# Ntropy86/review-recommender

Hardware: AMD Instinct MI355X
Metric: queries/sec at top-k=100 (hybrid alpha=0.5) (higher is better)
Workload: dtype f32; 1 GPU; hybrid BM25+dense alpha=0.5 top-k=100 pool=150, 10000000 products x 384 fp32, BM25 ~40 tokens/doc vocab 200000 (327073593 postings on rank 0, 11164874 postings per query), batches of 256 queries; query_sets=4, docs=10000000, docs_per_gpu=10000000, batch=256, k=100, pool=150, parallelism=single GPU: no collective

## Files before the change

include/rr_hip.h:

```cpp
#ifndef RR_HIP_H
#define RR_HIP_H

#include <stdint.h>

#ifdef __cplusplus
extern "C" {
#endif

#define RR_OK            0
#define RR_E_INVALID    -1
#define RR_E_HIP        -2
#define RR_E_NOMEM      -3
#define RR_E_STATE      -4

#define RR_DTYPE_F32     0
#define RR_DTYPE_BF16    1

#define RR_MAX_POOL   2048
#define RR_MAX_BATCH  1024
#define RR_MAX_QTERMS   64

typedef struct rr_index rr_index;
typedef struct rr_bm25  rr_bm25;

const char* rr_last_error(void);
int rr_version(void);
int rr_device_count(int* out);


int rr_index_create(const void* h_matrix, int64_t n_rows, int32_t dim, int32_t dtype,
                    int32_t device, int64_t row_offset, rr_index** out);
int rr_index_upload_rows(rr_index* ix, int64_t first_row, int64_t n_rows, const void* h_rows);
int rr_index_upload_rows_f32(rr_index* ix, int64_t first_row, int64_t n_rows, const float* h_rows,
                             float normalize_eps);
int rr_index_adopt_device(rr_index* ix, const void* d_matrix);
int rr_index_store_rows_dev(rr_index* ix, const float* d_rows, int64_t n, int64_t first_row, const int64_t* d_row_ids,
                            float normalize_eps, void* stream);
int rr_index_download_rows_f32(rr_index* ix, int64_t first_row, int64_t n, float* h_rows);
int rr_index_matrix_changed(rr_index* ix);
int rr_index_dim_padded(const rr_index* ix, int32_t* out);
int rr_index_l2_normalize(rr_index* ix, float eps);
int rr_index_set_meta(rr_index* ix, const double* h_n_reviews, const double* h_avg_stars,
                      const double* h_log1p_n);
int rr_index_destroy(rr_index* ix);


int rr_dense_topk(rr_index* ix, const float* h_queries, int32_t n_queries, int32_t pool,
                  int64_t* h_out_rows, float* h_out_scores, int32_t* pool_out);
int rr_dense_topk_dev(rr_index* ix, const float* d_queries, int32_t n_queries, int32_t pool,
                      int64_t* d_out_rows, float* d_out_scores, void* stream);
int rr_index_last_scan_ms(rr_index* ix, float* out_ms);
int rr_index_scan_stats(rr_index* ix, double* out_total_ms, int64_t* out_launches);
int rr_index_last_scan_info(rr_index* ix, int32_t* out8);
int rr_index_select_trace(rr_index* ix, int32_t* out16);
int rr_index_set_shadow(rr_index* ix, int32_t enable);
#define RR_SCAN_MODE_DEFAULT 0
#define RR_SCAN_MODE_STORED 1
int rr_index_set_scan_mode(rr_index* ix, int32_t mode);


int rr_bm25_create(int32_t device, int64_t n_docs, int64_t n_terms, int64_t nnz,
                   const int64_t* post_indptr, const int32_t* post_docs, const int32_t* post_tf,
                   const int64_t* doc_indptr, const int32_t* doc_terms, const int32_t* doc_tf,
                   const int32_t* doc_len, const double* idf, double avgdl, double k1, double b,
                   int64_t row_offset, rr_bm25** out);
int rr_bm25_create_dev(int32_t device, int64_t n_docs, int64_t n_terms, int64_t nnz,
                       const int64_t* d_post_indptr, const int32_t* d_post_docs, const int32_t* d_post_tf,
                       const int64_t* d_doc_indptr, const int32_t* d_doc_terms, const int32_t* d_doc_tf,
                       const int32_t* d_doc_len, const double* d_idf, double avgdl, double k1, double b,
                       int64_t row_offset, rr_bm25** out);
int rr_bm25_destroy(rr_bm25* bm);
int rr_bm25_get_scores(rr_bm25* bm, const int32_t* h_term_ids, int32_t n_terms_in_query,
                       double* h_out_scores);
int rr_bm25_scores_at(rr_bm25* bm, const int32_t* h_term_ids, const int32_t* h_term_off,
                      int32_t n_queries, const int64_t* h_rows, int32_t pool, int32_t mode,
                      float* h_out);
int rr_bm25_scores_at_dev(rr_bm25* bm, const int32_t* d_term_ids, const int32_t* d_term_off,
                          int32_t n_queries, const int64_t* d_rows, int32_t pool, int32_t mode,
                          float* d_out, void* stream);

int rr_bm25_build(int32_t device, int32_t inputs_on_device, const int32_t* tok, int64_t n_tok,
                  const int64_t* doc_off, int64_t n_src, int64_t n_terms, const int64_t* order,
                  int64_t n_order, int64_t row_lo, int64_t row_hi, double k1, double b,
                  int64_t row_offset, void* stream, rr_bm25** out);
int rr_bm25_build_stats(rr_bm25* bm, int64_t* h_df, int64_t* h_sizes);
int rr_bm25_set_idf(rr_bm25* bm, const double* h_idf, double avgdl);
int rr_bm25_copy_csr(rr_bm25* bm, int64_t* doc_indptr, int32_t* doc_terms, int32_t* doc_tf,
                     int32_t* doc_len, int64_t* post_indptr, int32_t* post_docs, int32_t* post_tf);


#define RR_MAX_CANDIDATES 4096

typedef struct rr_fuse_params {
    double w_dense, w_bm25, w_rerank, w_prior, w_best;
    double prior_C;
    int32_t min_reviews;
    int32_t trust_sat;
    int32_t apply_trust;
    int32_t rerank_active;
    int32_t rerank_k;
    int32_t k;
    int32_t n_candidates;
    int32_t pool;
    int32_t cand_per_rank;
    int32_t bm25_f64;
    int64_t cand_rank_stride_bytes;
} rr_fuse_params;

int rr_fuse_topk_dev(rr_index* ix, const rr_fuse_params* p, int32_t n_queries,
                     const int64_t* d_rows, const float* d_dense, const float* d_bm25,
                     const double* d_n_reviews, const double* d_avg_stars, const double* d_log1p_n,
                     const float* d_rerank, const float* d_best, const float* d_gate,
                     int64_t* d_out_rows, double* d_out_cols, int32_t* d_out_order, void* stream);
int rr_fuse_topk(rr_index* ix, const rr_fuse_params* p, int32_t n_queries,
                 const int64_t* h_rows, const float* h_dense, const float* h_bm25,
                 const double* h_n_reviews, const double* h_avg_stars, const double* h_log1p_n,
                 const float* h_rerank, const float* h_best, const float* h_gate,
                 int64_t* h_out_rows, double* h_out_cols, int32_t* h_out_order);
int rr_index_gather_meta_dev(rr_index* ix, const int64_t* d_rows, int64_t n,
                             double* d_n_reviews, double* d_avg_stars, double* d_log1p_n,
                             void* stream);

#define RR_COPY_MAX_SEGS 4
typedef struct rr_copy_seg {
    void* dst;
    const void* src;
    int64_t row_bytes, rows, dst_pitch, src_pitch;
} rr_copy_seg;
int rr_copy_segments_dev(const rr_copy_seg* segs, int32_t n_segs, int32_t device, void* stream);


typedef struct rr_reviews rr_reviews;
int rr_reviews_create(const float* h_emb, int64_t n_reviews, int32_t dim, int64_t n_products,
                      const int64_t* h_indptr, const int32_t* h_ids, int32_t device,
                      float normalize_eps, rr_reviews** out);
int rr_reviews_destroy(rr_reviews* rv);
int rr_reviews_best_dev(rr_reviews* rv, const float* d_queries, int32_t n_queries,
                        const int64_t* d_rows, int32_t pool, int64_t row_offset, int32_t max_review_id,
                        float* d_best_score, int32_t* d_best_id, void* stream);

int rr_reviews_best_cut_dev(rr_reviews* rv, const float* d_queries, int32_t n_queries,
                            const int64_t* d_rows, int32_t pool, int64_t row_offset, int64_t max_rows,
                            float* d_best_score, int32_t* d_best_id, void* stream);


typedef struct rr_ce rr_ce;
typedef struct rr_ce_config {
    int32_t hidden, n_layers, n_heads, ffn;
    int32_t vocab, max_pos, type_vocab;
    int32_t n_labels;
    float ln_eps;
    int32_t precision;
} rr_ce_config;
#define RR_CE_PRECISION_BF16 0
#define RR_CE_PRECISION_F32 1
int rr_ce_create(int32_t device, const rr_ce_config* cfg, const float* const* h_tensors, int32_t n_tensors, rr_ce** out);
int rr_ce_destroy(rr_ce* ce);
#define RR_CE_OUT_LOGITS 0
#define RR_CE_OUT_CLS    1
#define RR_CE_OUT_HIDDEN 2
int rr_ce_forward_dev(rr_ce* ce, const int32_t* d_token_ids, const int32_t* d_type_ids, const int32_t* d_pos_ids,
                      const int32_t* d_cu_seqlens, int32_t n_seqs, int64_t n_tokens, int32_t max_len, int32_t mode,
                      float* d_out, void* stream);
int rr_ce_last_forward_ms(rr_ce* ce, float* out_ms);
int rr_ce_range_status(rr_ce* ce, int32_t* out_of_range);
int rr_ce_set_wide_range(rr_ce* ce, int32_t on);


typedef struct rr_wp rr_wp;
int rr_wp_create(int32_t device, const uint8_t* h_piece_bytes, const int64_t* h_piece_off, int32_t n_pieces,
                 int32_t unk_id, int32_t cls_id, int32_t sep_id, int32_t max_chars_per_word, rr_wp** out);
int rr_wp_destroy(rr_wp* wp);
int rr_wp_create_utf8(int32_t device, const uint8_t* h_piece_bytes, const int64_t* h_piece_off, int32_t n_pieces,
                      int32_t unk_id, int32_t cls_id, int32_t sep_id, int32_t max_chars_per_word,
                      const uint16_t* h_stage1, int32_t n_stage1, const uint32_t* h_stage2, int32_t n_stage2,
                      const uint32_t* h_pool, int32_t n_pool, rr_wp** out);
int rr_wp_encode_dev(rr_wp* wp, const uint8_t* d_text, int64_t text_bytes, const int64_t* d_text_off, int32_t n_docs,
                     int32_t max_length, int64_t token_capacity, int32_t* d_token_ids, int32_t* d_type_ids, int32_t* d_pos_ids,
                     int32_t* d_cu_seqlens, int32_t* d_needs_host, int32_t* d_max_len, void* stream);
int rr_wp_status(rr_wp* wp, int32_t* out_bad_docs);
int rr_wp_table_slots(int32_t n_pieces, int32_t* out_slots);
int rr_wp_build_table(const uint8_t* h_piece_bytes, const int64_t* h_piece_off, int32_t n_pieces, int32_t max_chars_per_word,
                      int32_t n_slots, int32_t* h_slots, int32_t* out_kept);
int rr_wp_build_table_utf8(const uint8_t* h_piece_bytes, const int64_t* h_piece_off, int32_t n_pieces, int32_t max_chars_per_word,
                           int32_t n_slots, int32_t* h_slots, int32_t* out_kept);

int rr_dense_scan_dev(rr_index* ix, const float* d_queries, int32_t n_queries, int32_t top_k, int32_t kth,
                      float* d_bound, int32_t* applied, void* stream);
int rr_dense_select_dev(rr_index* ix, const float* d_queries, int32_t n_queries, int32_t top_k,
                        const float* d_floor, int64_t* d_out_rows, float* d_out_scores, void* stream);

int rr_dense_scan_slot_dev(rr_index* ix, int32_t slot, const float* d_queries, int32_t n_queries, int32_t top_k, int32_t kth,
                           float* d_bound, int32_t* applied, void* stream);
int rr_dense_select_slot_dev(rr_index* ix, int32_t slot, int32_t n_queries, int32_t top_k, const float* d_floor,
                             int64_t* d_out_rows, float* d_out_scores, void* stream);
int rr_dense_topk_slot_dev(rr_index* ix, int32_t slot, const float* d_queries, int32_t n_queries, int32_t top_k,
                           int64_t* d_out_rows, float* d_out_scores, void* stream);
#define RR_SELECT_LIST    1
#define RR_SELECT_RESCORE 2
#define RR_SELECT_ORDER   4
int rr_dense_select_part_dev(rr_index* ix, int32_t slot, int32_t parts, int32_t n_queries, int32_t top_k, const float* d_floor,
                             int64_t* d_out_rows, float* d_out_scores, void* stream);
int rr_stream_create_cu_range(int32_t device, int32_t first_cu, int32_t n_cus, void** out_stream);
int rr_stream_destroy(void* stream);
int rr_index_set_scan_cus(rr_index* ix, int32_t n_cus);

int rr_index_stream(rr_index* ix, void** out_stream);
int rr_index_synchronize(rr_index* ix);

#ifdef __cplusplus
}
#endif
#endif
```

review-recommender_amd/_lib.py:

```python
from __future__ import annotations

import ctypes as C
import os
import threading

from .build import DEBUG_BUILD_ID, BUILD_ID, DEBUG_LIB_PATH, LIB_PATH, library_digest

c_i32, c_i64, c_f32, c_f64, c_vp = C.c_int32, C.c_int64, C.c_float, C.c_double, C.c_void_p
P = C.POINTER


class CopySeg(C.Structure):
    _fields_ = [("dst", C.c_void_p), ("src", C.c_void_p), ("row_bytes", C.c_int64), ("rows", C.c_int64),
                ("dst_pitch", C.c_int64), ("src_pitch", C.c_int64)]


class FuseParams(C.Structure):
    _fields_ = [("w_dense", c_f64), ("w_bm25", c_f64), ("w_rerank", c_f64),
                ("w_prior", c_f64), ("w_best", c_f64), ("prior_C", c_f64),
                ("min_reviews", c_i32), ("trust_sat", c_i32), ("apply_trust", c_i32),
                ("rerank_active", c_i32), ("rerank_k", c_i32), ("k", c_i32),
                ("n_candidates", c_i32), ("pool", c_i32), ("cand_per_rank", c_i32),
                ("bm25_f64", c_i32), ("cand_rank_stride_bytes", c_i64)]


class CEConfig(C.Structure):
    _fields_ = [("hidden", c_i32), ("n_layers", c_i32), ("n_heads", c_i32), ("ffn", c_i32),
                ("vocab", c_i32), ("max_pos", c_i32), ("type_vocab", c_i32), ("n_labels", c_i32),
                ("ln_eps", c_f32), ("precision", c_i32)]


PROTOTYPES = {
    "rr_last_error": (C.c_char_p, []),
    "rr_version": (C.c_int, []),
    "rr_device_count": (C.c_int, [P(C.c_int)]),
    "rr_index_create": (C.c_int, [c_vp, c_i64, c_i32, c_i32, c_i32, c_i64, P(c_vp)]),
    "rr_index_upload_rows": (C.c_int, [c_vp, c_i64, c_i64, c_vp]),
    "rr_index_upload_rows_f32": (C.c_int, [c_vp, c_i64, c_i64, c_vp, c_f32]),
    "rr_index_adopt_device": (C.c_int, [c_vp, c_vp]),
    "rr_index_store_rows_dev": (C.c_int, [c_vp, c_vp, c_i64, c_i64, c_vp, c_f32, c_vp]),
    "rr_index_download_rows_f32": (C.c_int, [c_vp, c_i64, c_i64, c_vp]),
    "rr_index_dim_padded": (C.c_int, [c_vp, P(c_i32)]),
    "rr_index_l2_normalize": (C.c_int, [c_vp, c_f32]),
    "rr_index_set_meta": (C.c_int, [c_vp, c_vp, c_vp, c_vp]),
    "rr_index_destroy": (C.c_int, [c_vp]),
    "rr_dense_topk": (C.c_int, [c_vp, c_vp, c_i32, c_i32, c_vp, c_vp, P(c_i32)]),
    "rr_dense_topk_dev": (C.c_int, [c_vp, c_vp, c_i32, c_i32, c_vp, c_vp, c_vp]),
    "rr_index_last_scan_ms": (C.c_int, [c_vp, P(c_f32)]),
    "rr_index_scan_stats": (C.c_int, [c_vp, P(c_f64), P(c_i64)]),
    "rr_index_last_scan_info": (C.c_int, [c_vp, P(c_i32)]),
    "rr_index_select_trace": (C.c_int, [c_vp, P(c_i32)]),
    "rr_index_set_shadow": (C.c_int, [c_vp, c_i32]),
    "rr_index_set_scan_mode": (C.c_int, [c_vp, c_i32]),
    "rr_dense_scan_dev": (C.c_int, [c_vp, c_vp, c_i32, c_i32, c_i32, c_vp, P(c_i32), c_vp]),
    "rr_dense_select_dev": (C.c_int, [c_vp, c_vp, c_i32, c_i32, c_vp, c_vp, c_vp, c_vp]),
    "rr_dense_scan_slot_dev": (C.c_int, [c_vp, c_i32, c_vp, c_i32, c_i32, c_i32, c_vp, P(c_i32), c_vp]),
    "rr_dense_select_slot_dev": (C.c_int, [c_vp, c_i32, c_i32, c_i32, c_vp, c_vp, c_vp, c_vp]),
    "rr_dense_topk_slot_dev": (C.c_int, [c_vp, c_i32, c_vp, c_i32, c_i32, c_vp, c_vp, c_vp]),
    "rr_dense_select_part_dev": (C.c_int, [c_vp, c_i32, c_i32, c_i32, c_i32, c_vp, c_vp, c_vp, c_vp]),
    "rr_stream_create_cu_range": (C.c_int, [c_i32, c_i32, c_i32, P(c_vp)]),
    "rr_stream_destroy": (C.c_int, [c_vp]),
    "rr_index_set_scan_cus": (C.c_int, [c_vp, c_i32]),
    "rr_bm25_create": (C.c_int, [c_i32, c_i64, c_i64, c_i64, c_vp, c_vp, c_vp, c_vp, c_vp,
                                 c_vp, c_vp, c_vp, c_f64, c_f64, c_f64, c_i64, P(c_vp)]),
    "rr_bm25_create_dev": (C.c_int, [c_i32, c_i64, c_i64, c_i64, c_vp, c_vp, c_vp, c_vp, c_vp,
                                     c_vp, c_vp, c_vp, c_f64, c_f64, c_f64, c_i64, P(c_vp)]),
    "rr_bm25_destroy": (C.c_int, [c_vp]),
    "rr_bm25_get_scores": (C.c_int, [c_vp, c_vp, c_i32, c_vp]),
    "rr_bm25_scores_at": (C.c_int, [c_vp, c_vp, c_vp, c_i32, c_vp, c_i32, c_i32, c_vp]),
    "rr_bm25_scores_at_dev": (C.c_int, [c_vp, c_vp, c_vp, c_i32, c_vp, c_i32, c_i32, c_vp, c_vp]),
    "rr_bm25_build": (C.c_int, [c_i32, c_i32, c_vp, c_i64, c_vp, c_i64, c_i64, c_vp, c_i64, c_i64, c_i64,
                                c_f64, c_f64, c_i64, c_vp, P(c_vp)]),
    "rr_bm25_build_stats": (C.c_int, [c_vp, c_vp, c_vp]),
    "rr_bm25_set_idf": (C.c_int, [c_vp, c_vp, c_f64]),
    "rr_bm25_copy_csr": (C.c_int, [c_vp] + [c_vp] * 7),
    "rr_fuse_topk_dev": (C.c_int, [c_vp, P(FuseParams), c_i32] + [c_vp] * 9 + [c_vp] * 3 + [c_vp]),
    "rr_fuse_topk": (C.c_int, [c_vp, P(FuseParams), c_i32] + [c_vp] * 9 + [c_vp] * 3),
    "rr_index_gather_meta_dev": (C.c_int, [c_vp, c_vp, c_i64, c_vp, c_vp, c_vp, c_vp]),
    "rr_copy_segments_dev": (C.c_int, [c_vp, c_i32, c_i32, c_vp]),
    "rr_index_matrix_changed": (C.c_int, [c_vp]),
    "rr_reviews_create": (C.c_int, [c_vp, c_i64, c_i32, c_i64, c_vp, c_vp, c_i32, c_f32, P(c_vp)]),
    "rr_reviews_destroy": (C.c_int, [c_vp]),
    "rr_reviews_best_dev": (C.c_int, [c_vp, c_vp, c_i32, c_vp, c_i32, c_i64, c_i32, c_vp, c_vp, c_vp]),
    "rr_reviews_best_cut_dev": (C.c_int, [c_vp, c_vp, c_i32, c_vp, c_i32, c_i64, c_i64, c_vp, c_vp, c_vp]),
    "rr_ce_create": (C.c_int, [c_i32, P(CEConfig), P(c_vp), c_i32, P(c_vp)]),
    "rr_ce_destroy": (C.c_int, [c_vp]),
    "rr_ce_forward_dev": (C.c_int, [c_vp, c_vp, c_vp, c_vp, c_vp, c_i32, c_i64, c_i32, c_i32, c_vp, c_vp]),
    "rr_ce_last_forward_ms": (C.c_int, [c_vp, P(c_f32)]),
    "rr_ce_range_status": (C.c_int, [c_vp, P(C.c_int32)]),
    "rr_ce_set_wide_range": (C.c_int, [c_vp, C.c_int32]),
    "rr_wp_create": (C.c_int, [c_i32, c_vp, c_vp, c_i32, c_i32, c_i32, c_i32, c_i32, P(c_vp)]),
    "rr_wp_create_utf8": (C.c_int, [c_i32, c_vp, c_vp, c_i32, c_i32, c_i32, c_i32, c_i32, c_vp, c_i32, c_vp, c_i32, c_vp, c_i32,
                                    P(c_vp)]),
    "rr_wp_destroy": (C.c_int, [c_vp]),
    "rr_wp_encode_dev": (C.c_int, [c_vp, c_vp, c_i64, c_vp, c_i32, c_i32, c_i64, c_vp, c_vp, c_vp, c_vp, c_vp, c_vp, c_vp]),
    "rr_wp_status": (C.c_int, [c_vp, P(c_i32)]),
    "rr_wp_table_slots": (C.c_int, [c_i32, P(c_i32)]),
    "rr_wp_build_table": (C.c_int, [c_vp, c_vp, c_i32, c_i32, c_i32, c_vp, P(c_i32)]),
    "rr_wp_build_table_utf8": (C.c_int, [c_vp, c_vp, c_i32, c_i32, c_i32, c_vp, P(c_i32)]),
    "rr_index_stream": (C.c_int, [c_vp, P(c_vp)]),
    "rr_index_synchronize": (C.c_int, [c_vp]),
}

DEBUG_PROTOTYPES = {
    "rr_debug_scan_x3w": (C.c_int, [c_vp, c_i32, c_i32, P(c_f32)]),
    "rr_debug_scan_flt": (C.c_int, [c_vp, c_i32, c_i32, P(c_f32)]),
    "rr_debug_fltq_compare": (C.c_int, [c_vp, P(c_i64)]),
    "rr_debug_flt_words": (C.c_int, [c_vp, c_vp, c_i32, c_i32, c_i32, c_i32, c_i32, c_vp, c_vp, c_vp, c_vp, c_i64, c_vp, c_i64]),
    "rr_debug_flt_select": (C.c_int, [c_vp, c_i32, c_vp, c_i64, c_vp, c_vp, c_vp, c_vp]),
    "rr_debug_select_traces": (C.c_int, [c_vp, c_i32, c_vp]),
    "rr_debug_ce_ffn_stamps": (C.c_int, [P(C.c_uint64)]),
    "rr_debug_ce_h2_stamps": (C.c_int, [P(C.c_uint64)]),
    "rr_debug_ce_h2_gemm": (C.c_int, [c_i32, c_i32, c_i32, c_i32, c_vp, c_vp, c_vp, c_i32, c_vp, P(C.c_int32)]),
    "rr_debug_ce_h2_attention": (C.c_int, [c_vp, c_i32, c_vp, c_i32, c_i32, c_i32, c_i32, c_vp, P(C.c_int32)]),
    "rr_debug_ce_h2_add_ln": (C.c_int, [c_vp, c_vp, c_i32, c_vp, c_vp, c_f32, c_vp, c_vp, P(C.c_int32)]),
}

_lib = None
_lock = threading.Lock()


class HipLibraryError(RuntimeError):
    pass


def load():
    global _lib
    with _lock:
        if _lib is not None:
            return _lib
        debug = os.environ.get("RR_DEBUG_HARNESS") == "1"
        path = DEBUG_LIB_PATH if debug else LIB_PATH
        if not path.exists():
            raise HipLibraryError(
                f"{path} is missing: build it with `python __graft_entry__.py` "
                "(hipcc --offload-arch=gfx950).  There is no CPU fallback.")
        _refuse_stale(path, DEBUG_BUILD_ID if debug else BUILD_ID, debug)
        import torch
        lib = C.CDLL(str(path))
        protos = dict(PROTOTYPES, **DEBUG_PROTOTYPES) if debug else PROTOTYPES
        for name, (res, args) in protos.items():
            try:
                fn = getattr(lib, name)
            except AttributeError:
                raise HipLibraryError(f"stale library: {path.name} lacks the declared symbol {name}; rebuild it with "
                                      "`python __graft_entry__.py`") from None
            fn.restype = res
            fn.argtypes = args
        _lib = lib
        return lib


def _refuse_stale(path, build_id, debug: bool) -> None:
    have = build_id.read_text().strip() if build_id.exists() else None
    if have != library_digest(debug):
        raise HipLibraryError(
            f"stale library: {path.name} was built from other sources than the ones in csrc/ "
            f"(buildid {'missing' if have is None else have[:12]} != {library_digest(debug)[:12]}); "
            "rebuild it with `python __graft_entry__.py`")


def check(rc: int, what: str = "") -> None:
    if rc == 0:
        return
    msg = load().rr_last_error().decode("utf-8", "replace")
    if rc == -1:
        raise ValueError(f"{what}: {msg}" if what else msg)
    raise HipLibraryError(f"{what}: {msg} (status {rc})" if what else f"{msg} (status {rc})")


def ptr(a):
    if a is None:
        return None
    if not a.flags["C_CONTIGUOUS"]:
        raise ValueError("array passed to the HIP library must be C-contiguous")
    return a.ctypes.data_as(c_vp)
```

review-recommender_amd/csrc/rr_bm25.hip:

```cpp
#include "rr_common.h"

#define RR_SLICE 4096
#define RR_AT_CANDS 64

struct rr_bm25_view {
    const int64_t* post_indptr;
    const int32_t* post_docs;
    const int32_t* post_tf;
    const int64_t* doc_indptr;
    const int32_t* doc_terms;
    const int32_t* doc_tf;
    const int32_t* doc_len;
    const double* idf;
    double avgdl, k1, b;
    int64_t n_docs, n_terms, row_offset;
};

__device__ __forceinline__ double rr_bm25_term(double idf, int tf, int dl, double avgdl, double k1,
                                               double b) {
    const double f = (double)tf;
    const double one_minus_b = 1.0 - b;
    const double norm = one_minus_b + (b * (double)dl) / avgdl;
    return idf * ((f * (k1 + 1.0)) / (f + k1 * norm));
}

__device__ __forceinline__ int64_t rr_lower_bound(const int32_t* __restrict__ a, int64_t lo,
                                                  int64_t hi, int32_t key) {
    while (lo < hi) {
        const int64_t mid = lo + ((hi - lo) >> 1);
        if (a[mid] < key) lo = mid + 1; else hi = mid;
    }
    return lo;
}

__device__ __forceinline__ int64_t rr_lower_bound_wave(const int32_t* __restrict__ a, int64_t lo, int64_t hi, int32_t key) {
    const int lane = threadIdx.x & 63;
    while (hi - lo > 64) {
        const int64_t stride = (hi - lo + 63) >> 6;
        const int64_t at = lo + lane * stride;
        const bool below = at < hi && a[at] < key;
        const int c = __popcll(__ballot(below));
        if (c == 0) return lo;
        const int64_t nlo = lo + (int64_t)(c - 1) * stride + 1, nhi = lo + (int64_t)c * stride;
        lo = nlo;
        hi = nhi < hi ? nhi : hi;
    }
    const bool below = lo + lane < hi && a[lo + lane] < key;
    return lo + __popcll(__ballot(below));
}

#define RR_SLICE_TERMS 16
__global__ __launch_bounds__(256) void rr_bm25_slices(rr_bm25_view v, const int32_t* __restrict__ terms,
                                                      int n_terms_q, double* __restrict__ out, unsigned char* __restrict__ dirty) {
    __shared__ double acc[RR_SLICE];
    __shared__ int64_t range[RR_SLICE_TERMS][2];
    __shared__ int touched;
    const int tid = threadIdx.x, wave = tid >> 6;
    const int64_t d0 = (int64_t)blockIdx.x * RR_SLICE;
    const int64_t d1 = d0 + RR_SLICE < v.n_docs ? d0 + RR_SLICE : v.n_docs;
    for (int i = tid; i < RR_SLICE; i += 256) acc[i] = 0.0;
    if (tid == 0) touched = 0;
    for (int j0 = 0; j0 < n_terms_q; j0 += RR_SLICE_TERMS) {
        const int nj = n_terms_q - j0 < RR_SLICE_TERMS ? n_terms_q - j0 : RR_SLICE_TERMS;
        __syncthreads();
        for (int sidx = wave; sidx < 2 * nj; sidx += 4) {
            const int32_t t = terms[j0 + (sidx >> 1)];
            int64_t r = 0;
            if (t >= 0 && t < v.n_terms)
                r = rr_lower_bound_wave(v.post_docs, v.post_indptr[t], v.post_indptr[t + 1], (int32_t)((sidx & 1) ? d1 : d0));
            if ((tid & 63) == 0) range[sidx >> 1][sidx & 1] = r;
        }
        __syncthreads();
        int32_t nd = 0, ntf = 0, ndl = 0;
        bool nhave = false;
        {
            const int64_t p = range[0][0] + tid;
            nhave = p < range[0][1];
            if (nhave) { nd = v.post_docs[p]; ntf = v.post_tf[p]; ndl = v.doc_len[nd]; }
        }
        for (int j = 0; j < nj; ++j) {
            const int64_t lo = range[j][0], hi = range[j][1];
            const int32_t t = terms[j0 + j];
            const bool have = nhave;
            const int32_t d = nd, tf = ntf, dl = ndl;
            if (j + 1 < nj) {
                const int64_t p = range[j + 1][0] + tid;
                nhave = p < range[j + 1][1];
                if (nhave) { nd = v.post_docs[p]; ntf = v.post_tf[p]; ndl = v.doc_len[nd]; }
            }
            if (hi > lo) {
                const double idf = v.idf[t];
                if (tid == 0) touched = 1;
                if (have) acc[d - d0] += rr_bm25_term(idf, tf, dl, v.avgdl, v.k1, v.b);
                for (int64_t p = lo + 256 + tid; p < hi; p += 256) {
                    const int32_t dd = v.post_docs[p];
                    acc[dd - d0] += rr_bm25_term(idf, v.post_tf[p], v.doc_len[dd], v.avgdl, v.k1, v.b);
                }
            }
            __syncthreads();
        }
    }
    __syncthreads();
    const bool write = touched || dirty[blockIdx.x];
    if (write)
        for (int64_t i = tid; i < d1 - d0; i += 256) out[d0 + i] = acc[i];
    if (tid == 0) dirty[blockIdx.x] = (unsigned char)touched;
}

template <int MODE>
__global__ __launch_bounds__(256) void rr_bm25_at(rr_bm25_view v, const int32_t* __restrict__ term_ids,
                                                  const int32_t* __restrict__ term_off,
                                                  const int64_t* __restrict__ rows, int pool,
                                                  float* __restrict__ out) {
    __shared__ double contrib[RR_AT_CANDS][RR_MAX_QTERMS + 1];
    const int tid = threadIdx.x;
    const int q = blockIdx.y;
    const int c0 = blockIdx.x * RR_AT_CANDS;
    const int t0 = term_off[q];
    const int nt = term_off[q + 1] - t0;
    const int nc = pool - c0 < RR_AT_CANDS ? pool - c0 : RR_AT_CANDS;
    double sum = 0.0;

    for (int jb = 0; jb < nt; jb += RR_MAX_QTERMS) {
        const int nj = nt - jb < RR_MAX_QTERMS ? nt - jb : RR_MAX_QTERMS;
        for (int i = tid; i < nc * nj; i += 256) {
            const int c = i / nj, j = i % nj;
            const int64_t d = rows[(int64_t)q * pool + c0 + c] - v.row_offset;
            const int32_t t = term_ids[t0 + jb + j];
            double val = 0.0;
            if (d >= 0 && d < v.n_docs && t >= 0 && t < v.n_terms) {
                int tf = 0;
                if (MODE == 0) {
                    const int64_t s = v.doc_indptr[d], e = v.doc_indptr[d + 1];
                    const int64_t p = rr_lower_bound(v.doc_terms, s, e, t);
                    if (p < e && v.doc_terms[p] == t) tf = v.doc_tf[p];
                } else {
                    const int64_t s = v.post_indptr[t], e = v.post_indptr[t + 1];
                    const int64_t p = rr_lower_bound(v.post_docs, s, e, (int32_t)d);
                    if (p < e && v.post_docs[p] == (int32_t)d) tf = v.post_tf[p];
                }
                if (tf > 0) val = rr_bm25_term(v.idf[t], tf, v.doc_len[d], v.avgdl, v.k1, v.b);
            }
            contrib[c][j] = val;
        }
        __syncthreads();
        if (tid < nc)
            for (int j = 0; j < nj; ++j) sum += contrib[tid][j];
        __syncthreads();
    }
    if (tid < nc) out[(int64_t)q * pool + c0 + tid] = (float)sum;
}

template <typename T>
static int rr_upload(T** dst, const T* src, size_t n) {
    *dst = nullptr;
    RR_HIP_TRY(hipMalloc((void**)dst, sizeof(T) * (n ? n : 1)));
    if (n) RR_HIP_TRY(hipMemcpy(*dst, src, sizeof(T) * n, hipMemcpyHostToDevice));
    return RR_OK;
}

static rr_bm25_view rr_view(const rr_bm25* bm) {
    rr_bm25_view v;
    v.post_indptr = bm->d_post_indptr; v.post_docs = bm->d_post_docs; v.post_tf = bm->d_post_tf;
    v.doc_indptr = bm->d_doc_indptr; v.doc_terms = bm->d_doc_terms; v.doc_tf = bm->d_doc_tf;
    v.doc_len = bm->d_doc_len; v.idf = bm->d_idf;
    v.avgdl = bm->avgdl; v.k1 = bm->k1; v.b = bm->b;
    v.n_docs = bm->n_docs; v.n_terms = bm->n_terms; v.row_offset = bm->row_offset;
    return v;
}

extern "C" int rr_bm25_create(int32_t device, int64_t n_docs, int64_t n_terms, int64_t nnz,
                              const int64_t* post_indptr, const int32_t* post_docs,
                              const int32_t* post_tf, const int64_t* doc_indptr,
                              const int32_t* doc_terms, const int32_t* doc_tf,
                              const int32_t* doc_len, const double* idf, double avgdl, double k1,
                              double b, int64_t row_offset, rr_bm25** out) {
    RR_REQUIRE(out, "rr_bm25_create: NULL out");
    *out = nullptr;
    RR_REQUIRE(n_docs >= 1 && n_docs < (1ll << 31), "rr_bm25_create: n_docs %lld out of range",
               (long long)n_docs);
    RR_REQUIRE(n_terms >= 0 && n_terms < (1ll << 31) && nnz >= 0, "rr_bm25_create: bad sizes");
    RR_REQUIRE(post_indptr && doc_indptr && doc_len && (nnz == 0 || (post_docs && post_tf && doc_terms && doc_tf)) &&
                   (n_terms == 0 || idf),
               "rr_bm25_create: NULL array");
    RR_REQUIRE(post_indptr[n_terms] == nnz && doc_indptr[n_docs] == nnz,
               "rr_bm25_create: indptr tails (%lld, %lld) do not match nnz %lld",
               (long long)post_indptr[n_terms], (long long)doc_indptr[n_docs], (long long)nnz);
    RR_REQUIRE(avgdl > 0.0, "rr_bm25_create: avgdl must be positive");
    RR_HIP_TRY(hipSetDevice(device));
    rr_bm25* bm = new rr_bm25();
    bm->device = device; bm->n_docs = n_docs; bm->n_terms = n_terms; bm->nnz = nnz;
    bm->avgdl = avgdl; bm->k1 = k1; bm->b = b; bm->row_offset = row_offset;
    int rc = RR_OK;
    if (!rc) rc = rr_upload(&bm->d_post_indptr, post_indptr, (size_t)n_terms + 1);
    if (!rc) rc = rr_upload(&bm->d_post_docs, post_docs, (size_t)nnz);
    if (!rc) rc = rr_upload(&bm->d_post_tf, post_tf, (size_t)nnz);
    if (!rc) rc = rr_upload(&bm->d_doc_indptr, doc_indptr, (size_t)n_docs + 1);
    if (!rc) rc = rr_upload(&bm->d_doc_terms, doc_terms, (size_t)nnz);
    if (!rc) rc = rr_upload(&bm->d_doc_tf, doc_tf, (size_t)nnz);
    if (!rc) rc = rr_upload(&bm->d_doc_len, doc_len, (size_t)n_docs);
    if (!rc) rc = rr_upload(&bm->d_idf, idf, (size_t)n_terms);
    if (!rc && hipStreamCreateWithFlags(&bm->stream, hipStreamNonBlocking) != hipSuccess) {
        rr_set_error("rr_bm25_create: hipStreamCreate failed");
        rc = RR_E_HIP;
    }
    if (rc) { rr_bm25_destroy(bm); return rc; }
    *out = bm;
    return RR_OK;
}

extern "C" int rr_bm25_create_dev(int32_t device, int64_t n_docs, int64_t n_terms, int64_t nnz,
                                  const int64_t* d_post_indptr, const int32_t* d_post_docs,
                                  const int32_t* d_post_tf, const int64_t* d_doc_indptr,
                                  const int32_t* d_doc_terms, const int32_t* d_doc_tf,
                                  const int32_t* d_doc_len, const double* d_idf, double avgdl,
                                  double k1, double b, int64_t row_offset, rr_bm25** out) {
    RR_REQUIRE(out, "rr_bm25_create_dev: NULL out");
    *out = nullptr;
    RR_REQUIRE(n_docs >= 1 && n_docs < (1ll << 31) && n_terms >= 1 && n_terms < (1ll << 31) && nnz >= 1,
               "rr_bm25_create_dev: bad sizes");
    RR_REQUIRE(d_post_indptr && d_post_docs && d_post_tf && d_doc_indptr && d_doc_terms && d_doc_tf &&
                   d_doc_len && d_idf, "rr_bm25_create_dev: NULL array");
    RR_REQUIRE(avgdl > 0.0, "rr_bm25_create_dev: avgdl must be positive");
    RR_HIP_TRY(hipSetDevice(device));
    int64_t tails[2] = {-1, -1};
    RR_HIP_TRY(hipMemcpy(&tails[0], d_post_indptr + n_terms, sizeof(int64_t), hipMemcpyDeviceToHost));
    RR_HIP_TRY(hipMemcpy(&tails[1], d_doc_indptr + n_docs, sizeof(int64_t), hipMemcpyDeviceToHost));
    RR_REQUIRE(tails[0] == nnz && tails[1] == nnz, "rr_bm25_create_dev: indptr tails (%lld, %lld) != nnz %lld",
               (long long)tails[0], (long long)tails[1], (long long)nnz);
    rr_bm25* bm = new rr_bm25();
    bm->device = device; bm->n_docs = n_docs; bm->n_terms = n_terms; bm->nnz = nnz;
    bm->avgdl = avgdl; bm->k1 = k1; bm->b = b; bm->row_offset = row_offset;
    bm->owns_arrays = false;
    bm->d_post_indptr = const_cast<int64_t*>(d_post_indptr);
    bm->d_post_docs = const_cast<int32_t*>(d_post_docs);
    bm->d_post_tf = const_cast<int32_t*>(d_post_tf);
    bm->d_doc_indptr = const_cast<int64_t*>(d_doc_indptr);
    bm->d_doc_terms = const_cast<int32_t*>(d_doc_terms);
    bm->d_doc_tf = const_cast<int32_t*>(d_doc_tf);
    bm->d_doc_len = const_cast<int32_t*>(d_doc_len);
    bm->d_idf = const_cast<double*>(d_idf);
    if (hipStreamCreateWithFlags(&bm->stream, hipStreamNonBlocking) != hipSuccess) {
        rr_set_error("rr_bm25_create_dev: hipStreamCreate failed");
        delete bm;
        return RR_E_HIP;
    }
    *out = bm;
    return RR_OK;
}

extern "C" int rr_bm25_destroy(rr_bm25* bm) {
    if (!bm) return RR_OK;
    hipSetDevice(bm->device);
    if (bm->owns_arrays) {
        hipFree(bm->d_post_indptr); hipFree(bm->d_post_docs); hipFree(bm->d_post_tf);
        hipFree(bm->d_doc_indptr); hipFree(bm->d_doc_terms); hipFree(bm->d_doc_tf);
        hipFree(bm->d_doc_len); hipFree(bm->d_idf); hipFree(bm->d_df);
    }
    hipFree(bm->d_scores);
    hipFree(bm->d_dirty);
    if (bm->stream) hipStreamDestroy(bm->stream);
    delete bm;
    return RR_OK;
}

extern "C" int rr_bm25_get_scores(rr_bm25* bm, const int32_t* h_term_ids, int32_t n_terms_in_query,
                                  double* h_out_scores) {
    RR_REQUIRE(bm && h_out_scores && (n_terms_in_query == 0 || h_term_ids),
               "rr_bm25_get_scores: NULL argument");
    RR_REQUIRE(n_terms_in_query >= 0 && n_terms_in_query <= 4096,
               "rr_bm25_get_scores: %d query tokens out of [0,4096]", n_terms_in_query);
    if (!bm->d_idf) { rr_set_error("rr_bm25_get_scores: no idf yet (rr_bm25_set_idf)"); return RR_E_STATE; }
    std::lock_guard<std::mutex> lk(bm->mu);
    RR_HIP_TRY(hipSetDevice(bm->device));
    const unsigned grid = (unsigned)((bm->n_docs + RR_SLICE - 1) / RR_SLICE);
    if (!bm->d_scores) {
        RR_HIP_TRY(hipMalloc((void**)&bm->d_scores, sizeof(double) * (size_t)bm->n_docs));
        RR_HIP_TRY(hipMalloc((void**)&bm->d_dirty, grid));
        RR_HIP_TRY(hipMemsetAsync(bm->d_scores, 0, sizeof(double) * (size_t)bm->n_docs, bm->stream));
        RR_HIP_TRY(hipMemsetAsync(bm->d_dirty, 0, grid, bm->stream));
    }
    int32_t* d_terms = nullptr;
    RR_HIP_TRY(hipMalloc((void**)&d_terms, sizeof(int32_t) * (size_t)(n_terms_in_query + 1)));
    if (n_terms_in_query)
        hipMemcpyAsync(d_terms, h_term_ids, sizeof(int32_t) * n_terms_in_query, hipMemcpyHostToDevice,
                       bm->stream);
    hipLaunchKernelGGL(rr_bm25_slices, dim3(grid), dim3(256), 0, bm->stream, rr_view(bm), d_terms,
                       n_terms_in_query, bm->d_scores, bm->d_dirty);
    hipError_t e = hipGetLastError();
    if (e == hipSuccess)
        e = hipMemcpyAsync(h_out_scores, bm->d_scores, sizeof(double) * (size_t)bm->n_docs,
                           hipMemcpyDeviceToHost, bm->stream);
    if (e == hipSuccess) e = hipStreamSynchronize(bm->stream);
    hipFree(d_terms);
    if (e != hipSuccess) {
        rr_set_error("rr_bm25_get_scores: %s", hipGetErrorString(e));
        return RR_E_HIP;
    }
    return RR_OK;
}

extern "C" int rr_bm25_scores_at_dev(rr_bm25* bm, const int32_t* d_term_ids,
                                     const int32_t* d_term_off, int32_t n_queries,
                                     const int64_t* d_rows, int32_t pool, int32_t mode,
                                     float* d_out, void* stream) {
    RR_REQUIRE(bm && d_term_ids && d_term_off && d_rows && d_out, "rr_bm25_scores_at_dev: NULL argument");
    RR_REQUIRE(n_queries >= 1 && n_queries <= RR_MAX_BATCH && pool >= 1 && pool <= 8 * RR_MAX_POOL,
               "rr_bm25_scores_at_dev: n_queries %d / pool %d out of range", n_queries, pool);
    RR_REQUIRE(mode == 0 || mode == 1, "rr_bm25_scores_at_dev: mode must be 0 (forward) or 1 (postings)");
    if (!bm->d_idf) { rr_set_error("rr_bm25_scores_at_dev: no idf yet (rr_bm25_set_idf)"); return RR_E_STATE; }
    RR_HIP_TRY(hipSetDevice(bm->device));
    hipStream_t st = (hipStream_t)stream;
    dim3 grid((unsigned)((pool + RR_AT_CANDS - 1) / RR_AT_CANDS), (unsigned)n_queries);
    if (mode == 0)
        hipLaunchKernelGGL((rr_bm25_at<0>), grid, dim3(256), 0, st, rr_view(bm), d_term_ids, d_term_off,
                           d_rows, pool, d_out);
    else
        hipLaunchKernelGGL((rr_bm25_at<1>), grid, dim3(256), 0, st, rr_view(bm), d_term_ids, d_term_off,
                           d_rows, pool, d_out);
    RR_HIP_TRY(hipGetLastError());
    return RR_OK;
}

extern "C" int rr_bm25_scores_at(rr_bm25* bm, const int32_t* h_term_ids, const int32_t* h_term_off,
                                 int32_t n_queries, const int64_t* h_rows, int32_t pool,
                                 int32_t mode, float* h_out) {
    RR_REQUIRE(bm && h_term_off && h_rows && h_out, "rr_bm25_scores_at: NULL argument");
    RR_REQUIRE(n_queries >= 1 && n_queries <= RR_MAX_BATCH && pool >= 1 && pool <= 8 * RR_MAX_POOL,
               "rr_bm25_scores_at: n_queries %d / pool %d out of range", n_queries, pool);
    const int total_terms = h_term_off[n_queries];
    RR_REQUIRE(total_terms >= 0 && (total_terms == 0 || h_term_ids), "rr_bm25_scores_at: bad term arrays");
    for (int q = 0; q < n_queries; ++q)
        RR_REQUIRE(h_term_off[q + 1] - h_term_off[q] >= 0, "rr_bm25_scores_at: term offsets must not decrease (query %d)", q);
    std::lock_guard<std::mutex> lk(bm->mu);
    RR_HIP_TRY(hipSetDevice(bm->device));
    int32_t *d_ids = nullptr, *d_off = nullptr;
    int64_t* d_rows = nullptr;
    float* d_out = nullptr;
    const size_t n_out = (size_t)n_queries * pool;
    hipError_t e = hipMalloc((void**)&d_ids, sizeof(int32_t) * (size_t)(total_terms + 1));
    if (e == hipSuccess) e = hipMalloc((void**)&d_off, sizeof(int32_t) * (size_t)(n_queries + 1));
    if (e == hipSuccess) e = hipMalloc((void**)&d_rows, sizeof(int64_t) * n_out);
    if (e == hipSuccess) e = hipMalloc((void**)&d_out, sizeof(float) * n_out);
    if (e == hipSuccess && total_terms)
        e = hipMemcpyAsync(d_ids, h_term_ids, sizeof(int32_t) * total_terms, hipMemcpyHostToDevice, bm->stream);
    if (e == hipSuccess)
        e = hipMemcpyAsync(d_off, h_term_off, sizeof(int32_t) * (n_queries + 1), hipMemcpyHostToDevice, bm->stream);
    if (e == hipSuccess)
        e = hipMemcpyAsync(d_rows, h_rows, sizeof(int64_t) * n_out, hipMemcpyHostToDevice, bm->stream);
    int rc = RR_OK;
    if (e == hipSuccess)
        rc = rr_bm25_scores_at_dev(bm, d_ids, d_off, n_queries, d_rows, pool, mode, d_out, bm->stream);
    if (e == hipSuccess && rc == RR_OK)
        e = hipMemcpyAsync(h_out, d_out, sizeof(float) * n_out, hipMemcpyDeviceToHost, bm->stream);
    if (e == hipSuccess && rc == RR_OK) e = hipStreamSynchronize(bm->stream);
    hipFree(d_ids); hipFree(d_off); hipFree(d_rows); hipFree(d_out);
    if (rc) return rc;
    if (e != hipSuccess) {
        rr_set_error("rr_bm25_scores_at: %s", hipGetErrorString(e));
        return RR_E_HIP;
    }
    return RR_OK;
}
```

review-recommender_amd/csrc/rr_common.h:

```cpp
#pragma once

#include <hip/hip_runtime.h>
#include <stdint.h>
#include <stdio.h>
#include <string.h>
#include <mutex>
#include <string>

#include "../../include/rr_hip.h"

void rr_set_error(const char* fmt, ...);

#define RR_HIP_TRY(expr)                                                        \
    do {                                                                        \
        hipError_t _e = (expr);                                                 \
        if (_e != hipSuccess) {                                                 \
            rr_set_error("%s failed: %s (%s:%d)", #expr, hipGetErrorString(_e), \
                         __FILE__, __LINE__);                                   \
            return RR_E_HIP;                                                    \
        }                                                                       \
    } while (0)

#define RR_REQUIRE(cond, ...)             \
    do {                                  \
        if (!(cond)) {                    \
            rr_set_error(__VA_ARGS__);    \
            return RR_E_INVALID;          \
        }                                 \
    } while (0)

#define RR_SCAN_SLOTS 3
struct rr_scan_slot {
    float* d_q = nullptr;
    void* d_qplanes = nullptr;
    float* d_eps = nullptr;
    float* d_gmax = nullptr;
    uint32_t* d_smax = nullptr;
    int32_t maxima_q = 0;
    float* d_flt_samp = nullptr;
    float* d_flt_sigma = nullptr;
    uint32_t* d_flt_prog = nullptr;
    uint32_t flt_seq = 0;
    bool flt_prep_fresh = false;
    void* flt_pending = nullptr;
};

struct rr_index {
    int device = 0;
    int64_t n_rows = 0;
    int32_t dim = 0;
    int32_t dim_pad = 0;
    int32_t dtype = RR_DTYPE_F32;
    int64_t row_offset = 0;
    void* d_matrix = nullptr;
    bool owns_matrix = true;
    double* d_n_reviews = nullptr;
    double* d_avg_stars = nullptr;
    double* d_log1p_n = nullptr;
    bool has_meta = false;
    float* d_sims = nullptr;
    float* d_gmax = nullptr;
    int32_t* d_sel_trace = nullptr;
    int32_t* d_flag_list = nullptr;
    uint32_t* d_smax = nullptr;
    int32_t scratch_q = 0;
    int32_t maxima_q = 0;
    float* d_eps = nullptr;
    float* d_q = nullptr;
    float norm_bound = -1.f;
    float delta_bound = 0.f;
    int32_t last_scan[5] = {0, 0, 0, 0, 0};
    float* d_flt_samp = nullptr;
    float* d_flt_sigma = nullptr;
    uint32_t* d_flt_prog = nullptr;
    uint32_t flt_seq = 0;
    bool scratch_small = false;
    bool flt_prep_fresh = false;
    void* flt_pending = nullptr;
    unsigned short* d_shadow = nullptr;
    bool shadow_valid = false;
    int32_t use_shadow = 1;
    int32_t scan_mode = 0;
    void* d_x3 = nullptr;
    void* d_qplanes = nullptr;
    int64_t* d_rows_out = nullptr;
    float* d_scores_out = nullptr;
    hipStream_t stream = nullptr;
    hipEvent_t ev0 = nullptr, ev1 = nullptr;
    hipEvent_t ev_done = nullptr;
    hipStream_t last_stream = nullptr;
    bool has_done = false;
    rr_scan_slot parked[RR_SCAN_SLOTS];
    int cur_slot = 0;
    hipEvent_t slot_ev[RR_SCAN_SLOTS] = {};
    hipStream_t slot_stream[RR_SCAN_SLOTS] = {};
    bool slot_has[RR_SCAN_SLOTS] = {};
    int32_t n_cus = 0;
    int32_t scan_cus = 0;
    bool timing_valid = false;
    static const int kRing = 512;
    hipEvent_t ring0[kRing] = {}, ring1[kRing] = {};
    int64_t ring_head = 0, ring_tail = 0;
    std::mutex mu;
};

struct rr_bm25 {
    int device = 0;
    int64_t n_docs = 0, n_terms = 0, nnz = 0;
    int64_t row_offset = 0;
    int64_t* d_post_indptr = nullptr;
    int32_t* d_post_docs = nullptr;
    int32_t* d_post_tf = nullptr;
    int64_t* d_doc_indptr = nullptr;
    int32_t* d_doc_terms = nullptr;
    int32_t* d_doc_tf = nullptr;
    int32_t* d_doc_len = nullptr;
    double* d_idf = nullptr;
    int64_t* d_df = nullptr;
    int64_t n_src = 0, length_sum = 0;
    double avgdl = 1.0, k1 = 1.5, b = 0.75;
    bool owns_arrays = true;
    double* d_scores = nullptr;
    unsigned char* d_dirty = nullptr;
    hipStream_t stream = nullptr;
    std::mutex mu;
};

static inline int64_t rr_round_up(int64_t x, int64_t m) { return (x + m - 1) / m * m; }

#ifdef __HIPCC__

typedef float f32x4 __attribute__((ext_vector_type(4)));

__device__ __forceinline__ uint32_t rr_f2key(float f) {
    uint32_t u = __float_as_uint(f);
    return (u & 0x80000000u) ? ~u : (u | 0x80000000u);
}
__device__ __forceinline__ float rr_key2f(uint32_t k) {
    uint32_t u = (k & 0x80000000u) ? (k & 0x7FFFFFFFu) : ~k;
    return __uint_as_float(u);
}

__device__ __forceinline__ float rr_row16_sum(float v) {
    int t;
    t = __builtin_amdgcn_update_dpp(0, __float_as_int(v), 0xB1, 0xF, 0xF, true);
    v = v + __int_as_float(t);
    t = __builtin_amdgcn_update_dpp(0, __float_as_int(v), 0x4E, 0xF, 0xF, true);
    v = v + __int_as_float(t);
    t = __builtin_amdgcn_update_dpp(0, __float_as_int(v), 0x141, 0xF, 0xF, true);
    v = v + __int_as_float(t);
    t = __builtin_amdgcn_update_dpp(0, __float_as_int(v), 0x140, 0xF, 0xF, true);
    v = v + __int_as_float(t);
    return v;
}

__device__ __forceinline__ float rr_wave_max(float v) {
#pragma unroll
    for (int m = 32; m >= 1; m >>= 1) v = fmaxf(v, __shfl_xor(v, m, 64));
    return v;
}

#endif
```

review-recommender_amd/csrc/rr_dense.h:

```cpp
#pragma once
#include "rr_common.h"

#define RR_SCAN_THREADS 256
#define RR_MAX_SCAN_WAVES 8192
#define RR_MFMA_MAXQ 64
#define RR_FLT_MAXQ 128
#define RR_SEL_MAXQ 256
#define RR_FLT_SAMP_CAP 8192
#define RR_FLT_NO_BOUND 1000
#define RR_FLT_SMALL 1001

struct rr_scan_geom {
    int64_t n_rows, n_tiles;
    int64_t tiles_per_wave;
    int32_t n_waves;
    int32_t qs;
    int64_t n_pad;
    int32_t mm_pairs;
    int32_t gpw;
    int64_t tiles_per_group;
};


rr_scan_geom rr_make_geom(const rr_index* ix, int resident_blocks);
static inline void rr_scan_note(rr_index* ix, int kernel, int variant, int nq, int terms, int elem_bytes = 0) {
    ix->last_scan[0] = kernel; ix->last_scan[1] = variant; ix->last_scan[2] = nq; ix->last_scan[3] = terms;
    ix->last_scan[4] = elem_bytes ? elem_bytes : (ix->dtype == RR_DTYPE_BF16 ? 2 : 4);
}
static inline void rr_matrix_written(rr_index* ix) {
    ix->norm_bound = -1.f;
    ix->shadow_valid = false;
}
int rr_slot_activate(rr_index* ix, int slot);
void rr_slot_park(rr_index* ix);
int rr_scan_events_begin(rr_index* ix, hipStream_t st);
void rr_scan_events_end(rr_index* ix, int slot, hipStream_t st);
int rr_dense_listed_fallback(rr_index* ix, const float* d_q, int nq, int pool, int64_t* d_rows, float* d_scores,
                             int32_t* flags, hipStream_t st);
void rr_launch_select(rr_index* ix, const rr_scan_geom& G, int nq, int pool, int64_t* d_rows,
                      float* d_scores, hipStream_t st, const int32_t* only_if = nullptr, int slices = 1,
                      int64_t sims_slice = 0, int64_t gmax_slice = 0, int64_t smax_slice = 0);
#define RR_X3_MCAP 16384
struct rr_x3_scratch {
    uint32_t* mtiles;
    int32_t* count;
    uint32_t* tau;
    int32_t* fb;
    float* eps;
    float* sc;
};
rr_x3_scratch rr_x3_scratch_of(const rr_index* ix);
size_t rr_x3_scratch_bytes();
void rr_launch_select_mtiles(rr_index* ix, const rr_scan_geom& G, int nq, int pool, hipStream_t st,
                             const float* eps = nullptr, const float* sigma = nullptr, int nq_b = 0,
                             int64_t mmax_set_stride = 0, int64_t smax_set_stride = 0, const float* floor = nullptr);
void rr_launch_select_rescored(rr_index* ix, const rr_scan_geom& G, int nq, int pool, int64_t* d_rows,
                               float* d_scores, hipStream_t st, bool floor_mode = false);
void rr_launch_group_kth(rr_index* ix, const rr_scan_geom& G, int nq_a, int nq_b, int kth, const float* eps, float* d_bound,
                         int64_t smax_set_stride, hipStream_t st);
int rr_resident_waves(const void* kernel, int threads, int device);
int rr_dense_chunk_bf16(rr_index* ix, const float* d_q, int nq, int pool, int64_t* d_rows,
                        float* d_scores, hipStream_t st);
int rr_dense_chunk_mfma_bf16(rr_index* ix, const float* d_q, int nq, int pool, int64_t* d_rows,
                             float* d_scores, hipStream_t st);
int rr_l2norm_rows_f32(rr_index* ix, int64_t first_row, int64_t n, float eps, hipStream_t st);
int rr_l2norm_rows_f32_at(float* d_rows, int32_t dim_pad, int64_t n, float eps, hipStream_t st);
int rr_dense_chunk_x3(rr_index* ix, const float* d_q, int nq, int pool, int64_t* d_rows,
                      float* d_scores, hipStream_t st);
int rr_dense_chunk_flt(rr_index* ix, const float* d_q, int nq, int pool, int64_t* d_rows,
                       float* d_scores, hipStream_t st, int phase = 0, int kth = 0, float* d_bound = nullptr,
                       const float* d_floor = nullptr, int parts = 7);
void rr_flt_drop_pending(rr_index* ix);
int rr_store_rows_bf16(rr_index* ix, int64_t first_row, int64_t n, float* d_rows_f32, float eps, hipStream_t st);
int rr_store_rows_bf16_at(void* d_dst, int32_t dim, int32_t dim_pad, int64_t n, const float* d_rows_f32, float eps, hipStream_t st);

int rr_device_visible(const void* p, const void** out, const char* what);

int rr_flt_pad_prep(rr_index* ix, const float* d_queries, int nq, int slots, hipStream_t st);
```

review-recommender_amd/csrc/rr_dense.hip:

```cpp
#include <stdlib.h>

#include "rr_common.h"
#include "rr_dense.h"
#include "rr_x3.h"

#define RR_SEL_THREADS 1024
#define RR_SEL_GCAP 4096
#define RR_SEL_CCAP 12288
#define RR_SEL_SORTCAP 8192
#define RR_SEL_RCAP 8192
#define RR_SEL_LCAP 4096

template <int NF>
__device__ __forceinline__ void rr_load_rows(f32x4 (&dst)[NF], const f32x4* __restrict__ mat,
                                             int64_t row, int64_t n_rows, int sub) {
    row = row < n_rows ? row : n_rows - 1;
    const f32x4* p = mat + row * (int64_t)(NF * 16) + sub;
#pragma unroll
    for (int i = 0; i < NF; ++i) dst[i] = __builtin_nontemporal_load(p + 16 * i);
}

template <int NF, int NB, bool FROM_LDS>
__device__ __forceinline__ void rr_dot_rows(const f32x4 (&x)[NF], const f32x4 (&qreg)[NF],
                                            const f32x4 (*qs)[NF * 16], int sub, int it,
                                            float (&mine)[NB]) {
#pragma unroll
    for (int b = 0; b < NB; ++b) {
        if (FROM_LDS) asm volatile("" ::: "memory");
        float acc = 0.f;
#pragma unroll
        for (int i = 0; i < NF; ++i) {
            const f32x4 q = FROM_LDS ? qs[b][16 * i + sub] : qreg[i];
            acc = __builtin_fmaf(x[i].x, q.x, acc);
            acc = __builtin_fmaf(x[i].y, q.y, acc);
            acc = __builtin_fmaf(x[i].z, q.z, acc);
            acc = __builtin_fmaf(x[i].w, q.w, acc);
        }
        acc = rr_row16_sum(acc);
        mine[b] = (sub == it) ? acc : mine[b];
    }
}

template <int NB>
__device__ __forceinline__ void rr_finish_tile(const rr_scan_geom& G, int64_t tile, int64_t wave,
                                               int64_t t0, int64_t t1, int lane, int sub, int grp,
                                               float (&mine)[NB], float (&gm)[NB],
                                               float* __restrict__ sims, float* __restrict__ gmax,
                                               uint32_t* __restrict__ smax) {
    const int64_t my_row = tile * 64 + 4 * sub + grp;
    const bool valid = my_row < G.n_rows;
    const bool group_end = tile == t1 - 1;
#pragma unroll
    for (int b = 0; b < NB; ++b) {
        float v = mine[b];
        v = (valid && v == v) ? v : -INFINITY;
        sims[(int64_t)b * G.n_pad + my_row] = v;
        const float m = rr_wave_max(v);
        gm[b] = fmaxf(gm[b], m);
        if (lane == 0) {
            gmax[(int64_t)b * G.n_tiles + tile] = m;
            if (group_end)
                smax[(int64_t)b * G.n_waves + wave] = rr_f2key(gm[b]);
        }
        if (group_end) gm[b] = -INFINITY;
    }
}

template <int NB>
__device__ __forceinline__ int rr_flagged_list(const int32_t* __restrict__ flags, int nq, int lane, int (&list)[NB]) {
    int n = 0, total = 0;
#pragma unroll
    for (int b = 0; b < NB; ++b) list[b] = 0;
    for (int i = 0; i < (nq + 63) / 64; ++i) {
        const int q = 64 * i + lane;
        unsigned long long m = __ballot(q < nq && flags[q] != 0);
        total += __builtin_popcountll(m);
        while (m && n < NB) {
            const int b = __builtin_ctzll(m);
            m &= m - 1;
#pragma unroll
            for (int j = 0; j < NB; ++j)
                if (j == n) list[j] = 64 * i + b;
            ++n;
        }
    }
    if (total > NB) return 0;
#pragma unroll
    for (int j = 1; j < NB; ++j)
        if (j >= n && n > 0) list[j] = list[j - 1];
    return n;
}

template <int NF, int NB, bool LISTED = false>
__global__ __launch_bounds__(RR_SCAN_THREADS, (NB <= 1 ? 4 : 2)) void rr_scan_f32(
    const f32x4* __restrict__ mat, rr_scan_geom G, const float* __restrict__ queries,
    float* __restrict__ sims, float* __restrict__ gmax, uint32_t* __restrict__ smax,
    const int32_t* __restrict__ flags = nullptr, int nq_total = 0, int32_t* __restrict__ list_out = nullptr) {
    __shared__ f32x4 qs[NB][NF * 16];
    const int tid = threadIdx.x;
    if (LISTED) {
        int list[NB];
        const int n = rr_flagged_list<NB>(flags, nq_total, tid & 63, list);
        if (blockIdx.x == 0 && tid == 0) {
            list_out[0] = n;
#pragma unroll
            for (int b = 0; b < NB; ++b) list_out[1 + b] = list[b];
        }
        if (n == 0) return;
#pragma unroll
        for (int b = 0; b < NB; ++b)
            for (int i = tid; i < NF * 16; i += RR_SCAN_THREADS)
                qs[b][i] = reinterpret_cast<const f32x4*>(queries)[(int64_t)list[b] * (NF * 16) + i];
    } else {
        for (int i = tid; i < NB * NF * 16; i += RR_SCAN_THREADS)
            qs[i / (NF * 16)][i % (NF * 16)] = reinterpret_cast<const f32x4*>(queries)[i];
    }
    __syncthreads();

    const int lane = tid & 63;
    const int sub = lane & 15;
    const int grp = lane >> 4;
    const int64_t wave = (int64_t)blockIdx.x * (RR_SCAN_THREADS / 64) + (tid >> 6);
    if (wave >= G.n_waves) return;
    const int64_t t0 = wave * G.tiles_per_wave;
    const int64_t t1 = t0 + G.tiles_per_wave < G.n_tiles ? t0 + G.tiles_per_wave : G.n_tiles;

    f32x4 qreg[NF];
#pragma unroll
    for (int i = 0; i < NF; ++i) qreg[i] = (NB == 1) ? qs[0][16 * i + sub] : f32x4{0.f, 0.f, 0.f, 0.f};

    float gm[NB];
#pragma unroll
    for (int b = 0; b < NB; ++b) gm[b] = -INFINITY;

    f32x4 bufA[NF], bufB[NF];
    rr_load_rows<NF>(bufA, mat, t0 * 64 + grp, G.n_rows, sub);
#pragma unroll 1
    for (int64_t tile = t0; tile < t1; ++tile) {
        const int64_t row0 = tile * 64;
        float mine[NB];
#pragma unroll
        for (int b = 0; b < NB; ++b) mine[b] = 0.f;
#pragma unroll(NB == 1 ? 8 : 1)
        for (int it = 0; it < 16; it += 2) {
            rr_load_rows<NF>(bufB, mat, row0 + 4 * (it + 1) + grp, G.n_rows, sub);
            rr_dot_rows<NF, NB, (NB > 1)>(bufA, qreg, qs, sub, it, mine);
            rr_load_rows<NF>(bufA, mat, row0 + 4 * (it + 2) + grp, G.n_rows, sub);
            rr_dot_rows<NF, NB, (NB > 1)>(bufB, qreg, qs, sub, it + 1, mine);
        }
        rr_finish_tile<NB>(G, tile, wave, t0, t1, lane, sub, grp, mine, gm, sims, gmax, smax);
    }
}

template <int NB>
__global__ __launch_bounds__(RR_SCAN_THREADS) void rr_scan_f32_generic(
    const f32x4* __restrict__ mat, rr_scan_geom G, int nf, const float* __restrict__ queries,
    float* __restrict__ sims, float* __restrict__ gmax, uint32_t* __restrict__ smax) {
    const int tid = threadIdx.x;
    const int lane = tid & 63;
    const int sub = lane & 15;
    const int grp = lane >> 4;
    const int64_t wave = (int64_t)blockIdx.x * (RR_SCAN_THREADS / 64) + (tid >> 6);
    if (wave >= G.n_waves) return;
    const int64_t t0 = wave * G.tiles_per_wave;
// ... 263 lines not shown
            const int64_t t = all_tiles ? (i >> 6) : (int64_t)glist[i >> 6];
            const int64_t row = t * 64 + (i & 63);
            if (row < n_rows) {
                const uint64_t key = ((uint64_t)rr_f2key(score_at(row)) << 32) |
                                     (uint64_t)(0xFFFFFFFFu - (uint32_t)row);
                if (key >= prefix) {
                    const uint32_t slot = atomicAdd(&counters[1], 1u);
                    if (slot < RR_SEL_SORTCAP) cand[slot] = key;
                }
            }
        }
        __syncthreads();
        n_cand = counters[1] < RR_SEL_SORTCAP ? counters[1] : RR_SEL_SORTCAP;
    }

    if (n_cand > RR_SEL_SORTCAP) n_cand = RR_SEL_SORTCAP;
    int n_sort = 1;
    while (n_sort < (int)n_cand) n_sort <<= 1;
    for (int i = tid; i < n_sort; i += RR_SEL_THREADS)
        if (i >= (int)n_cand) cand[i] = 0;
    rr_bitonic_desc(cand, n_sort);
}

#define RR_SEL_RK 8
template <int RK>
__device__ uint32_t rr_kth_largest_reg(const uint32_t (&r)[RR_SEL_RK], int n_mine, uint32_t k,
                                       uint32_t (*cnt)[3][16], int& phase, int max_steps) {
    const int tid = threadIdx.x;
    const int ln = tid & 63;
    uint32_t mx = 0, mn = 0xFFFFFFFFu, nz = 0;
#pragma unroll
    for (int j = 0; j < RK; ++j) {
        const bool live = j < n_mine && r[j] != 0u;
        if (j < n_mine) mx = r[j] > mx ? r[j] : mx;
        if (live) mn = r[j] < mn ? r[j] : mn;
        nz += (uint32_t)__popcll(__ballot(live));
    }
#pragma unroll
    for (int m = 32; m >= 1; m >>= 1) {
        const uint32_t a = __shfl_xor(mx, m, 64), b = __shfl_xor(mn, m, 64);
        mx = a > mx ? a : mx;
        mn = b < mn ? b : mn;
    }
    if (ln == 0) {
        cnt[phase][0][tid >> 6] = mx;
        cnt[phase][1][tid >> 6] = mn;
        cnt[phase][2][tid >> 6] = nz;
    }
    __syncthreads();
    uint32_t nz_all = 0;
    for (int w = 0; w < 16; ++w) {
        mx = cnt[phase][0][w] > mx ? cnt[phase][0][w] : mx;
        mn = cnt[phase][1][w] < mn ? cnt[phase][1][w] : mn;
        nz_all += cnt[phase][2][w];
    }
    if (nz_all < k) mn = 0u;
    phase ^= 1;
    if (mx == mn) return mx;
    int bit = 31 - __clz(mx ^ mn);
    uint32_t prefix = (bit == 31) ? 0u : (mx >> (bit + 1)) << (bit + 1);
    for (int step = 0; bit >= 0 && step < max_steps; ++step) {
        const int lo = bit >= 1 ? bit - 1 : 0;
        const bool two = bit >= 1;
        const uint32_t t1 = prefix | (1u << lo);
        const uint32_t t2 = prefix | (1u << bit);
        const uint32_t t3 = prefix | (1u << bit) | (1u << lo);
        uint32_t c1 = 0, c2 = 0, c3 = 0;
#pragma unroll
        for (int j = 0; j < RK; ++j) {
            const bool have = j < n_mine;
            c1 += (uint32_t)__popcll(__ballot(have && r[j] >= t1));
            c2 += (uint32_t)__popcll(__ballot(have && r[j] >= t2));
            c3 += (uint32_t)__popcll(__ballot(have && r[j] >= t3));
        }
        if (ln == 0) {
            cnt[phase][0][tid >> 6] = c1;
            cnt[phase][1][tid >> 6] = c2;
            cnt[phase][2][tid >> 6] = c3;
        }
        __syncthreads();
        int v = ln < 48 ? (int)(&cnt[phase][0][0])[ln] : 0;
        v += __builtin_amdgcn_update_dpp(0, v, 0xB1, 0xF, 0xF, true);
        v += __builtin_amdgcn_update_dpp(0, v, 0x4E, 0xF, 0xF, true);
        v += __builtin_amdgcn_update_dpp(0, v, 0x141, 0xF, 0xF, true);
        v += __builtin_amdgcn_update_dpp(0, v, 0x140, 0xF, 0xF, true);
        const uint32_t s1 = (uint32_t)__builtin_amdgcn_readlane(v, 0);
        const uint32_t s2 = (uint32_t)__builtin_amdgcn_readlane(v, 16);
        const uint32_t s3 = (uint32_t)__builtin_amdgcn_readlane(v, 32);
        phase ^= 1;
        if (two) {
            if (s3 >= k) prefix = t3;
            else if (s2 >= k) prefix = t2;
            else if (s1 >= k) prefix = t1;
        } else if (s2 >= k) {
            prefix = t2;
        }
        bit = lo - 1;
    }
    return prefix;
}

__device__ void rr_rank_sort_desc(const uint64_t* keys, int n, uint64_t* out) {
    const int tid = threadIdx.x;
    uint64_t mine = 0;
    int rank = 0;
    if (tid < n) {
        mine = keys[tid];
        for (int j = 0; j < n; ++j) rank += keys[j] > mine ? 1 : 0;
    }
    __syncthreads();
    if (tid < n) out[rank] = mine;
    __syncthreads();
}

template <typename GroupKeyAt>
__device__ uint32_t rr_sel_open_groups(GroupKeyAt group_key_at, int ng, int pool, uint32_t (*cnt)[3][16],
                                       int& phase, uint32_t* counters, uint32_t* list2,
                                       float eps2 = -1.f, uint32_t* open_key = nullptr, uint32_t thr_floor = 0u) {
    const int tid = threadIdx.x;
    uint32_t r[RR_SEL_RK];
    int n_mine = 0;
#pragma unroll
    for (int j = 0; j < RR_SEL_RK; ++j) {
        const int i = tid + j * RR_SEL_THREADS;
        r[j] = i < ng ? group_key_at(i) : 0u;
        n_mine += i < ng ? 1 : 0;
    }
    uint32_t tau = 1u;
    if (ng > pool) {
        if (ng <= 1 * RR_SEL_THREADS) tau = rr_kth_largest_reg<1>(r, n_mine, (uint32_t)pool, cnt, phase, 7);
        else if (ng <= 2 * RR_SEL_THREADS) tau = rr_kth_largest_reg<2>(r, n_mine, (uint32_t)pool, cnt, phase, 7);
        else if (ng <= 4 * RR_SEL_THREADS) tau = rr_kth_largest_reg<4>(r, n_mine, (uint32_t)pool, cnt, phase, 7);
        else tau = rr_kth_largest_reg<8>(r, n_mine, (uint32_t)pool, cnt, phase, 7);
    }
    if (tau == 0u) tau = 1u;
    uint32_t thr = tau;
    if (eps2 >= 0.f) {
        thr = rr_f2key(rr_key2f(tau) - eps2);
        if (thr == 0u) thr = 1u;
        if (thr_floor > thr) thr = thr_floor;
        if (open_key) *open_key = thr;
    }
#pragma unroll
    for (int j = 0; j < RR_SEL_RK; ++j) {
        if (j < n_mine && r[j] >= thr) {
            const uint32_t slot = atomicAdd(&counters[0], 1u);
            if (slot < RR_SEL_LCAP) list2[slot] = (uint32_t)(tid + j * RR_SEL_THREADS);
        }
    }
    __syncthreads();
    return tau;
}

__global__ __launch_bounds__(RR_SEL_THREADS) void rr_select(
    rr_scan_geom G, const float* __restrict__ sims, const float* __restrict__ gmax,
    const uint32_t* __restrict__ smax, int pool, int64_t row_offset,
    int64_t* __restrict__ out_rows, float* __restrict__ out_scores, int32_t* __restrict__ dbg,
    const int32_t* __restrict__ only_if, int n_total, int64_t sims_slice, int64_t gmax_slice, int64_t smax_slice,
    const int32_t* __restrict__ qlist, int32_t* __restrict__ clear_flags) {
    if (qlist) {
        if ((int)blockIdx.x >= qlist[0]) return;
        const int qo = qlist[1 + blockIdx.x] - (int)blockIdx.x;
        out_rows += (int64_t)qo * pool; out_scores += (int64_t)qo * pool; dbg += qo * 16;
        if (threadIdx.x == 0) clear_flags[qo + (int)blockIdx.x] = 0;
    }
    if (gridDim.y > 1) {
        const int y = blockIdx.y;
        if (64 * y + (int)blockIdx.x >= n_total) return;
        only_if += 64 * y;
        out_rows += (int64_t)64 * y * pool; out_scores += (int64_t)64 * y * pool; dbg += 64 * y * 16;
        sims += y * sims_slice; gmax += y * gmax_slice; smax += y * smax_slice;
    }
    if (only_if && !only_if[blockIdx.x]) return;
    __shared__ uint32_t hist[256];
    __shared__ uint32_t wsum[4];
    __shared__ uint32_t cnt[2][3][16];
    __shared__ uint32_t sel[2];
    __shared__ uint32_t counters[4];
    __shared__ uint32_t list2[RR_SEL_LCAP];
    __shared__ uint32_t list1[RR_SEL_GCAP];
    __shared__ uint64_t cand[RR_SEL_CCAP];

    const int tid = threadIdx.x;
    const int q = blockIdx.x;
    const int QS = G.qs;
    auto score_at = [&](int64_t row) -> float {
        return QS ? sims[((row >> 4) * QS + q) * 16 + (row & 15)] : sims[(int64_t)q * G.n_pad + row];
    };
    auto tile_max_at = [&](int64_t t) -> float {
        return QS ? gmax[t * QS + q] : gmax[(int64_t)q * G.n_tiles + t];
    };
    auto group_key_at = [&](int i) -> uint32_t {
        return QS ? smax[(int64_t)i * QS + q] : smax[(int64_t)q * G.n_waves + i];
    };
    const int64_t n_rows = G.n_rows, n_tiles = G.n_tiles;
    int phase = 0;
    long long stamp[8];
    int n_stamp = 0;
#define RR_STAMP() do { if (n_stamp < 8) stamp[n_stamp++] = clock64(); } while (0)
    RR_STAMP();
    const int ng = G.n_waves;
    bool fast = ng <= RR_SEL_RK * RR_SEL_THREADS;

    if (tid < 4) counters[tid] = 0;
    __syncthreads();

    if (fast) {
        const uint32_t tau = rr_sel_open_groups(group_key_at, ng, pool, cnt, phase, counters, list2);
        RR_STAMP();
        if (counters[0] > RR_SEL_LCAP) fast = false;

        if (fast) {
            const int C = (int)G.tiles_per_wave;
            const int64_t n2 = (int64_t)counters[0] * C;
            for (int64_t i = tid; i < n2; i += RR_SEL_THREADS) {
                const int64_t t = (int64_t)list2[i / C] * C + (i % C);
                if (t < n_tiles && rr_f2key(tile_max_at(t)) >= tau) {
                    const uint32_t slot = atomicAdd(&counters[1], 1u);
                    if (slot < RR_SEL_GCAP) list1[slot] = (uint32_t)t;
                }
            }
            __syncthreads();
            if (counters[1] > RR_SEL_GCAP) fast = false;
        }
        RR_STAMP();
        if (fast) {
            const int n1 = (int)counters[1] * 64;
            for (int i = tid; i < n1; i += RR_SEL_THREADS) {
                const uint32_t row = list1[i >> 6] * 64u + (uint32_t)(i & 63);
                if ((int64_t)row < n_rows) {
                    const uint32_t key = rr_f2key(score_at(row));
                    if (key >= tau) {
                        const uint32_t slot = atomicAdd(&counters[2], 1u);
                        if (slot < RR_SEL_CCAP / 2)
                            cand[slot] = ((uint64_t)key << 32) | (uint64_t)(0xFFFFFFFFu - row);
                    }
                }
            }
            __syncthreads();
            RR_STAMP();
            const uint32_t n_cand = counters[2];
            if (n_cand > RR_SEL_CCAP / 2 || n_cand < (uint32_t)pool) {
                fast = false;
            } else if (n_cand <= RR_SEL_THREADS) {
                rr_rank_sort_desc(cand, (int)n_cand, cand + RR_SEL_CCAP / 2);
                for (int i = tid; i < pool; i += RR_SEL_THREADS) cand[i] = cand[RR_SEL_CCAP / 2 + i];
                __syncthreads();
            } else {
                int n_sort = 1;
                while (n_sort < (int)n_cand) n_sort <<= 1;
                for (int i = tid; i < n_sort; i += RR_SEL_THREADS)
                    if (i >= (int)n_cand) cand[i] = 0;
                rr_bitonic_desc(cand, n_sort);
            }
        }
    }
    RR_STAMP();
    if (tid == 0) {
        dbg[q * 16 + 0] = fast ? 1 : 0;
        dbg[q * 16 + 1] = (int32_t)counters[0];
        dbg[q * 16 + 2] = (int32_t)counters[1];
        dbg[q * 16 + 3] = (int32_t)counters[2];
        for (int i = 1; i < 8; ++i) dbg[q * 16 + 3 + i] = i < n_stamp ? (int32_t)(stamp[i] - stamp[i - 1]) : -1;
    }
    if (!fast) {
        __syncthreads();
        rr_select_slow(score_at, tile_max_at, n_rows, n_tiles, pool, hist, wsum, sel, counters, list1, cand);
    }
    for (int i = tid; i < pool; i += RR_SEL_THREADS) {
        const uint64_t key = cand[i];
        const uint32_t row = 0xFFFFFFFFu - (uint32_t)(key & 0xFFFFFFFFu);
        out_rows[(int64_t)q * pool + i] = (int64_t)row + row_offset;
        out_scores[(int64_t)q * pool + i] = rr_key2f((uint32_t)(key >> 32));
    }
}

__global__ __launch_bounds__(RR_SEL_THREADS) void rr_select_mtiles(
    rr_scan_geom G, const float* __restrict__ mmax, const uint32_t* __restrict__ smax, int pool,
    uint32_t* __restrict__ out_mtiles, int32_t* __restrict__ out_count, uint32_t* __restrict__ out_tau,
    int32_t* __restrict__ fb, int32_t* __restrict__ dbg, const float* __restrict__ eps,
    const float* __restrict__ sigma, int nq_a, int nq_b, int64_t mmax_set_stride, int64_t smax_set_stride,
    const float* __restrict__ floor) {
    __shared__ uint32_t cnt[2][3][16];
    __shared__ uint32_t counters[4];
    __shared__ uint32_t list2[RR_SEL_LCAP];
    const int tid = threadIdx.x;
    const int Q = blockIdx.x;
    const int set = (nq_b > 0 && Q >= nq_a) ? 1 : 0;
    const int q = set ? Q - nq_a : Q;
    const int nq_set = set ? nq_b : nq_a;
    mmax += set * mmax_set_stride;
    smax += set * smax_set_stride;
    if (eps) eps += set * RR_FLT_MAXQ;
    if (sigma) sigma += set * RR_FLT_MAXQ;
    out_mtiles += (int64_t)(Q - q) * RR_X3_MCAP;
    out_count += Q - q; out_tau += Q - q; fb += Q - q; dbg += (Q - q) * 16;
    const int QS = G.qs;
    auto group_key_at = [&](int i) -> uint32_t { return smax[(int64_t)i * QS + q]; };
    const int gpw = G.gpw > 1 ? G.gpw : 1;
    const int ng = G.n_waves * gpw;
    int phase = 0;
    const long long c0 = clock64();
    long long c1 = c0, c2 = c0;
    if (tid < 4) counters[tid] = 0;
    __syncthreads();
    bool ok = ng <= RR_SEL_RK * RR_SEL_THREADS && ng > pool;
    uint32_t tau = 1u;
    uint32_t open = 1u;
    if (ok) {
        const float e = eps ? eps[q] : -1.f;
        if (eps && !(e >= 0.f && e < 3.0e38f)) ok = false;
        if (ok) {
            const float fl = (floor && eps) ? floor[Q] - 1.05f * e : -INFINITY;
            if (fl > -3.0e38f) {
                open = rr_f2key(fl);
                if (open == 0u) open = 1u;
                for (int i = tid; i < ng; i += RR_SEL_THREADS) {
                    if (group_key_at(i) >= open) {
                        const uint32_t slot = atomicAdd(&counters[0], 1u);
                        if (slot < RR_SEL_LCAP) list2[slot] = (uint32_t)i;
                    }
                }
                __syncthreads();
                tau = rr_f2key(floor[Q]);
                if (counters[0] > RR_SEL_LCAP) {
                    __syncthreads();
                    if (tid == 0) counters[0] = 0;
                    __syncthreads();
                    const uint32_t floor_open = open, floor_tau = tau;
                    tau = rr_sel_open_groups(group_key_at, ng, pool, cnt, phase, counters, list2, 2.05f * e, &open, floor_open);
                    tau = rr_f2key(rr_key2f(tau) - 1.02f * e);
                    if (floor_tau > tau) tau = floor_tau;
                }
            } else {
                tau = rr_sel_open_groups(group_key_at, ng, pool, cnt, phase, counters, list2, eps ? 2.05f * e : -1.f, &open, 0u);
                if (!eps) open = tau;
                else tau = rr_f2key(rr_key2f(tau) - 1.02f * e);
            }
            if (tau == 0u) tau = 1u;
            if (counters[0] > RR_SEL_LCAP) ok = false;
        }
    }
    c1 = clock64();
    if (ok) {
        const int C = (int)G.tiles_per_group;
        const int64_t n2 = (int64_t)counters[0] * C;
        const f32x4* mm4 = reinterpret_cast<const f32x4*>(mmax);
        if (G.mm_pairs == 3) {
            constexpr int U = 4;
            const float step = rr_flt_gap_step(eps, nq_set);
            const float openf = open <= 0x007FFFFFu ? -INFINITY : rr_key2f(open);
            if (sigma && !(sigma[q] <= openf)) ok = false;
            const int n2i = (int)n2;
            for (int i0 = tid; i0 < n2i; i0 += U * RR_SEL_THREADS) {
                int64_t tt[U];
                uint32_t w0[U], w1[U];
#pragma unroll
                for (int u = 0; u < U; ++u) {
                    const int i = i0 + u * RR_SEL_THREADS;
                    tt[u] = -1;
                    if (i < n2i) {
                        const int g = (int)list2[i / C], k = g % gpw, j = i % C;
                        const int64_t in_run = (int64_t)k * C + j;
                        const int64_t t = (int64_t)(g / gpw) * G.tiles_per_wave + in_run;
                        if (in_run < G.tiles_per_wave && t < G.n_tiles) tt[u] = t;
                    }
                    const int64_t ts = tt[u] < 0 ? 0 : tt[u];
                    w0[u] = reinterpret_cast<const uint32_t*>(mmax)[(2 * ts) * QS + q];
                    w1[u] = reinterpret_cast<const uint32_t*>(mmax)[(2 * ts + 1) * QS + q];
                }
#pragma unroll
                for (int u = 0; u < U; ++u) {
                    if (tt[u] < 0) continue;
#pragma unroll
                    for (int half = 0; half < 2; ++half) {
                        const uint32_t w = half ? w1[u] : w0[u];
                        const float mx = __uint_as_float(w << 16);
                        if (!(mx >= openf)) continue;
#pragma unroll
                        for (int g = 0; g < 4; ++g) {
                            const uint32_t code = (w >> (16 + 4 * g)) & 15u;
                            const float bound = mx - rr_flt_gap_steps(code) * step;
                            if (bound >= openf) {
                                const uint32_t slot = atomicAdd(&counters[1], 1u);
                                if (slot < RR_X3_MCAP) out_mtiles[(int64_t)q * RR_X3_MCAP + slot] = (uint32_t)(tt[u] * 8 + 4 * half + g);
                            }
                        }
                    }
                }
            }
        } else
        for (int64_t i = tid; i < n2; i += RR_SEL_THREADS) {
            const int g = (int)list2[i / C], k = g % gpw, j = (int)(i % C);
            const int64_t in_run = (int64_t)k * C + j;
            const int64_t t = (int64_t)(g / gpw) * G.tiles_per_wave + in_run;
            if (in_run >= G.tiles_per_wave || t >= G.n_tiles) continue;
            float v[4];
            if (G.mm_pairs) {
                const float2 m0 = reinterpret_cast<const float2*>(mmax)[(2 * t) * QS + q];
                const float2 m1 = reinterpret_cast<const float2*>(mmax)[(2 * t + 1) * QS + q];
                v[0] = m0.x, v[1] = m0.y, v[2] = m1.x, v[3] = m1.y;
            } else {
                const f32x4 m = mm4[t * QS + q];
                v[0] = m.x, v[1] = m.y, v[2] = m.z, v[3] = m.w;
            }
#pragma unroll
            for (int sub = 0; sub < 4; ++sub) {
                if (rr_f2key(v[sub]) >= open) {
                    const uint32_t slot = atomicAdd(&counters[1], 1u);
                    if (slot < RR_X3_MCAP) out_mtiles[(int64_t)q * RR_X3_MCAP + slot] = (uint32_t)(t * 4 + sub);
                }
            }
        }
        __syncthreads();
        if (counters[1] > RR_X3_MCAP) ok = false;
    }
    c2 = clock64();
    if (tid == 0) {
        out_count[q] = ok ? (int32_t)counters[1] : 0;
        out_tau[q] = tau;
        fb[q] = ok ? 0 : 1;
        dbg[q * 16 + 0] = ok ? 2 : 0;
        dbg[q * 16 + 1] = (int32_t)counters[0];
        dbg[q * 16 + 2] = (int32_t)counters[1];
        dbg[q * 16 + 3] = 0;
        dbg[q * 16 + 4] = (int32_t)(c1 - c0);
        dbg[q * 16 + 5] = (int32_t)(c2 - c1);
        for (int i = 6; i < 16; ++i) dbg[q * 16 + i] = -1;
#ifdef RR_DEBUG_HARNESS
        dbg[q * 16 + 6] = (int32_t)open;
#endif
    }
}

template <int RCAP>
__global__ __launch_bounds__(RR_SEL_THREADS) void rr_select_rescored(
    rr_scan_geom G, const uint32_t* __restrict__ mtiles, const int32_t* __restrict__ count,
    const uint32_t* __restrict__ tau_of, const float* __restrict__ sc, int pool, int64_t row_offset,
    int64_t* __restrict__ out_rows, float* __restrict__ out_scores, int32_t* __restrict__ fb,
    int32_t* __restrict__ dbg, int floor_mode) {
    __shared__ uint32_t counters[2];
    __shared__ uint64_t cand[RCAP];
    const int tid = threadIdx.x;
    const int q = blockIdx.x;
    if (fb[q]) return;
    if (tid < 2) counters[tid] = 0;
    __syncthreads();
    const uint32_t tau = tau_of[q];
    const int sh = G.mm_pairs == 3 ? 3 : 4;
    const int n1 = count[q] << sh;
    const bool all_rows = floor_mode && (uint32_t)n1 <= RCAP / 2;
    for (int i = tid; i < n1 && !all_rows; i += RR_SEL_THREADS) {
        const int64_t at = (int64_t)q * RR_X3_MCAP + (i >> sh);
        const int r = i & ((1 << sh) - 1);
        const uint32_t row = (mtiles[at] << sh) + (uint32_t)r;
        if ((int64_t)row < G.n_rows) {
            const uint32_t key = rr_f2key(sc[(at << sh) + r]);
            if (key >= tau) {
                const uint32_t slot = atomicAdd(&counters[0], 1u);
                if (slot < RCAP / 2) cand[slot] = ((uint64_t)key << 32) | (uint64_t)(0xFFFFFFFFu - row);
            }
        }
    }
    __syncthreads();
    uint32_t n_cand = counters[0];
    if (all_rows || (floor_mode && n_cand < (uint32_t)pool && (uint32_t)n1 <= RCAP / 2)) {
        __syncthreads();
        if (tid == 0) counters[0] = 0;
        __syncthreads();
        for (int i = tid; i < n1; i += RR_SEL_THREADS) {
            const int64_t at = (int64_t)q * RR_X3_MCAP + (i >> sh);
            const int r = i & ((1 << sh) - 1);
            const uint32_t row = (mtiles[at] << sh) + (uint32_t)r;
            if ((int64_t)row < G.n_rows) {
                const uint32_t key = rr_f2key(sc[(at << sh) + r]);
                const uint32_t slot = atomicAdd(&counters[0], 1u);
                if (slot < RCAP / 2) cand[slot] = ((uint64_t)key << 32) | (uint64_t)(0xFFFFFFFFu - row);
            }
        }
        __syncthreads();
        n_cand = counters[0];
    }
    if (tid == 0) dbg[q * 16 + 3] = (int32_t)n_cand;
    if (n_cand > RCAP / 2 || n_cand < (uint32_t)pool) {
        if (tid == 0) {
            fb[q] = 1;
            dbg[q * 16 + 0] = 0;
        }
        return;
    }
    if (n_cand <= RR_SEL_THREADS) {
        rr_rank_sort_desc(cand, (int)n_cand, cand + RCAP / 2);
        for (int i = tid; i < pool; i += RR_SEL_THREADS) cand[i] = cand[RCAP / 2 + i];
        __syncthreads();
    } else {
        int n_sort = 1;
        while (n_sort < (int)n_cand) n_sort <<= 1;
        for (int i = tid; i < n_sort; i += RR_SEL_THREADS)
            if (i >= (int)n_cand) cand[i] = 0;
        rr_bitonic_desc(cand, n_sort);
    }
    for (int i = tid; i < pool; i += RR_SEL_THREADS) {
        const uint64_t key = cand[i];
        const uint32_t row = 0xFFFFFFFFu - (uint32_t)(key & 0xFFFFFFFFu);
        out_rows[(int64_t)q * pool + i] = (int64_t)row + row_offset;
        out_scores[(int64_t)q * pool + i] = rr_key2f((uint32_t)(key >> 32));
    }
}

rr_x3_scratch rr_x3_scratch_of(const rr_index* ix) {
    rr_x3_scratch s;
    char* p = static_cast<char*>(ix->d_x3);
    s.mtiles = reinterpret_cast<uint32_t*>(p);  p += sizeof(uint32_t) * RR_SEL_MAXQ * RR_X3_MCAP;
    s.count = reinterpret_cast<int32_t*>(p);    p += sizeof(int32_t) * RR_SEL_MAXQ;
    s.tau = reinterpret_cast<uint32_t*>(p);     p += sizeof(uint32_t) * RR_SEL_MAXQ;
    s.fb = reinterpret_cast<int32_t*>(p);       p += sizeof(int32_t) * RR_SEL_MAXQ;
    p += sizeof(float) * RR_SEL_MAXQ;
    s.eps = ix->d_eps;
    s.sc = reinterpret_cast<float*>(p);
    return s;
}
size_t rr_x3_scratch_bytes() {
    return sizeof(uint32_t) * RR_SEL_MAXQ * RR_X3_MCAP + 4 * sizeof(int32_t) * RR_SEL_MAXQ +
           sizeof(float) * (size_t)RR_SEL_MAXQ * RR_X3_MCAP * 16;
}
void rr_launch_select_mtiles(rr_index* ix, const rr_scan_geom& G, int nq, int pool, hipStream_t st, const float* eps,
                             const float* sigma, int nq_b, int64_t mmax_set_stride, int64_t smax_set_stride,
                             const float* floor) {
    const rr_x3_scratch s = rr_x3_scratch_of(ix);
    hipLaunchKernelGGL(rr_select_mtiles, dim3(nq + nq_b), dim3(RR_SEL_THREADS), 0, st, G, ix->d_gmax, ix->d_smax, pool,
                       s.mtiles, s.count, s.tau, s.fb, ix->d_sel_trace, eps, sigma, nq, nq_b, mmax_set_stride,
                       smax_set_stride, floor);
}
void rr_launch_select_rescored(rr_index* ix, const rr_scan_geom& G, int nq, int pool, int64_t* d_rows,
                               float* d_scores, hipStream_t st, bool floor_mode) {
    const rr_x3_scratch s = rr_x3_scratch_of(ix);
    if (pool <= 512)
        hipLaunchKernelGGL((rr_select_rescored<RR_SEL_RCAP>), dim3(nq), dim3(RR_SEL_THREADS), 0, st, G, s.mtiles, s.count, s.tau,
                           s.sc, pool, ix->row_offset, d_rows, d_scores, s.fb, ix->d_sel_trace, floor_mode ? 1 : 0);
    else
        hipLaunchKernelGGL((rr_select_rescored<RR_SEL_CCAP>), dim3(nq), dim3(RR_SEL_THREADS), 0, st, G, s.mtiles, s.count, s.tau,
                           s.sc, pool, ix->row_offset, d_rows, d_scores, s.fb, ix->d_sel_trace, floor_mode ? 1 : 0);
}

__global__ __launch_bounds__(RR_SEL_THREADS) void rr_group_kth(rr_scan_geom G, const uint32_t* __restrict__ smax, int kth,
                                                               const float* __restrict__ eps, float* __restrict__ bound,
                                                               int nq_a, int nq_b, int64_t smax_set_stride) {
    __shared__ uint32_t cnt[2][3][16];
    const int tid = threadIdx.x;
    const int Q = blockIdx.x;
    const int set = (nq_b > 0 && Q >= nq_a) ? 1 : 0;
    const int q = set ? Q - nq_a : Q;
    smax += set * smax_set_stride;
    eps += set * RR_FLT_MAXQ;
    const int QS = G.qs;
    const int gpw = G.gpw > 1 ? G.gpw : 1;
    const int ng = G.n_waves * gpw;
    int phase = 0;
    float out = -INFINITY;
    if (ng > kth && ng <= RR_SEL_RK * RR_SEL_THREADS) {
        uint32_t r[RR_SEL_RK];
        int n_mine = 0;
#pragma unroll
        for (int j = 0; j < RR_SEL_RK; ++j) {
            const int i = tid + j * RR_SEL_THREADS;
            r[j] = i < ng ? smax[(int64_t)i * QS + q] : 0u;
            n_mine += i < ng ? 1 : 0;
        }
        uint32_t tau;
        if (ng <= 1 * RR_SEL_THREADS) tau = rr_kth_largest_reg<1>(r, n_mine, (uint32_t)kth, cnt, phase, 7);
        else if (ng <= 2 * RR_SEL_THREADS) tau = rr_kth_largest_reg<2>(r, n_mine, (uint32_t)kth, cnt, phase, 7);
        else if (ng <= 4 * RR_SEL_THREADS) tau = rr_kth_largest_reg<4>(r, n_mine, (uint32_t)kth, cnt, phase, 7);
        else tau = rr_kth_largest_reg<8>(r, n_mine, (uint32_t)kth, cnt, phase, 7);
        const float e = eps[q];
        if (tau > 0x007FFFFFu && e >= 0.f && e < 3.0e38f) out = rr_key2f(tau) - 1.01f * e;
        if (!(out == out)) out = -INFINITY;
    }
    if (tid == 0) bound[Q] = out;
}
void rr_launch_group_kth(rr_index* ix, const rr_scan_geom& G, int nq_a, int nq_b, int kth, const float* eps, float* d_bound,
                         int64_t smax_set_stride, hipStream_t st) {
    hipLaunchKernelGGL(rr_group_kth, dim3(nq_a + nq_b), dim3(RR_SEL_THREADS), 0, st, G, ix->d_smax, kth, eps, d_bound, nq_a,
                       nq_b, smax_set_stride);
}

__global__ void rr_l2norm_f32(float* __restrict__ mat, int64_t n_rows, int dim_pad, float eps) {
    const int lane = threadIdx.x & 63;
    const int64_t row = (int64_t)blockIdx.x * (blockDim.x >> 6) + (threadIdx.x >> 6);
    if (row >= n_rows) return;
    float* p = mat + row * dim_pad;
    float ss = 0.f;
    for (int i = lane; i < dim_pad; i += 64) ss = __builtin_fmaf(p[i], p[i], ss);
#pragma unroll
    for (int m = 32; m >= 1; m >>= 1) ss += __shfl_xor(ss, m, 64);
    const float nrm = fmaxf(sqrtf(ss), eps);
    for (int i = lane; i < dim_pad; i += 64) p[i] = p[i] / nrm;
}

static int rr_ensure_maxima(rr_index* ix, int nq) {
    const size_t nm = nq >= RR_MFMA_MAXQ ? RR_FLT_MAXQ : nq;
    if (ix->maxima_q >= (int)nm) return RR_OK;
    const int64_t n_tiles = rr_round_up(ix->n_rows, 64) / 64;
    if (ix->d_gmax) hipFree(ix->d_gmax);
    if (ix->d_smax) hipFree(ix->d_smax);
    ix->d_gmax = nullptr;
    ix->d_smax = nullptr;
    ix->maxima_q = 0;
    const size_t groups_cap = (size_t)RR_MAX_SCAN_WAVES;
    const size_t gmax_words = nm * n_tiles * 4 + (size_t)RR_MAX_SCAN_WAVES * RR_FLT_MAXQ;
    RR_HIP_TRY(hipMalloc(&ix->d_gmax, sizeof(float) * gmax_words));
    RR_HIP_TRY(hipMemsetD32Async((hipDeviceptr_t)ix->d_gmax, 0x0000FF80, gmax_words, nullptr));
    RR_HIP_TRY(hipStreamSynchronize(nullptr));
    RR_HIP_TRY(hipMalloc(&ix->d_smax, sizeof(uint32_t) * 2 * nm * groups_cap));
    ix->maxima_q = (int32_t)nm;
    return RR_OK;
}

static int rr_ensure_scratch(rr_index* ix, int nq) {
    const int rc = rr_ensure_maxima(ix, nq);
    if (rc) return rc;
    if (ix->scratch_q >= nq || (ix->scratch_small && ix->scratch_q >= RR_MFMA_MAXQ)) return RR_OK;
    const int64_t n_tiles = rr_round_up(ix->n_rows, 64) / 64;
    if (ix->d_sims) hipFree(ix->d_sims);
    ix->d_sims = nullptr;
    ix->scratch_q = 0;
    static const bool force_small = getenv("RR_SCRATCH_SMALL") != nullptr;
    if ((force_small && nq > RR_MFMA_MAXQ) ||
        hipMalloc(&ix->d_sims, sizeof(float) * (size_t)nq * n_tiles * 64) != hipSuccess) {
        (void)hipGetLastError();
        ix->d_sims = nullptr;
        if (nq <= RR_MFMA_MAXQ) { rr_set_error("rr_dense_topk: out of device memory for the score scratch"); return RR_E_NOMEM; }
        nq = RR_MFMA_MAXQ;
        RR_HIP_TRY(hipMalloc(&ix->d_sims, sizeof(float) * (size_t)nq * n_tiles * 64));
        ix->scratch_small = true;
    }
    ix->scratch_q = nq;
    return RR_OK;
}

static void rr_slot_store(const rr_index* ix, rr_scan_slot& s) {
    s.d_q = ix->d_q; s.d_qplanes = ix->d_qplanes; s.d_eps = ix->d_eps; s.d_gmax = ix->d_gmax; s.d_smax = ix->d_smax;
    s.maxima_q = ix->maxima_q; s.d_flt_samp = ix->d_flt_samp; s.d_flt_sigma = ix->d_flt_sigma; s.d_flt_prog = ix->d_flt_prog;
    s.flt_seq = ix->flt_seq; s.flt_prep_fresh = ix->flt_prep_fresh; s.flt_pending = ix->flt_pending;
}
static void rr_slot_fetch(rr_index* ix, const rr_scan_slot& s) {
    ix->d_q = s.d_q; ix->d_qplanes = s.d_qplanes; ix->d_eps = s.d_eps; ix->d_gmax = s.d_gmax; ix->d_smax = s.d_smax;
    ix->maxima_q = s.maxima_q; ix->d_flt_samp = s.d_flt_samp; ix->d_flt_sigma = s.d_flt_sigma; ix->d_flt_prog = s.d_flt_prog;
    ix->flt_seq = s.flt_seq; ix->flt_prep_fresh = s.flt_prep_fresh; ix->flt_pending = s.flt_pending;
}
void rr_slot_park(rr_index* ix) {
    rr_slot_store(ix, ix->parked[ix->cur_slot]);
    rr_slot_fetch(ix, rr_scan_slot());
}
int rr_slot_activate(rr_index* ix, int slot) {
    RR_REQUIRE(slot >= 0 && slot < RR_SCAN_SLOTS, "scan slot %d outside [0, %d)", slot, RR_SCAN_SLOTS);
    if (slot != ix->cur_slot) {
        rr_slot_store(ix, ix->parked[ix->cur_slot]);
        rr_slot_fetch(ix, ix->parked[slot]);
        ix->parked[slot] = rr_scan_slot();
        ix->cur_slot = slot;
    }
    if (!ix->d_q) {
        RR_HIP_TRY(hipSetDevice(ix->device));
        RR_HIP_TRY(hipMalloc(&ix->d_qplanes, (size_t)2 * 3 * 64 * 384 * 2));
        RR_HIP_TRY(hipMalloc((void**)&ix->d_eps, sizeof(float) * RR_SEL_MAXQ));
        RR_HIP_TRY(hipMalloc((void**)&ix->d_q, sizeof(float) * (size_t)RR_MAX_BATCH * ix->dim_pad));
    }
    return RR_OK;
}

template <typename K>
static int rr_resident_grid(K kernel, int device) {
    int per_cu = 0, cus = 0;
    if (hipOccupancyMaxActiveBlocksPerMultiprocessor(&per_cu, kernel, RR_SCAN_THREADS, 0) != hipSuccess ||
        per_cu < 1)
        per_cu = 2;
    if (hipDeviceGetAttribute(&cus, hipDeviceAttributeMultiprocessorCount, device) != hipSuccess || cus < 1)
        cus = 256;
    int grid = per_cu * cus;
    if (grid * (RR_SCAN_THREADS / 64) > RR_MAX_SCAN_WAVES) grid = RR_MAX_SCAN_WAVES / (RR_SCAN_THREADS / 64);
    return grid;
}

rr_scan_geom rr_make_geom(const rr_index* ix, int resident_blocks) {
    rr_scan_geom G;
    G.n_rows = ix->n_rows;
    G.n_tiles = rr_round_up(ix->n_rows, 64) / 64;
    G.n_pad = G.n_tiles * 64;
    int64_t max_waves = (int64_t)resident_blocks * (RR_SCAN_THREADS / 64);
    if (ix->scan_cus > 0 && ix->n_cus > 0) {
        max_waves = max_waves * ix->scan_cus / ix->n_cus;
        if (max_waves < 1) max_waves = 1;
    }
    G.tiles_per_wave = (G.n_tiles + max_waves - 1) / max_waves;
    G.n_waves = (int32_t)((G.n_tiles + G.tiles_per_wave - 1) / G.tiles_per_wave);
    G.qs = 0;
    G.mm_pairs = 0;
    G.gpw = 1;
    G.tiles_per_group = G.tiles_per_wave;
    return G;
}

int rr_scan_events_begin(rr_index* ix, hipStream_t st) {
    const int slot = (int)(ix->ring_head % rr_index::kRing);
    hipEventRecord(ix->ring0[slot], st);
    return slot;
}
void rr_scan_events_end(rr_index* ix, int slot, hipStream_t st) {
    hipEventRecord(ix->ring1[slot], st);
    ix->ring_head++;
    if (ix->ring_head - ix->ring_tail > rr_index::kRing) ix->ring_tail = ix->ring_head - rr_index::kRing;
}
void rr_launch_select(rr_index* ix, const rr_scan_geom& G, int nq, int pool, int64_t* d_rows,
                      float* d_scores, hipStream_t st, const int32_t* only_if, int slices, int64_t sims_slice,
                      int64_t gmax_slice, int64_t smax_slice) {
    const dim3 grid(slices > 1 ? RR_MFMA_MAXQ : nq, slices > 1 ? slices : 1);
    hipLaunchKernelGGL(rr_select, grid, dim3(RR_SEL_THREADS), 0, st, G, ix->d_sims, ix->d_gmax,
                       ix->d_smax, pool, ix->row_offset, d_rows, d_scores, ix->d_sel_trace, only_if, nq, sims_slice,
                       gmax_slice, smax_slice, (const int32_t*)nullptr, (int32_t*)nullptr);
}
int rr_resident_waves(const void* kernel, int threads, int device) {
    int per_cu = 0, cus = 0;
    if (hipOccupancyMaxActiveBlocksPerMultiprocessor(&per_cu, kernel, threads, 0) != hipSuccess || per_cu < 1)
        per_cu = 1;
    if (hipDeviceGetAttribute(&cus, hipDeviceAttributeMultiprocessorCount, device) != hipSuccess || cus < 1)
        cus = 256;
    int waves = per_cu * cus * (threads / 64);
    return waves > RR_MAX_SCAN_WAVES ? RR_MAX_SCAN_WAVES : waves;
}

template <int NB>
static rr_scan_geom rr_launch_scan(rr_index* ix, const float* d_q, hipStream_t st) {
    const f32x4* mat = reinterpret_cast<const f32x4*>(ix->d_matrix);
    const int nf = ix->dim_pad / 64;
    static int cap6 = 0, capg = 0;
    rr_scan_geom G;
    if (nf == 6) {
        if (!cap6) cap6 = rr_resident_grid(rr_scan_f32<6, NB>, ix->device);
        G = rr_make_geom(ix, cap6);
        const int grid = (G.n_waves + 3) / 4;
        hipLaunchKernelGGL((rr_scan_f32<6, NB>), dim3(grid), dim3(RR_SCAN_THREADS), 0, st, mat, G, d_q,
                           ix->d_sims, ix->d_gmax, ix->d_smax, (const int32_t*)nullptr, 0, (int32_t*)nullptr);
    } else {
        if (!capg) capg = rr_resident_grid(rr_scan_f32_generic<NB>, ix->device);
        G = rr_make_geom(ix, capg);
        const int grid = (G.n_waves + 3) / 4;
        hipLaunchKernelGGL((rr_scan_f32_generic<NB>), dim3(grid), dim3(RR_SCAN_THREADS), 0, st, mat, G, nf,
                           d_q, ix->d_sims, ix->d_gmax, ix->d_smax);
    }
    return G;
}

int rr_dense_listed_fallback(rr_index* ix, const float* d_q, int nq, int pool, int64_t* d_rows, float* d_scores,
                             int32_t* flags, hipStream_t st) {
    static const bool off = getenv("RR_NO_CHAIN_FALLBACK") != nullptr;
    if (off || ix->dtype != RR_DTYPE_F32 || ix->dim_pad != 384 || !ix->d_flag_list) return RR_OK;
    static int cap = 0;
    if (!cap) cap = rr_resident_grid(rr_scan_f32<6, 8, true>, ix->device);
    rr_scan_geom G = rr_make_geom(ix, cap);
    hipLaunchKernelGGL((rr_scan_f32<6, 8, true>), dim3((G.n_waves + 3) / 4), dim3(RR_SCAN_THREADS), 0, st,
                       reinterpret_cast<const f32x4*>(ix->d_matrix), G, d_q, ix->d_sims, ix->d_gmax, ix->d_smax,
                       (const int32_t*)flags, nq, ix->d_flag_list);
    hipLaunchKernelGGL(rr_select, dim3(8), dim3(RR_SEL_THREADS), 0, st, G, ix->d_sims, ix->d_gmax, ix->d_smax, pool,
                       ix->row_offset, d_rows, d_scores, ix->d_sel_trace, (const int32_t*)nullptr, 8, (int64_t)0, (int64_t)0,
                       (int64_t)0, (const int32_t*)ix->d_flag_list, flags);
    RR_HIP_TRY(hipGetLastError());
    return RR_OK;
}

static int rr_dense_chunk(rr_index* ix, const float* d_q, int nq, int pool, int64_t* d_rows,
                          float* d_scores, hipStream_t st, bool time_it) {
    if (time_it) hipEventRecord(ix->ev0, st);
    const int slot = (int)(ix->ring_head % rr_index::kRing);
    hipEventRecord(ix->ring0[slot], st);
    rr_scan_note(ix, 1, nq <= 1 ? 1 : nq <= 2 ? 2 : nq <= 4 ? 4 : 8, nq, 0);
    rr_scan_geom G;
    switch (nq) {
        case 1: G = rr_launch_scan<1>(ix, d_q, st); break;
        case 2: G = rr_launch_scan<2>(ix, d_q, st); break;
        case 3: case 4: G = rr_launch_scan<4>(ix, d_q, st); break;
        default: G = rr_launch_scan<8>(ix, d_q, st); break;
    }
    hipEventRecord(ix->ring1[slot], st);
    ix->ring_head++;
    if (ix->ring_head - ix->ring_tail > rr_index::kRing) ix->ring_tail = ix->ring_head - rr_index::kRing;
    if (time_it) {
        hipEventRecord(ix->ev1, st);
        ix->timing_valid = true;
    }
    hipLaunchKernelGGL(rr_select, dim3(nq), dim3(RR_SEL_THREADS), 0, st, G, ix->d_sims, ix->d_gmax,
                       ix->d_smax, pool, ix->row_offset, d_rows, d_scores, ix->d_sel_trace, (const int32_t*)nullptr, nq, (int64_t)0, (int64_t)0, (int64_t)0,
                       (const int32_t*)nullptr, (int32_t*)nullptr);
    RR_HIP_TRY(hipGetLastError());
    return RR_OK;
}

template <int NQT>
static int rr_dense_chunk_mfma(rr_index* ix, const float* d_q, int nq, int pool, int64_t* d_rows,
                               float* d_scores, hipStream_t st) {
    constexpr int THREADS = NQT == 4 ? 512 : 256;
    static int cap_waves = 0;
    if (!cap_waves) {
        int per_cu = 0, cus = 0;
        if (hipOccupancyMaxActiveBlocksPerMultiprocessor(&per_cu, rr_scan_mfma_f32<NQT>, THREADS, 0) != hipSuccess ||
            per_cu < 1)
            per_cu = 1;
        if (hipDeviceGetAttribute(&cus, hipDeviceAttributeMultiprocessorCount, ix->device) != hipSuccess || cus < 1)
            cus = 256;
        cap_waves = per_cu * cus * (THREADS / 64);
        if (cap_waves > RR_MAX_SCAN_WAVES) cap_waves = RR_MAX_SCAN_WAVES;
    }
    rr_scan_geom G = rr_make_geom(ix, cap_waves / 4);
    G.qs = 16 * NQT;
    const int slot = (int)(ix->ring_head % rr_index::kRing);
    hipEventRecord(ix->ring0[slot], st);
    rr_scan_note(ix, 6, NQT, nq, 0);
    hipLaunchKernelGGL((rr_scan_mfma_f32<NQT>), dim3((G.n_waves + THREADS / 64 - 1) / (THREADS / 64)), dim3(THREADS), 0, st,
                       reinterpret_cast<const f32x4*>(ix->d_matrix), G, d_q, ix->d_sims, ix->d_gmax, ix->d_smax);
    hipEventRecord(ix->ring1[slot], st);
    ix->ring_head++;
    if (ix->ring_head - ix->ring_tail > rr_index::kRing) ix->ring_tail = ix->ring_head - rr_index::kRing;
    hipLaunchKernelGGL(rr_select, dim3(nq), dim3(RR_SEL_THREADS), 0, st, G, ix->d_sims, ix->d_gmax,
                       ix->d_smax, pool, ix->row_offset, d_rows, d_scores, ix->d_sel_trace, (const int32_t*)nullptr, nq, (int64_t)0, (int64_t)0, (int64_t)0,
                       (const int32_t*)nullptr, (int32_t*)nullptr);
    RR_HIP_TRY(hipGetLastError());
    return RR_OK;
}

static int rr_scratch_enter(rr_index* ix, hipStream_t st, bool scan = true, bool select = true) {
    (void)scan;
    const int s = ix->cur_slot;
    if (ix->slot_has[s] && ix->slot_stream[s] != st) RR_HIP_TRY(hipStreamWaitEvent(st, ix->slot_ev[s], 0));
    if (select && ix->has_done && st != ix->last_stream) RR_HIP_TRY(hipStreamWaitEvent(st, ix->ev_done, 0));
    return RR_OK;
}
static int rr_scratch_leave(rr_index* ix, hipStream_t st, bool scan = true, bool select = true) {
    (void)scan;
    const int s = ix->cur_slot;
    RR_HIP_TRY(hipEventRecord(ix->slot_ev[s], st));
    ix->slot_stream[s] = st;
    ix->slot_has[s] = true;
    if (select) {
        RR_HIP_TRY(hipEventRecord(ix->ev_done, st));
        ix->last_stream = st;
        ix->has_done = true;
    }
    return RR_OK;
}

static int rr_dense_topk_impl(rr_index* ix, const float* d_q_padded, int nq, int pool,
                              int64_t* d_rows, float* d_scores, hipStream_t st) {
    RR_HIP_TRY(hipSetDevice(ix->device));
    const bool bf16 = ix->dtype == RR_DTYPE_BF16;
    const bool mfma_ok = ix->dim_pad == 384 && ix->n_rows >= 64;
    static const bool f32_chain = getenv("RR_SCAN_F32_CHAIN") != nullptr;
    static const bool exact_scan = getenv("RR_SCAN_EXACT") != nullptr;
    const int valu_max = mfma_ok ? 4 : 8;
    const int scratch_slots = (int)rr_round_up(nq < RR_SEL_MAXQ ? nq : RR_SEL_MAXQ, RR_MFMA_MAXQ);
    int rc = rr_ensure_scratch(ix, (mfma_ok && nq > valu_max) ? scratch_slots : 8);
    if (rc) return rc;
    int q0 = 0;
    while (q0 < nq) {
        const int left = nq - q0;
        const float* q = d_q_padded + (int64_t)q0 * ix->dim_pad;
        int64_t* rows = d_rows + (int64_t)q0 * pool;
        float* scores = d_scores + (int64_t)q0 * pool;
        int n;
        bool small = false;
        if (mfma_ok && left > valu_max && !f32_chain && !exact_scan && ix->scan_mode == RR_SCAN_MODE_DEFAULT &&
            (ix->n_rows + 63) / 64 < 8 * (int64_t)pool)
            small = true;
        if (mfma_ok && left > valu_max && !small) {
            n = left < RR_MFMA_MAXQ ? left : RR_MFMA_MAXQ;
            bool done = false;
            if (!f32_chain && !exact_scan && ix->scan_mode == RR_SCAN_MODE_DEFAULT) {
                static const bool no_pair = getenv("RR_NO_PAIR") != nullptr;
                int nf = left < RR_FLT_MAXQ ? left : RR_FLT_MAXQ;
                if (!no_pair && left > RR_FLT_MAXQ + RR_MFMA_MAXQ) nf = left < RR_SEL_MAXQ ? left : RR_SEL_MAXQ;
                rc = rr_dense_chunk_flt(ix, q, nf, pool, rows, scores, st);
                if (rc != RR_FLT_NO_BOUND && rc != RR_FLT_SMALL) {
                    done = true;
                    n = nf;
                }
            }
            if (done) {
            } else if (!f32_chain) rc = rr_dense_chunk_x3(ix, q, n, pool, rows, scores, st);
            else if (bf16) rc = rr_dense_chunk_mfma_bf16(ix, q, n, pool, rows, scores, st);
            else if (n <= 16) rc = rr_dense_chunk_mfma<1>(ix, q, n, pool, rows, scores, st);
            else if (n <= 32) rc = rr_dense_chunk_mfma<2>(ix, q, n, pool, rows, scores, st);
            else rc = rr_dense_chunk_mfma<4>(ix, q, n, pool, rows, scores, st);
        } else {
            const int vmax = small ? 8 : valu_max;
            n = left < vmax ? left : vmax;
            rc = bf16 ? rr_dense_chunk_bf16(ix, q, n, pool, rows, scores, st)
                      : rr_dense_chunk(ix, q, n, pool, rows, scores, st, q0 == 0);
        }
        if (rc) return rc;
        q0 += n;
    }
    return RR_OK;
}

__global__ void rr_pad_queries(const float* __restrict__ src, float* __restrict__ dst, int nq,
                               int dim, int dim_pad, int slots) {
    const int64_t i = (int64_t)blockIdx.x * blockDim.x + threadIdx.x;
    if (i >= (int64_t)slots * dim_pad) return;
    const int qi = (int)(i / dim_pad), c = (int)(i % dim_pad);
    dst[i] = (qi < nq && c < dim) ? src[(int64_t)qi * dim + c] : 0.f;
}

extern "C" int rr_dense_scan_slot_dev(rr_index* ix, int32_t slot, const float* d_queries, int32_t n_queries, int32_t pool,
                                      int32_t kth, float* d_bound, int32_t* applied, void* stream) {
    RR_REQUIRE(ix && d_queries && applied, "rr_dense_scan_dev: NULL argument");
    RR_REQUIRE(n_queries >= 1 && n_queries <= RR_MAX_BATCH, "rr_dense_scan_dev: n_queries %d out of [1,%d]", n_queries, RR_MAX_BATCH);
    RR_REQUIRE(pool >= 1 && pool <= RR_MAX_POOL && pool <= ix->n_rows, "rr_dense_scan_dev: pool %d out of range", pool);
    RR_REQUIRE(kth >= 0 && kth <= pool && (kth == 0) == (d_bound == nullptr),
               "rr_dense_scan_dev: kth %d out of [1, pool] (or 0 with a NULL bound: no bound wanted)", kth);
    RR_REQUIRE(ix->d_matrix, "rr_dense_scan_dev: index has no matrix");
    *applied = 0;
    std::lock_guard<std::mutex> lk(ix->mu);
    RR_HIP_TRY(hipSetDevice(ix->device));
    static const bool exact_scan = getenv("RR_SCAN_EXACT") != nullptr, f32_chain = getenv("RR_SCAN_F32_CHAIN") != nullptr;
    const bool mfma_ok = ix->dim_pad == 384 && ix->n_rows >= 64;
    if (!mfma_ok || n_queries <= 4 || n_queries > RR_SEL_MAXQ || exact_scan || f32_chain || ix->scan_mode != RR_SCAN_MODE_DEFAULT ||
        (n_queries > RR_FLT_MAXQ && n_queries <= RR_FLT_MAXQ + RR_MFMA_MAXQ))
        return RR_OK;
    hipStream_t st = (hipStream_t)stream;
    const void* q_vis = nullptr;
    int rc = rr_device_visible(d_queries, &q_vis, "rr_dense_scan_dev (queries)");
    if (rc) return rc;
    d_queries = static_cast<const float*>(q_vis);
    rc = rr_slot_activate(ix, slot);
    if (rc) return rc;
    rc = rr_scratch_enter(ix, st, true, false);
    if (rc) return rc;
    rc = rr_ensure_scratch(ix, (int)rr_round_up(n_queries, RR_MFMA_MAXQ));
    if (rc) return rc;
    const int slots = (int)rr_round_up(n_queries, RR_MFMA_MAXQ);
    const int64_t total = (int64_t)slots * ix->dim_pad;
    if (rr_flt_pad_prep(ix, d_queries, n_queries, slots, st) != RR_OK)
        hipLaunchKernelGGL(rr_pad_queries, dim3((unsigned)((total + 255) / 256)), dim3(256), 0, st,
                           d_queries, ix->d_q, n_queries, ix->dim, ix->dim_pad, slots);
    rc = rr_dense_chunk_flt(ix, ix->d_q, n_queries, pool, nullptr, nullptr, st, 1, kth, d_bound, nullptr);
    if (rc == RR_FLT_NO_BOUND || rc == RR_FLT_SMALL) return rr_scratch_leave(ix, st, true, false);
    if (rc) return rc;
    *applied = 1;
    return rr_scratch_leave(ix, st, true, false);
}

extern "C" int rr_dense_select_part_dev(rr_index* ix, int32_t slot, int32_t parts, int32_t n_queries, int32_t pool,
                                        const float* d_floor, int64_t* d_out_rows, float* d_out_scores, void* stream) {
    RR_REQUIRE(ix, "rr_dense_select_dev: NULL handle");
    RR_REQUIRE(parts >= 1 && parts <= 7, "rr_dense_select_dev: parts %d is not a combination of RR_SELECT_LIST | _RESCORE | _ORDER", parts);
    RR_REQUIRE(!(parts & 4) || (d_out_rows && d_out_scores), "rr_dense_select_dev: NULL output");
    std::lock_guard<std::mutex> lk(ix->mu);
    RR_HIP_TRY(hipSetDevice(ix->device));
    hipStream_t st = (hipStream_t)stream;
    int rc = rr_slot_activate(ix, slot);
    if (rc) return rc;
    rc = rr_scratch_enter(ix, st, false, true);
    if (rc) return rc;
    rc = rr_dense_chunk_flt(ix, ix->d_q, n_queries, pool, d_out_rows, d_out_scores, st, 2, 0, nullptr, d_floor, parts);
    RR_REQUIRE(rc != RR_FLT_SMALL, "rr_dense_select_dev: no scan of these %d queries (pool %d) is pending in slot %d: call "
               "rr_dense_scan_dev first and use its `applied` answer", n_queries, pool, slot);
    if (rc) return rc;
    return rr_scratch_leave(ix, st, false, true);
}

extern "C" int rr_dense_select_slot_dev(rr_index* ix, int32_t slot, int32_t n_queries, int32_t pool, const float* d_floor,
                                        int64_t* d_out_rows, float* d_out_scores, void* stream) {
    return rr_dense_select_part_dev(ix, slot, 7, n_queries, pool, d_floor, d_out_rows, d_out_scores, stream);
}

extern "C" int rr_dense_scan_dev(rr_index* ix, const float* d_queries, int32_t n_queries, int32_t pool, int32_t kth,
                                 float* d_bound, int32_t* applied, void* stream) {
    RR_REQUIRE(kth >= 1 && d_bound, "rr_dense_scan_dev: kth %d out of [1, pool] / NULL bound", kth);
    return rr_dense_scan_slot_dev(ix, 0, d_queries, n_queries, pool, kth, d_bound, applied, stream);
}

extern "C" int rr_dense_select_dev(rr_index* ix, const float* d_queries, int32_t n_queries, int32_t pool,
                                   const float* d_floor, int64_t* d_out_rows, float* d_out_scores, void* stream) {
    RR_REQUIRE(d_queries, "rr_dense_select_dev: NULL argument");
    return rr_dense_select_slot_dev(ix, 0, n_queries, pool, d_floor, d_out_rows, d_out_scores, stream);
}

extern "C" int rr_dense_topk_slot_dev(rr_index* ix, int32_t slot, const float* d_queries, int32_t n_queries,
                                      int32_t pool, int64_t* d_out_rows, float* d_out_scores,
                                      void* stream) {
    RR_REQUIRE(ix && d_queries && d_out_rows && d_out_scores, "rr_dense_topk_dev: NULL argument");
    RR_REQUIRE(n_queries >= 1 && n_queries <= RR_MAX_BATCH, "rr_dense_topk_dev: n_queries %d out of [1,%d]",
               n_queries, RR_MAX_BATCH);
    RR_REQUIRE(pool >= 1 && pool <= RR_MAX_POOL && pool <= ix->n_rows,
               "rr_dense_topk_dev: pool %d out of [1,min(%d,n_rows=%lld)]", pool, RR_MAX_POOL,
               (long long)ix->n_rows);
    RR_REQUIRE(ix->d_matrix, "rr_dense_topk_dev: index has no matrix");
    RR_REQUIRE(ix->dtype == RR_DTYPE_F32 || ix->dim_pad == 384,
               "rr_dense_topk_dev: bf16 storage is built for dim 384 only");
    std::lock_guard<std::mutex> lk(ix->mu);
    RR_HIP_TRY(hipSetDevice(ix->device));
    hipStream_t st = (hipStream_t)stream;
    int rc0 = rr_slot_activate(ix, slot);
    if (rc0) return rc0;
    rr_flt_drop_pending(ix);
    const void* q_vis = nullptr;
    int rc = rr_device_visible(d_queries, &q_vis, "rr_dense_topk_dev (queries)");
    if (rc) return rc;
    d_queries = static_cast<const float*>(q_vis);
    rc = rr_scratch_enter(ix, st);
    if (rc) return rc;
    const int slots = (int)rr_round_up(n_queries, RR_MFMA_MAXQ);
    const int64_t total = (int64_t)slots * ix->dim_pad;
    static const bool plain_front = getenv("RR_SCAN_EXACT") != nullptr || getenv("RR_SCAN_F32_CHAIN") != nullptr;
    const bool filter_call = ix->dim_pad == 384 && ix->n_rows >= 64 && n_queries > 4 && n_queries <= RR_SEL_MAXQ && !plain_front &&
                             ix->scan_mode == RR_SCAN_MODE_DEFAULT && (ix->n_rows + 63) / 64 >= 8 * (int64_t)pool;
    if (!filter_call || rr_flt_pad_prep(ix, d_queries, n_queries, slots, st) != RR_OK)
        hipLaunchKernelGGL(rr_pad_queries, dim3((unsigned)((total + 255) / 256)), dim3(256), 0, st,
                           d_queries, ix->d_q, n_queries, ix->dim, ix->dim_pad, slots);
    rc = rr_dense_topk_impl(ix, ix->d_q, n_queries, pool, d_out_rows, d_out_scores, st);
    ix->flt_prep_fresh = false;
    if (rc) return rc;
    return rr_scratch_leave(ix, st);
}

extern "C" int rr_dense_topk_dev(rr_index* ix, const float* d_queries, int32_t n_queries,
                                 int32_t pool, int64_t* d_out_rows, float* d_out_scores,
                                 void* stream) {
    return rr_dense_topk_slot_dev(ix, 0, d_queries, n_queries, pool, d_out_rows, d_out_scores, stream);
}

extern "C" int rr_dense_topk(rr_index* ix, const float* h_queries, int32_t n_queries, int32_t pool,
                             int64_t* h_out_rows, float* h_out_scores, int32_t* pool_out) {
    RR_REQUIRE(ix && h_queries && pool_out, "rr_dense_topk: NULL argument");
    RR_REQUIRE(n_queries >= 1 && n_queries <= RR_MAX_BATCH, "rr_dense_topk: n_queries %d out of [1,%d]",
               n_queries, RR_MAX_BATCH);
    RR_REQUIRE(pool >= 0, "rr_dense_topk: negative pool");
    int eff = pool;
    if ((int64_t)eff > ix->n_rows) eff = (int)ix->n_rows;
    RR_REQUIRE(eff <= RR_MAX_POOL, "rr_dense_topk: pool %d exceeds RR_MAX_POOL %d", eff, RR_MAX_POOL);
    *pool_out = eff;
    if (eff == 0) return RR_OK;
    RR_REQUIRE(h_out_rows && h_out_scores, "rr_dense_topk: NULL output");
    RR_REQUIRE(ix->d_matrix, "rr_dense_topk: index has no matrix");
    RR_REQUIRE(ix->dtype == RR_DTYPE_F32 || ix->dim_pad == 384,
               "rr_dense_topk: bf16 storage is built for dim 384 only");
    std::lock_guard<std::mutex> lk(ix->mu);
    RR_HIP_TRY(hipSetDevice(ix->device));
    hipStream_t st = nullptr;
    int rce = rr_slot_activate(ix, 0);
    if (rce) return rce;
    rce = rr_scratch_enter(ix, st);
    if (rce) return rce;
    const int slots = (int)rr_round_up(n_queries, RR_MFMA_MAXQ);
    RR_HIP_TRY(hipMemsetAsync(ix->d_q, 0, sizeof(float) * (size_t)slots * ix->dim_pad, st));
    RR_HIP_TRY(hipMemcpy2DAsync(ix->d_q, sizeof(float) * ix->dim_pad, h_queries,
                                sizeof(float) * ix->dim, sizeof(float) * ix->dim, n_queries,
                                hipMemcpyHostToDevice, st));
    int rc = rr_dense_topk_impl(ix, ix->d_q, n_queries, eff, ix->d_rows_out, ix->d_scores_out, st);
    if (rc) return rc;
    RR_HIP_TRY(hipMemcpyAsync(h_out_rows, ix->d_rows_out, sizeof(int64_t) * (size_t)n_queries * eff,
                              hipMemcpyDeviceToHost, st));
    RR_HIP_TRY(hipMemcpyAsync(h_out_scores, ix->d_scores_out, sizeof(float) * (size_t)n_queries * eff,
                              hipMemcpyDeviceToHost, st));
    RR_HIP_TRY(hipStreamSynchronize(st));
    return rr_scratch_leave(ix, st);
}

extern "C" int rr_index_last_scan_ms(rr_index* ix, float* out_ms) {
    RR_REQUIRE(ix && out_ms, "rr_index_last_scan_ms: NULL argument");
    std::lock_guard<std::mutex> lk(ix->mu);
    RR_REQUIRE(ix->timing_valid, "rr_index_last_scan_ms: no scan has been timed yet");
    RR_HIP_TRY(hipSetDevice(ix->device));
    RR_HIP_TRY(hipEventSynchronize(ix->ev1));
    RR_HIP_TRY(hipEventElapsedTime(out_ms, ix->ev0, ix->ev1));
    return RR_OK;
}

extern "C" int rr_index_last_scan_info(rr_index* ix, int32_t* out8) {
    RR_REQUIRE(ix && out8, "rr_index_last_scan_info: NULL argument");
    std::lock_guard<std::mutex> lk(ix->mu);
    for (int i = 0; i < 8; ++i) out8[i] = i < 5 ? ix->last_scan[i] : 0;
    return RR_OK;
}

extern "C" int rr_index_set_shadow(rr_index* ix, int32_t enable) {
    RR_REQUIRE(ix != nullptr, "null index");
    std::lock_guard<std::mutex> lk(ix->mu);
    ix->use_shadow = enable ? 1 : 0;
    if (!enable && ix->d_shadow) {
        RR_HIP_TRY(hipSetDevice(ix->device));
        RR_HIP_TRY(hipDeviceSynchronize());
        hipFree(ix->d_shadow);
        ix->d_shadow = nullptr;
        ix->shadow_valid = false;
    }
    return RR_OK;
}

extern "C" int rr_index_set_scan_mode(rr_index* ix, int32_t mode) {
    RR_REQUIRE(ix != nullptr, "null index");
    RR_REQUIRE(mode == RR_SCAN_MODE_DEFAULT || mode == RR_SCAN_MODE_STORED, "unknown scan mode %d", mode);
    ix->scan_mode = mode;
    return RR_OK;
}

extern "C" int rr_index_select_trace(rr_index* ix, int32_t* out4) {
    RR_REQUIRE(ix && out4, "rr_index_select_trace: NULL argument");
    std::lock_guard<std::mutex> lk(ix->mu);
    RR_HIP_TRY(hipSetDevice(ix->device));
    RR_HIP_TRY(hipDeviceSynchronize());
    RR_HIP_TRY(hipMemcpy(out4, ix->d_sel_trace, sizeof(int32_t) * 16, hipMemcpyDeviceToHost));
    return RR_OK;
}

extern "C" int rr_index_scan_stats(rr_index* ix, double* out_total_ms, int64_t* out_launches) {
    RR_REQUIRE(ix && out_total_ms && out_launches, "rr_index_scan_stats: NULL argument");
    std::lock_guard<std::mutex> lk(ix->mu);
    RR_HIP_TRY(hipSetDevice(ix->device));
    double total = 0.0;
    int64_t n = 0;
    for (; ix->ring_tail < ix->ring_head; ++ix->ring_tail) {
        const int slot = (int)(ix->ring_tail % rr_index::kRing);
        RR_HIP_TRY(hipEventSynchronize(ix->ring1[slot]));
        float ms = 0.f;
        RR_HIP_TRY(hipEventElapsedTime(&ms, ix->ring0[slot], ix->ring1[slot]));
        total += ms;
        ++n;
    }
    *out_total_ms = total;
    *out_launches = n;
    return RR_OK;
}

int rr_l2norm_rows_f32_at(float* d_rows, int32_t dim_pad, int64_t n, float eps, hipStream_t st) {
    if (n == 0) return RR_OK;
    hipLaunchKernelGGL(rr_l2norm_f32, dim3((unsigned)((n + 3) / 4)), dim3(256), 0, st, d_rows, n, dim_pad, eps);
    RR_HIP_TRY(hipGetLastError());
    return RR_OK;
}

int rr_l2norm_rows_f32(rr_index* ix, int64_t first_row, int64_t n, float eps, hipStream_t st) {
    return rr_l2norm_rows_f32_at((float*)ix->d_matrix + first_row * ix->dim_pad, ix->dim_pad, n, eps, st);
}

extern "C" int rr_index_l2_normalize(rr_index* ix, float eps) {
    RR_REQUIRE(ix && ix->d_matrix, "rr_index_l2_normalize: index has no matrix");
    RR_REQUIRE(ix->dtype == RR_DTYPE_F32,
               "rr_index_l2_normalize: a bf16 index is normalised in fp32 before rounding (rr_index_upload_rows_f32)");
    std::lock_guard<std::mutex> lk(ix->mu);
    RR_HIP_TRY(hipSetDevice(ix->device));
    rr_matrix_written(ix);
    const int rows_per_block = 4;
    const unsigned grid = (unsigned)((ix->n_rows + rows_per_block - 1) / rows_per_block);
    hipLaunchKernelGGL(rr_l2norm_f32, dim3(grid), dim3(64 * rows_per_block), 0, ix->stream,
                       (float*)ix->d_matrix, ix->n_rows, ix->dim_pad, eps);
    RR_HIP_TRY(hipGetLastError());
    RR_HIP_TRY(hipStreamSynchronize(ix->stream));
    return RR_OK;
}
```

review-recommender_amd/csrc/rr_dense_flt.hip:

```cpp
#include "rr_x3.h"

typedef float f32x16 __attribute__((ext_vector_type(16)));
typedef __bf16 bf16x2 __attribute__((ext_vector_type(2)));
typedef unsigned int u32x2 __attribute__((ext_vector_type(2)));

#define RR_FLT_QSTRIDE 49

struct rr_flt_bounds {
    float row_norm;
    float row_delta;
};
__global__ __launch_bounds__(64) void rr_flt_prep_queries(const float* __restrict__ q, unsigned short* __restrict__ plane,
                                                          float* __restrict__ eps, rr_flt_bounds B) {
    const int slot = blockIdx.x, lane = threadIdx.x;
    const float* src = q + (int64_t)slot * 384;
    float ss = 0.f, sr = 0.f, sd = 0.f;
#pragma unroll
    for (int i = 0; i < 6; ++i) {
        const int pos = lane + 64 * i;
        const float x = src[pos];
        const __bf16 r = (__bf16)x;
        const float xr = (float)r, d = x - xr;
        ss = __builtin_fmaf(x, x, ss);
        sr = __builtin_fmaf(xr, xr, sr);
// ... 1038 lines not shown
            hipLaunchKernelGGL((rr_row_norm_max<true>), dim3(blocks), dim3(256), 0, st, ix->d_matrix, ix->n_rows, ix->dim_pad, d);
        else
            hipLaunchKernelGGL((rr_row_norm_max<false>), dim3(blocks), dim3(256), 0, st, ix->d_matrix, ix->n_rows, ix->dim_pad, d);
        unsigned int bits[2] = {0u, 0u};
        RR_HIP_TRY(hipMemcpyAsync(bits, d, sizeof(bits), hipMemcpyDeviceToHost, st));
        RR_HIP_TRY(hipStreamSynchronize(st));
        float nb[2];
        memcpy(nb, bits, sizeof(nb));
        ix->norm_bound = nb[0] * 1.0001f;
        ix->delta_bound = nb[1] * 1.0001f;
    }
    out->row_norm = ix->norm_bound;
    out->row_delta = ix->delta_bound;
    return RR_OK;
}

template <int NQ2, bool A_BF16>
static rr_scan_geom rr_flt_geom(rr_index* ix, bool dual = false) {
    constexpr int THREADS = RR_FLT_THREADS(NQ2);
    static int waves = 0;
    if (!waves) waves = A_BF16 ? rr_resident_waves((const void*)rr_scan_flt16<NQ2>, 512, ix->device)
                               : rr_resident_waves((const void*)rr_scan_flt<NQ2>, THREADS, ix->device);
    rr_scan_geom G = rr_make_geom(ix, dual ? waves / 8 : waves / 4);
    G.qs = 32 * NQ2;
    G.mm_pairs = 3;
    const int gcap = dual ? 8 : 4;
    G.gpw = RR_MAX_SCAN_WAVES / G.n_waves < gcap ? (RR_MAX_SCAN_WAVES / G.n_waves < 1 ? 1 : RR_MAX_SCAN_WAVES / G.n_waves) : gcap;
    if (G.gpw > G.tiles_per_wave) G.gpw = (int32_t)G.tiles_per_wave;
    G.tiles_per_group = (G.tiles_per_wave + G.gpw - 1) / G.gpw;
    G.gpw = (int32_t)((G.tiles_per_wave + G.tiles_per_group - 1) / G.tiles_per_group);
    return G;
}

static rr_scan_geom rr_fltq_geom(rr_index* ix) {
    static int runs = 0;
    if (!runs) runs = rr_resident_waves((const void*)rr_scan_fltq<true>, 256, ix->device) / 4;
    rr_scan_geom G = rr_make_geom(ix, runs / 4);
    G.qs = RR_FLT_MAXQ;
    G.mm_pairs = 3;
    G.gpw = RR_MAX_SCAN_WAVES / G.n_waves < 32 ? (RR_MAX_SCAN_WAVES / G.n_waves < 1 ? 1 : RR_MAX_SCAN_WAVES / G.n_waves) : 32;
    if (G.gpw > G.tiles_per_wave) G.gpw = (int32_t)G.tiles_per_wave;
    G.tiles_per_group = (G.tiles_per_wave + G.gpw - 1) / G.gpw;
    if (G.tiles_per_group < 8 && (int64_t)G.n_waves * ((G.tiles_per_wave + 7) / 8) > 2048) G.tiles_per_group = 8;
    G.tiles_per_group += G.tiles_per_group & 1;
    G.gpw = (int32_t)((G.tiles_per_wave + G.tiles_per_group - 1) / G.tiles_per_group);
    return G;
}

__global__ __launch_bounds__(256) void rr_shadow_from_f32(const f32x4* __restrict__ src, u32x2* __restrict__ dst, int64_t n4) {
    const int64_t i = (int64_t)blockIdx.x * 256 + threadIdx.x;
    if (i >= n4) return;
    const f32x4 x = __builtin_nontemporal_load(src + i);
    const bf16x2 lo = bf16x2{(__bf16)x.x, (__bf16)x.y}, hi = bf16x2{(__bf16)x.z, (__bf16)x.w};
    dst[i] = u32x2{__builtin_bit_cast(unsigned int, lo), __builtin_bit_cast(unsigned int, hi)};
}

static int rr_flt_ensure_shadow(rr_index* ix, hipStream_t st) {
    if (ix->shadow_valid) return RR_OK;
    const size_t bytes = (size_t)ix->n_rows * 384 * 2;
    if (!ix->d_shadow) {
        const hipError_t e = hipMalloc((void**)&ix->d_shadow, bytes);
        if (e != hipSuccess) {
            (void)hipGetLastError();
            ix->use_shadow = 0;
            return RR_OK;
        }
    }
    const int64_t n4 = ix->n_rows * 96;
    hipLaunchKernelGGL(rr_shadow_from_f32, dim3((unsigned)((n4 + 255) / 256)), dim3(256), 0, st,
                       reinterpret_cast<const f32x4*>(ix->d_matrix), reinterpret_cast<u32x2*>(ix->d_shadow), n4);
    RR_HIP_TRY(hipGetLastError());
    ix->shadow_valid = true;
    return RR_OK;
}

static int rr_flt_tune() {
    static const int t = getenv("RR_FLT_TUNE") ? atoi(getenv("RR_FLT_TUNE")) : 0;
    return t;
}

static int64_t rr_flt_mmax_set_stride(const rr_scan_geom& G) { return (int64_t)2 * G.n_tiles * RR_FLT_MAXQ; }
static int64_t rr_flt_smax_set_stride() { return (int64_t)RR_FLT_MAXQ * RR_MAX_SCAN_WAVES; }

template <int NQ2, bool SCAN_BF16>
static int rr_flt_scan_set(rr_index* ix, int set, const rr_scan_geom& G, const void* scan_mat, const float* d_q, int nq,
                           int pool, rr_flt_bounds bounds, hipStream_t st, const float** sigma_out,
                           bool launch_scan = true, bool allow_prefilter = true, int prep_sets = 1) {
    constexpr int THREADS = RR_FLT_THREADS(NQ2);
    constexpr int QN = 32 * NQ2;
    unsigned short* plane = reinterpret_cast<unsigned short*>(ix->d_qplanes) + (size_t)set * RR_FLT_MAXQ * 384;
    const rr_x3_scratch X = rr_x3_scratch_of(ix);
    float* eps = X.eps + set * RR_FLT_MAXQ;
    float* gmax = ix->d_gmax + set * rr_flt_mmax_set_stride(G);
    uint32_t* smax = ix->d_smax + set * rr_flt_smax_set_stride();
    if (prep_sets && !ix->flt_prep_fresh)
        hipLaunchKernelGGL(rr_flt_prep_queries, dim3(QN * prep_sets), dim3(64), 0, st, d_q, plane, eps, bounds);
    const dim3 grid((G.n_waves + THREADS / 64 - 1) / (THREADS / 64)), block(THREADS);
    const float* sigma = nullptr;
    uint32_t* dummy = nullptr;
    static const bool no_prefilter = getenv("RR_NO_PREFILTER") != nullptr;
    const int64_t n_tiles32 = (G.n_rows + 31) / 32;
    if (SCAN_BF16 && !no_prefilter && allow_prefilter && G.n_rows >= 2000000) {
        const int stride = 64;
        int64_t n_samp = (n_tiles32 - 1) / stride;
        if (n_samp > RR_FLT_SAMP_CAP) n_samp = RR_FLT_SAMP_CAP;
        const int m = 16 + (4 * pool + stride - 1) / stride;
        if (!ix->d_flt_samp) {
            RR_HIP_TRY(hipMalloc((void**)&ix->d_flt_samp, sizeof(float) * (size_t)RR_FLT_SAMP_CAP * RR_FLT_MAXQ));
            RR_HIP_TRY(hipMalloc((void**)&ix->d_flt_sigma, sizeof(float) * 2 * RR_FLT_MAXQ));
        }
        float* sg = ix->d_flt_sigma + set * RR_FLT_MAXQ;
        hipLaunchKernelGGL((rr_flt_sample<NQ2>), dim3(256), dim3(512), 0, st, reinterpret_cast<const u32x4*>(scan_mat),
                           reinterpret_cast<const u32x4*>(plane), stride, (int)n_samp, ix->d_flt_samp);
        static const int force = getenv("RR_FLT_SIGMA_FORCE") ? atoi(getenv("RR_FLT_SIGMA_FORCE")) : 0;
        hipLaunchKernelGGL(rr_flt_sigma, dim3(QN), dim3(256), 0, st, ix->d_flt_samp, (int)n_samp, QN, nq, m, eps, sg, force);
        sigma = sg;
        dummy = reinterpret_cast<uint32_t*>(ix->d_gmax) + (size_t)4 * G.n_tiles * RR_FLT_MAXQ;
    }
    *sigma_out = sigma ? ix->d_flt_sigma : nullptr;
    if (!launch_scan) {
        RR_HIP_TRY(hipGetLastError());
        return RR_OK;
    }
    const int slot = rr_scan_events_begin(ix, st);
    rr_scan_note(ix, 5, NQ2, nq, 1, SCAN_BF16 ? 2 : 4);
    if (SCAN_BF16)
        hipLaunchKernelGGL((rr_scan_flt16<NQ2>), grid, block, 0, st, reinterpret_cast<const u32x4*>(scan_mat), G,
                           reinterpret_cast<const u32x4*>(plane), gmax, smax, eps, nq, sigma, dummy, 0, (int64_t)0,
                           (uint32_t*)nullptr, 0u, rr_flt_tune());
    else
        hipLaunchKernelGGL((rr_scan_flt<NQ2>), grid, block, 0, st, reinterpret_cast<const u32x4*>(scan_mat), G,
                           reinterpret_cast<const u32x4*>(plane), gmax, smax, eps, nq, sigma, dummy);
    rr_scan_events_end(ix, slot, st);
    RR_HIP_TRY(hipGetLastError());
    return RR_OK;
}

template <bool ROWS_BF16>
static int rr_flt_finish(rr_index* ix, const rr_scan_geom& G, const float* d_q, int nq_a, int nq_b, int pool,
                         int64_t* d_rows, float* d_scores, const float* sigma, hipStream_t st, const float* floor = nullptr,
                         int parts = 7) {
    const rr_x3_scratch X = rr_x3_scratch_of(ix);
    const int nq = nq_a + nq_b;
    if (parts & 1)
        rr_launch_select_mtiles(ix, G, nq_a, pool, st, X.eps, sigma, nq_b, rr_flt_mmax_set_stride(G), rr_flt_smax_set_stride(), floor);
    static const bool no_pre = getenv("RR_NO_RESCORE_PLANE") != nullptr;
    const u32x4* plane_rows = (!ROWS_BF16 && ix->shadow_valid && ix->d_shadow && !no_pre)
                                  ? reinterpret_cast<const u32x4*>(ix->d_shadow) : nullptr;
    if (parts & 2)
        hipLaunchKernelGGL((rr_rescore_chain<ROWS_BF16>), dim3(floor ? 4 : 16, nq), dim3(256), 0, st, ix->d_matrix, G.n_rows, d_q,
                           X.mtiles, X.count, X.fb, X.sc, plane_rows, X.tau, X.eps);
    RR_HIP_TRY(hipGetLastError());
    if (!(parts & 4)) return RR_OK;
    rr_launch_select_rescored(ix, G, nq, pool, d_rows, d_scores, st, floor != nullptr);
    RR_HIP_TRY(hipGetLastError());
    if (!ROWS_BF16) {
        const int rc = rr_dense_listed_fallback(ix, d_q, nq, pool, d_rows, d_scores, X.fb, st);
        if (rc != RR_OK) return rc;
    }
    return rr_dense_x3w_fallback_all(ix, d_q, nq, pool, d_rows, d_scores, X.fb, st);
}

struct rr_flt_pending {
    bool valid;
    rr_scan_geom G;
    const float* d_q;
    int nq_a, nq_b, pool;
    const float* sigma;
    bool rows_bf16;
};
struct rr_flt_phase {
    int phase = 0;
    int kth = 0;
    float* d_bound = nullptr;
    const float* d_floor = nullptr;
};
static rr_flt_pending* rr_flt_pending_of(rr_index* ix) {
    if (!ix->flt_pending) ix->flt_pending = calloc(1, sizeof(rr_flt_pending));
    return static_cast<rr_flt_pending*>(ix->flt_pending);
}
void rr_flt_drop_pending(rr_index* ix) {
    if (ix->flt_pending) static_cast<rr_flt_pending*>(ix->flt_pending)->valid = false;
}
template <bool ROWS_BF16>
static int rr_flt_after_scan(rr_index* ix, const rr_scan_geom& G, const float* d_q, int nq_a, int nq_b, int pool,
                             int64_t* d_rows, float* d_scores, const float* sigma, hipStream_t st, const rr_flt_phase& ph) {
    if (ph.phase != 1) return rr_flt_finish<ROWS_BF16>(ix, G, d_q, nq_a, nq_b, pool, d_rows, d_scores, sigma, st);
    rr_flt_pending* p = rr_flt_pending_of(ix);
    if (!p) return RR_E_HIP;
    *p = rr_flt_pending{true, G, d_q, nq_a, nq_b, pool, sigma, ROWS_BF16};
    if (ph.kth > 0 && ph.d_bound)
        rr_launch_group_kth(ix, G, nq_a, nq_b, ph.kth, rr_x3_scratch_of(ix).eps, ph.d_bound, rr_flt_smax_set_stride(), st);
    RR_HIP_TRY(hipGetLastError());
    return RR_OK;
}

template <int NQ2, bool SCAN_BF16, bool ROWS_BF16>
static int rr_dense_chunk_flt_t(rr_index* ix, const void* scan_mat, const float* d_q, int nq, int pool, int64_t* d_rows,
                                float* d_scores, rr_flt_bounds bounds, hipStream_t st, const rr_flt_phase& ph = rr_flt_phase()) {
    const rr_scan_geom G = rr_flt_geom<NQ2, SCAN_BF16>(ix);
    const float* sigma = nullptr;
    const int rc = rr_flt_scan_set<NQ2, SCAN_BF16>(ix, 0, G, scan_mat, d_q, nq, pool, bounds, st, &sigma);
    if (rc != RR_OK) return rc;
    return rr_flt_after_scan<ROWS_BF16>(ix, G, d_q, nq, 0, pool, d_rows, d_scores, sigma, st, ph);
}

static int rr_flt_launch_fltq(rr_index* ix, const rr_scan_geom& G, const void* scan_mat, int nq_a, int nq_b, bool noasm, hipStream_t st) {
    const rr_x3_scratch X = rr_x3_scratch_of(ix);
    const int slot = rr_scan_events_begin(ix, st);
    rr_scan_note(ix, 5, 9, nq_a + nq_b, 1, 2);
    if (noasm)
        hipLaunchKernelGGL((rr_scan_fltq<false>), dim3(G.n_waves), dim3(256), 0, st, reinterpret_cast<const u32x4*>(scan_mat), G,
                           reinterpret_cast<const u32x4*>(ix->d_qplanes), ix->d_gmax, ix->d_smax, X.eps, nq_a, nq_b,
                           rr_flt_mmax_set_stride(G), (unsigned long long*)nullptr);
    else
        hipLaunchKernelGGL((rr_scan_fltq<true>), dim3(G.n_waves), dim3(256), 0, st, reinterpret_cast<const u32x4*>(scan_mat), G,
                           reinterpret_cast<const u32x4*>(ix->d_qplanes), ix->d_gmax, ix->d_smax, X.eps, nq_a, nq_b,
                           rr_flt_mmax_set_stride(G), (unsigned long long*)nullptr);
    rr_scan_events_end(ix, slot, st);
    RR_HIP_TRY(hipGetLastError());
    return RR_OK;
}
static int rr_flt_launch_dual(rr_index* ix, const rr_scan_geom& G, const void* scan_mat, int nq_a, int nq_b, const float* sg0, hipStream_t st) {
    constexpr int THREADS = RR_FLT_THREADS(4);
    const int nb = (G.n_waves + THREADS / 64 - 1) / (THREADS / 64);
    const dim3 grid(((nb + 7) / 8) * 16), block(THREADS);
    const rr_x3_scratch X = rr_x3_scratch_of(ix);
    uint32_t* dummy = sg0 ? reinterpret_cast<uint32_t*>(ix->d_gmax) + (size_t)4 * G.n_tiles * RR_FLT_MAXQ : nullptr;
    const int slot = rr_scan_events_begin(ix, st);
    rr_scan_note(ix, 5, 8, nq_a + nq_b, 1, 2);
    static const bool no_couple = getenv("RR_NO_COUPLE") != nullptr;
    if (!ix->d_flt_prog) {
        RR_HIP_TRY(hipMalloc((void**)&ix->d_flt_prog, sizeof(uint32_t) * 2 * RR_MAX_SCAN_WAVES));
        RR_HIP_TRY(hipMemsetAsync(ix->d_flt_prog, 0, sizeof(uint32_t) * 2 * RR_MAX_SCAN_WAVES, st));
    }
    ix->flt_seq = (ix->flt_seq + 1) & 0x7FFFu;
    hipLaunchKernelGGL((rr_scan_flt16<4, 0, true>), grid, block, 0, st, reinterpret_cast<const u32x4*>(scan_mat), G,
                       reinterpret_cast<const u32x4*>(ix->d_qplanes), ix->d_gmax, ix->d_smax, X.eps, nq_a, sg0, dummy,
                       nq_b, rr_flt_mmax_set_stride(G), no_couple ? (uint32_t*)nullptr : ix->d_flt_prog,
                       (uint32_t)(ix->flt_seq + 1) << 16, rr_flt_tune());
    rr_scan_events_end(ix, slot, st);
    RR_HIP_TRY(hipGetLastError());
    return RR_OK;
}

template <bool SCAN_BF16, bool ROWS_BF16>
static int rr_dense_pair_flt_t(rr_index* ix, const void* scan_mat, const float* d_q, int nq_a, int nq_b, int pool,
                               int64_t* d_rows, float* d_scores, rr_flt_bounds bounds, hipStream_t st,
                               const rr_flt_phase& ph = rr_flt_phase()) {
    static const bool no_dual = getenv("RR_NO_DUAL") != nullptr;
    const bool dual = SCAN_BF16 && !no_dual;
    static const bool use_q = getenv("RR_NO_FLTQ") == nullptr;
    const bool fltq = dual && use_q;
    const rr_scan_geom G = fltq ? rr_fltq_geom(ix) : rr_flt_geom<4, SCAN_BF16>(ix, dual);
    const float *sg0 = nullptr, *sg1 = nullptr;
    static const bool dual_prefilter = getenv("RR_DUAL_PREFILTER") != nullptr;
    const bool pre = !dual || dual_prefilter;
    const bool prep_both = dual && !pre && nq_a == RR_FLT_MAXQ;
    int rc = rr_flt_scan_set<4, SCAN_BF16>(ix, 0, G, scan_mat, d_q, nq_a, pool, bounds, st, &sg0, !dual, pre, prep_both ? 2 : 1);
    if (rc != RR_OK) return rc;
    rc = rr_flt_scan_set<4, SCAN_BF16>(ix, 1, G, scan_mat, d_q + (int64_t)nq_a * ix->dim_pad, nq_b, pool, bounds, st, &sg1, !dual, pre,
                                       prep_both ? 0 : 1);
    if (rc != RR_OK) return rc;
    if (fltq) {
        static const bool noasm = getenv("RR_FLTQ_NOASM") != nullptr;
        rc = rr_flt_launch_fltq(ix, G, scan_mat, nq_a, nq_b, noasm, st);
        if (rc != RR_OK) return rc;
    } else if (dual) {
        rc = rr_flt_launch_dual(ix, G, scan_mat, nq_a, nq_b, sg0, st);
        if (rc != RR_OK) return rc;
    }
    return rr_flt_after_scan<ROWS_BF16>(ix, G, d_q, nq_a, nq_b, pool, d_rows, d_scores, sg0, st, ph);
}

int rr_flt_pad_prep(rr_index* ix, const float* d_queries, int nq, int slots, hipStream_t st) {
    ix->flt_prep_fresh = false;
    rr_flt_bounds nb;
    const int rc = rr_flt_get_bounds(ix, st, &nb);
    if (rc != RR_OK) return rc;
    if (!(nb.row_norm < 3.0e18f) || slots > RR_SEL_MAXQ || ix->dim_pad != 384) return RR_FLT_NO_BOUND;
    const rr_x3_scratch X = rr_x3_scratch_of(ix);
    hipLaunchKernelGGL(rr_flt_pad_prep_queries, dim3(slots), dim3(64), 0, st, d_queries, nq, ix->dim, ix->d_q,
                       reinterpret_cast<unsigned short*>(ix->d_qplanes), X.eps, nb);
    RR_HIP_TRY(hipGetLastError());
    ix->flt_prep_fresh = true;
    return RR_OK;
}

struct rr_flt_fresh_guard {
    rr_index* ix;
    ~rr_flt_fresh_guard() { ix->flt_prep_fresh = false; }
};

int rr_dense_chunk_flt(rr_index* ix, const float* d_q, int nq, int pool, int64_t* d_rows,
                       float* d_scores, hipStream_t st, int phase, int kth, float* d_bound, const float* d_floor, int parts) {
    rr_flt_fresh_guard fresh_guard{ix};
    if (d_q != ix->d_q) ix->flt_prep_fresh = false;
    if (phase == 2) {
        rr_flt_pending* p = rr_flt_pending_of(ix);
        if (!p || !p->valid || p->nq_a + p->nq_b != nq || p->pool != pool || p->d_q != d_q) return RR_FLT_SMALL;
        if (parts & 4) p->valid = false;
        return p->rows_bf16 ? rr_flt_finish<true>(ix, p->G, d_q, p->nq_a, p->nq_b, pool, d_rows, d_scores, p->sigma, st, d_floor, parts)
                            : rr_flt_finish<false>(ix, p->G, d_q, p->nq_a, p->nq_b, pool, d_rows, d_scores, p->sigma, st, d_floor, parts);
    }
    rr_flt_phase ph;
    ph.phase = phase;
    ph.kth = kth;
    ph.d_bound = d_bound;
// ... 365 lines not shown
```

review-recommender_amd/engine.py:

```python
from __future__ import annotations

import ctypes as C
import os
import threading
from dataclasses import dataclass
from typing import Callable, Dict, List, Optional, Sequence, Tuple

import numpy as np
import pandas as pd

from . import _lib, text
from .bm25 import BM25Corpus, BM25Index, build_bm25_index_ids, factorize_corpus
from .index import MAX_POOL, ProductIndex

APP_POOL_FLOOR = 150
CLI_POOL_FLOOR = 100
APP_TRUST_SAT = 80
COLUMN_NAMES = ("_dense", "_bm25", "_prior", "_rerank", "_best", "_gate", "_trust", "_final")
_FLOAT32_COLUMNS = {"_dense", "_bm25", "_best", "_gate", "_trust", "_final"}


@dataclass
class FusionWeights:
    w_dense: float = 0.55
# ... 26 lines not shown
    def topk_column(self, name: str) -> np.ndarray:
        c = self.columns[:, COLUMN_NAMES.index(name), :]
        return np.take_along_axis(c, self.order.astype(np.int64), axis=1)


def _torch():
    import torch
    return torch


_KERNEL_COPIES = os.environ.get("RR_NO_KERNEL_COPY") is None


class StagedTerms:
    __slots__ = ("ids", "off", "slot", "n_ids")

    def __init__(self, ids, off, slot, n_ids):
        self.ids, self.off, self.slot, self.n_ids = ids, off, slot, int(n_ids)


class StagedBatch:
    __slots__ = ("q", "terms", "ready", "slot")

    def __init__(self, q, terms, ready, slot):
        self.q, self.terms, self.ready, self.slot = q, terms, ready, slot


class HybridSearcher:

    def __init__(self, index: ProductIndex, bm25: Optional[BM25Index] = None):
        if not index.has_meta:
            raise ValueError("the index needs metadata (ProductIndex.set_meta) before searching")
        self.index, self.bm25 = index, bm25
        self.lib = _lib.load()
        torch = _torch()
        if not torch.cuda.is_available():
            raise _lib.HipLibraryError("no GPU visible: the search path runs on the device only")
        self.device = torch.device("cuda", index.device)
        self._stage_slots = [{"host": None, "dev": None, "event": None, "consumed": None} for _ in range(8)]
        self._stage_next = 0
        self._q_slots = [{"dev": None, "free": None} for _ in range(4)]
        self._q_next = 0
        self._in = None
        self._ring_lock = threading.RLock()

    def _stream(self):
        return C.c_void_p(_torch().cuda.current_stream(self.device).cuda_stream)

    def copy_segments(self, pairs) -> None:
        segs = (_lib.CopySeg * len(pairs))()
        for i, (dst, src) in enumerate(pairs):
            if dst.shape != src.shape or dst.dtype != src.dtype:
                raise ValueError("copy_segments: shape / dtype mismatch")
            for t in (dst, src):
                if not t.is_cuda and not t.is_pinned():
                    raise ValueError("copy_segments: host tensors must be pinned")
            esz = dst.element_size()
            if dst.is_contiguous() and src.is_contiguous():
                rows, row_bytes, dp, sp = 1, dst.numel() * esz, dst.numel() * esz, dst.numel() * esz
            else:
                if dst.dim() != 2 or dst.stride(1) != 1 or src.stride(1) != 1:
                    raise ValueError("copy_segments: tensors must be contiguous or 2-D with contiguous rows")
                rows, row_bytes = dst.shape[0], dst.shape[1] * esz
                dp, sp = dst.stride(0) * esz, src.stride(0) * esz
            segs[i] = _lib.CopySeg(dst.data_ptr(), src.data_ptr(), row_bytes, rows, dp, sp)
        _lib.check(self.lib.rr_copy_segments_dev(segs, len(pairs), self.device.index, self._stream()), "rr_copy_segments_dev")

    def dense_pool(self, q_dev, pool: int, out=None, slot: int = 0):
        torch = _torch()
        B = q_dev.shape[0]
        if out is not None:
            rows, dense = out
        else:
            rows = torch.empty((B, pool), dtype=torch.int64, device=self.device)
            dense = torch.empty((B, pool), dtype=torch.float32, device=self.device)
        _lib.check(self.lib.rr_dense_topk_slot_dev(self.index.handle, int(slot), C.c_void_p(q_dev.data_ptr()), B, pool,
                                                   C.c_void_p(rows.data_ptr()), C.c_void_p(dense.data_ptr()),
                                                   self._stream()), "rr_dense_topk_dev")
        return rows, dense

    def dense_scan(self, q_dev, pool: int, kth: int):
        torch = _torch()
        B = q_dev.shape[0]
        bound = torch.empty((B,), dtype=torch.float32, device=self.device)
        applied = C.c_int32(0)
        _lib.check(self.lib.rr_dense_scan_dev(self.index.handle, C.c_void_p(q_dev.data_ptr()), B, pool, int(kth),
                                              C.c_void_p(bound.data_ptr()), C.byref(applied), self._stream()),
                   "rr_dense_scan_dev")
        return bound if applied.value else None

    def dense_select(self, q_dev, pool: int, floor, out=None):
        torch = _torch()
        B = q_dev.shape[0]
        if out is not None:
            rows, dense = out
        else:
            rows = torch.empty((B, pool), dtype=torch.int64, device=self.device)
            dense = torch.empty((B, pool), dtype=torch.float32, device=self.device)
        _lib.check(self.lib.rr_dense_select_dev(self.index.handle, C.c_void_p(q_dev.data_ptr()), B, pool,
                                                C.c_void_p(floor.data_ptr()), C.c_void_p(rows.data_ptr()),
                                                C.c_void_p(dense.data_ptr()), self._stream()), "rr_dense_select_dev")
        return rows, dense

    def dense_scan_slot(self, slot: int, q_dev, pool: int, kth: int = 0, bound_out=None):
        torch = _torch()
        B = q_dev.shape[0]
        bound = None
        if kth > 0:
            bound = bound_out if bound_out is not None else torch.empty((B,), dtype=torch.float32, device=self.device)
        applied = C.c_int32(0)
        _lib.check(self.lib.rr_dense_scan_slot_dev(self.index.handle, int(slot), C.c_void_p(q_dev.data_ptr()), B, pool, int(kth),
                                                   C.c_void_p(bound.data_ptr()) if kth > 0 else None, C.byref(applied),
                                                   self._stream()), "rr_dense_scan_slot_dev")
        if not applied.value:
            return None
        return bound if kth > 0 else True

    SELECT_LIST, SELECT_RESCORE, SELECT_ORDER = 1, 2, 4

    def dense_select_slot(self, slot: int, B: int, pool: int, floor=None, out=None, parts: int = 7):
        torch = _torch()
        rows = dense = None
        if parts & self.SELECT_ORDER:
            if out is not None:
                rows, dense = out
            else:
                rows = torch.empty((B, pool), dtype=torch.int64, device=self.device)
                dense = torch.empty((B, pool), dtype=torch.float32, device=self.device)
        p = lambda t: C.c_void_p(t.data_ptr()) if t is not None else None
        _lib.check(self.lib.rr_dense_select_part_dev(self.index.handle, int(slot), int(parts), B, pool, p(floor), p(rows), p(dense),
                                                     self._stream()), "rr_dense_select_part_dev")
        return (rows, dense) if parts & self.SELECT_ORDER else None

    def bm25_at(self, term_id_lists: Sequence[Sequence[int]], rows_dev, mode: str = "forward", out=None):
        torch = _torch()
        B, pool = rows_dev.shape
        staged = isinstance(term_id_lists, StagedTerms)
        flat_form = isinstance(term_id_lists, tuple) and len(term_id_lists) == 2 and isinstance(term_id_lists[1], np.ndarray)
        empty = (term_id_lists.n_ids == 0) if staged else \
            (len(term_id_lists[0]) == 0) if flat_form else not any(len(t) for t in term_id_lists)
        if self.bm25 is None or empty:
            if out is None:
                return torch.zeros((B, pool), dtype=torch.float32, device=self.device)
            out.zero_()
            return out
        if out is None:
            out = torch.empty((B, pool), dtype=torch.float32, device=self.device)
        ids_dev, off_dev = (term_id_lists.ids, term_id_lists.off) if staged else self._stage_terms(term_id_lists)[:2]
        _lib.check(self.lib.rr_bm25_scores_at_dev(
            self.bm25.handle, C.c_void_p(ids_dev.data_ptr()), C.c_void_p(off_dev.data_ptr()), B,
            C.c_void_p(rows_dev.data_ptr()), pool, {"forward": 0, "postings": 1}[mode],
            C.c_void_p(out.data_ptr()), self._stream()), "rr_bm25_scores_at_dev")
        return out

    def _stage_terms(self, term_id_lists):
        torch = _torch()
        if isinstance(term_id_lists, tuple) and len(term_id_lists) == 2 and isinstance(term_id_lists[1], np.ndarray):
            flat = np.ascontiguousarray(term_id_lists[0], dtype=np.int32).reshape(-1)
            off = np.ascontiguousarray(term_id_lists[1], dtype=np.int32).reshape(-1)
        else:
            B = len(term_id_lists)
            off = np.zeros(B + 1, dtype=np.int32)
            np.cumsum([len(t) for t in term_id_lists], out=off[1:])
            flat = (np.concatenate([np.asarray(t, dtype=np.int32).reshape(-1) for t in term_id_lists])
                    if off[-1] else np.zeros(0, dtype=np.int32))
        n_off, n_ids = off.shape[0], flat.shape[0]
        need = n_off + max(n_ids, 1)
        with self._ring_lock:
            return self._stage_terms_locked(off, flat, n_off, n_ids, need)

    def _stage_terms_locked(self, off, flat, n_off, n_ids, need):
        torch = _torch()
        slot = self._stage_slots[self._stage_next % len(self._stage_slots)]
        self._stage_next += 1
        if slot["host"] is None or slot["host"].numel() < need:
            cap = max(2 * need, 16384)
            torch.cuda.synchronize(self.device)
            for sl in self._stage_slots:
                if sl["host"] is None or sl["host"].numel() < need:
                    if sl["event"] is not None:
                        sl["event"].synchronize()
                    sl["host"] = torch.empty(cap, dtype=torch.int32).pin_memory()
                    sl["dev"] = torch.empty(cap, dtype=torch.int32, device=self.device)
                    sl["event"] = torch.cuda.Event()
        else:
            slot["event"].synchronize()
        h = slot["host"].numpy()
        h[:n_off] = off
        h[n_off:n_off + n_ids] = flat
        cur = torch.cuda.current_stream(self.device)
        if slot["consumed"] is not None:
            cur.wait_event(slot["consumed"])
            slot["consumed"] = None
        if _KERNEL_COPIES:
            self.copy_segments([(slot["dev"][:need], slot["host"][:need])])
        else:
            slot["dev"][:need].copy_(slot["host"][:need], non_blocking=True)
        slot["event"].record(cur)
        return slot["dev"][n_off:n_off + max(n_ids, 1)], slot["dev"][:n_off], slot, n_ids

    def stage_batch(self, q_host, term_id_lists=None) -> "StagedBatch":
        torch = _torch()
        with self._ring_lock:
            return self._stage_batch_locked(q_host, term_id_lists)

    def _stage_batch_locked(self, q_host, term_id_lists):
        torch = _torch()
        if self._in is None:
            self._in = torch.cuda.Stream(device=self.device)
        slot = self._q_slots[self._q_next % len(self._q_slots)]
        self._q_next += 1
        if slot["dev"] is None or slot["dev"].shape != q_host.shape:
            slot["dev"] = torch.empty(tuple(q_host.shape), dtype=torch.float32, device=self.device)
            slot["free"] = torch.cuda.Event()
            slot["free"].record(torch.cuda.current_stream(self.device))
        with torch.cuda.stream(self._in):
            if slot["free"] is not None:
                self._in.wait_event(slot["free"])
            slot["dev"].copy_(q_host, non_blocking=True)
            terms = None
            if term_id_lists is not None:
                ids, off, tslot, n_ids = self._stage_terms(term_id_lists)
                terms = StagedTerms(ids, off, tslot, n_ids)
            ready = torch.cuda.Event()
            ready.record(self._in)
        return StagedBatch(slot["dev"], terms, ready, slot)

    def release(self, batch: "StagedBatch") -> None:
        torch = _torch()
        ev = torch.cuda.Event()
        ev.record(torch.cuda.current_stream(self.device))
        batch.slot["free"] = ev
        if batch.terms is not None:
            batch.terms.slot["consumed"] = ev

    def fuse(self, params: "_lib.FuseParams", B: int, rows, dense, bm25, meta=None,
             rerank=None, best=None, gate=None):
        torch = _torch()
        pool, k = params.pool, params.k
        out_rows = torch.empty((B, pool), dtype=torch.int64, device=self.device)
        cols = torch.empty((B, 8, pool), dtype=torch.float64, device=self.device)
        order = torch.empty((B, k), dtype=torch.int32, device=self.device)
        p = lambda t: C.c_void_p(t.data_ptr()) if t is not None else None
        n, avg, l1p = meta if meta is not None else (None, None, None)
        _lib.check(self.lib.rr_fuse_topk_dev(
            self.index.handle, C.byref(params), B, p(rows), p(dense), p(bm25), p(n), p(avg), p(l1p),
            p(rerank), p(best), p(gate), p(out_rows), p(cols), p(order), self._stream()),
            "rr_fuse_topk_dev")
        return out_rows, cols, order

    @staticmethod
    def make_params(w: FusionWeights, k: int, pool: int, n_candidates: int, rerank_k: int,
                    cand_per_rank: int = 0, stride_bytes: int = 0, bm25_f64: bool = False) -> "_lib.FuseParams":
        return _lib.FuseParams(
            w_dense=w.w_dense, w_bm25=w.w_bm25, w_rerank=w.w_rerank, w_prior=w.w_prior,
            w_best=w.w_best, prior_C=w.prior_C, min_reviews=int(w.min_reviews),
            trust_sat=int(w.trust_sat), apply_trust=int(bool(w.apply_trust)),
            rerank_active=int(rerank_k > 0), rerank_k=int(rerank_k), k=int(k),
            n_candidates=int(n_candidates), pool=int(pool), cand_per_rank=int(cand_per_rank),
            bm25_f64=int(bool(bm25_f64)), cand_rank_stride_bytes=int(stride_bytes))

    def search_batch(self, qvecs: np.ndarray, term_id_lists: Optional[Sequence[Sequence[int]]],
                     k: int, rerank_k: int = 0, weights: Optional[FusionWeights] = None,
                     pool_floor: int = APP_POOL_FLOOR,
                     gate_fn: Optional[Callable[[np.ndarray], np.ndarray]] = None,
                     rerank_fn: Optional[Callable[[np.ndarray], np.ndarray]] = None,
                     bm25_mode: str = "forward", reviews=None, max_scan: int = 0,
                     bm25_f64: bool = False) -> BatchResult:
        torch = _torch()
        w = weights or FusionWeights()
        q = np.ascontiguousarray(qvecs, dtype=np.float32)
        if q.ndim != 2 or q.shape[1] != self.index.dim:
            raise ValueError(f"qvecs must be (B, {self.index.dim}); got {q.shape}")
        B = q.shape[0]
        if k < 1:
            raise ValueError("k must be >= 1")
        pool = min(max(k, rerank_k, pool_floor), self.index.n_rows)
        if pool > MAX_POOL:
            raise ValueError(f"pool {pool} exceeds the kernels' limit {MAX_POOL}")
        k_eff = min(k, pool)
        rr_k = min(rerank_k, pool)
        with torch.cuda.device(self.device):
            q_dev = torch.from_numpy(q).to(self.device)
            rows, dense = self.dense_pool(q_dev, pool)
            tl = term_id_lists if term_id_lists is not None else [[] for _ in range(B)]
            bm = self.bm25_at(tl, rows, bm25_mode)
            gate = rerank = best = None
            best_ids = None
            rows_h = None
            if reviews is not None:
                best = torch.empty((B, pool), dtype=torch.float32, device=self.device)
                best_ids = torch.empty((B, pool), dtype=torch.int32, device=self.device)
                _lib.check(self.lib.rr_reviews_best_cut_dev(
                    reviews.handle, C.c_void_p(q_dev.data_ptr()), B, C.c_void_p(rows.data_ptr()), pool,
                    self.index.row_offset, int(max_scan), C.c_void_p(best.data_ptr()),
                    C.c_void_p(best_ids.data_ptr()), self._stream()), "rr_reviews_best_cut_dev")
            if gate_fn is not None or (rerank_fn is not None and rr_k > 0):
                rows_h = rows.cpu().numpy() if rows_h is None else rows_h
                if gate_fn is not None:
                    g = np.ascontiguousarray(gate_fn(rows_h), dtype=np.float32)
                    gate = torch.from_numpy(g).to(self.device)
                if rerank_fn is not None and rr_k > 0:
                    r = np.zeros((B, pool), dtype=np.float32)
                    r[:, :rr_k] = np.asarray(rerank_fn(rows_h[:, :rr_k]), dtype=np.float32)
                    rerank = torch.from_numpy(r).to(self.device)
            params = self.make_params(w, k_eff, pool, pool, rr_k, bm25_f64=bm25_f64 and self.bm25 is None)
# ... 213 lines not shown
```

review-recommender_amd/sharded.py:

```python
from __future__ import annotations

import ctypes as C
import os
from dataclasses import dataclass
from typing import Optional, Sequence, Tuple

import numpy as np

from . import _lib
from .engine import FusionWeights, HybridSearcher
from .index import MAX_CANDIDATES


def shard_bounds(n_rows: int, world: int, rank: int) -> Tuple[int, int]:
    if not (0 <= rank < world):
        raise ValueError("rank outside [0, world)")
    base, extra = divmod(n_rows, world)
    lo = rank * base + min(rank, extra)
    return lo, lo + base + (1 if rank < extra else 0)


@dataclass(frozen=True)
class PayloadLayout:
    n_queries: int
# ... 127 lines not shown
        dist.all_gather([out[r * share:(r + 1) * share] for r in range(world)], buf, group=group)
    parts = []
    for r in range(world):
        lo, hi = split_pairs(n_pairs, world, r)
        parts.append(out[r * share:r * share + (hi - lo)])
    return torch.cat(parts)


@dataclass
class PendingBatch:
    B: int
    k: int
    pool: int
    pool_local: int
    rr_k: int
    w: FusionWeights
    lay: "PayloadLayout"
    buf: object
    pending: "PendingExchange"
    gate_fn: object = None
    rerank_fn: object = None
    stage: int = 1
    slot: int = -1
    bound: object = None
    floor_work: object = None
    terms: object = None
    bm25_mode: str = "forward"
    plain_q: object = None


class _Overlap:
    SLOTS = 3

    def __init__(self, searcher: HybridSearcher, scan_cus: int):
        import torch
        lib, dev = searcher.lib, searcher.device
        total = torch.cuda.get_device_properties(dev).multi_processor_count
        if not (0 < scan_cus < total) or scan_cus % 32 or (total - scan_cus) % 32:
            raise ValueError(f"scan_cus {scan_cus} must be a multiple of 32 inside (0, {total})")
        self.scan_cus, self.handles = scan_cus, []
        streams = []
        for first, n in ((0, scan_cus), (scan_cus, total - scan_cus)):
            h = C.c_void_p()
            _lib.check(lib.rr_stream_create_cu_range(dev.index, first, n, C.byref(h)), "rr_stream_create_cu_range")
            self.handles.append(h)
            streams.append(torch.cuda.ExternalStream(h.value, device=dev))
        self.scan_stream, self.tail_stream = streams
        _lib.check(lib.rr_index_set_scan_cus(searcher.index.handle, scan_cus), "rr_index_set_scan_cus")
        self.lib, self.index = lib, searcher.index
        self.seq = 0
        self.pending = None
        self.unfinished = 0
        self.rings = {}

    def buffers(self, key, make):
        if key not in self.rings:
            self.rings[key] = [make() for _ in range(self.SLOTS)]
        return self.rings[key]

    def close(self):
        import torch
        torch.cuda.synchronize()
        if self.index.handle:
            _lib.check(self.lib.rr_index_set_scan_cus(self.index.handle, 0), "rr_index_set_scan_cus")
        for h in self.handles:
            _lib.check(self.lib.rr_stream_destroy(h), "rr_stream_destroy")
        self.handles = []


class ShardedSearcher:

    def __init__(self, searcher: HybridSearcher, n_total_rows: int, rank: int, world: int, group=None):
        lo, hi = shard_bounds(n_total_rows, world, rank)
        ix = searcher.index
        if ix.row_offset != lo or ix.n_rows != hi - lo:
            raise ValueError(f"rank {rank} must hold rows [{lo}, {hi}); its index holds "
                             f"[{ix.row_offset}, {ix.row_offset + ix.n_rows})")
        self.s, self.rank, self.world, self.group, self.n_total = searcher, rank, world, group, n_total_rows
        self.force_payload = False
        self.use_floor = os.environ.get("RR_NO_SHARD_FLOOR") is None
        self._ov: Optional[_Overlap] = None

    def enable_overlap(self, scan_cus: Optional[int] = None) -> bool:
        if self._ov is not None:
            return True
        if os.environ.get("RR_NO_TAIL_OVERLAP") is not None:
            return False
        forced = os.environ.get("RR_TAIL_OVERLAP_CUS")
        if scan_cus is None and forced:
            scan_cus = int(forced)
        if scan_cus is None and self.world > 1:
            n = self.s.index.n_rows
            scan_cus = 128 if n <= 1_500_000 else 160 if n <= 3_000_000 else 192 if n <= 6_000_000 else None
        if scan_cus is None:
            return False
        self._ov = _Overlap(self.s, scan_cus)
        return True

    def disable_overlap(self) -> None:
        if self._ov is not None:
            self._flush_overlap()
            self._ov.close()
            self._ov = None

    def local_scan(self, q_dev, pool_local: int):
        self._flush_overlap()
        kth = max((pool_local + self.world - 1) // self.world, (pool_local + 7) // 8 + 1)
        return self.s.dense_scan(q_dev, pool_local, min(kth, pool_local))

    def local_payload(self, q_dev, term_id_lists, pool_local: int, bm25_mode: str = "forward", floor=None, buf=None):
        import torch
        self._flush_overlap()
        s = self.s
        B = q_dev.shape[0]
        lay = PayloadLayout(B, pool_local)
        if buf is None:
            buf = torch.empty(lay.nbytes, dtype=torch.uint8, device=s.device)
        v = lay.views(buf)
        import torch.distributed as dist
        if floor is None and self.world > 1 and self.use_floor and dist.is_available() and dist.is_initialized():
            bound = self.local_scan(q_dev, pool_local)
            mine = bound if bound is not None else torch.full((B,), float("-inf"), dtype=torch.float32, device=s.device)
            floor = exchange_floor(mine, self.world, self.group)
            if bound is None:
                floor = False
        if floor is None or floor is False:
            s.dense_pool(q_dev, pool_local, out=(v["rows"], v["dense"]))
        else:
            s.dense_select(q_dev, pool_local, floor, out=(v["rows"], v["dense"]))
        s.bm25_at(term_id_lists, v["rows"], bm25_mode, out=v["bm25"])
        _lib.check(s.lib.rr_index_gather_meta_dev(
            s.index.handle, C.c_void_p(v["rows"].data_ptr()), B * pool_local,
            C.c_void_p(v["n"].data_ptr()), C.c_void_p(v["avg"].data_ptr()),
            C.c_void_p(v["l1p"].data_ptr()), s._stream()), "rr_index_gather_meta_dev")
        return lay, buf

    def search_batch_dev(self, q_dev, term_id_lists: Optional[Sequence[Sequence[int]]], k: int,
                         weights: Optional[FusionWeights] = None, pool_floor: int = 150,
                         bm25_mode: str = "forward", rerank_k: int = 0, gate_fn=None, rerank_fn=None):
        import torch
        w = weights or FusionWeights()
        B = q_dev.shape[0]
        pool = min(max(k, rerank_k, pool_floor), self.n_total)
        self._check_merge_size(pool)
        pool_local = min(pool, self.s.index.n_rows)
        rr_k = min(rerank_k, pool)
        if self.world > 1:
            assert pool_local == pool, "each shard needs at least `pool` rows"
        tl = term_id_lists if term_id_lists is not None else [[] for _ in range(B)]
        s = self.s
        two_pass = gate_fn is not None or (rerank_fn is not None and rr_k > 0)
        if self.world == 1 and not self.force_payload:
            self._flush_overlap()
            rows, dense = s.dense_pool(q_dev, pool)
            bm = s.bm25_at(tl, rows, bm25_mode)
            gate = rerank = None
            if two_pass:
                gate, rerank = self._pool_columns(rows, B, pool, rr_k, gate_fn, rerank_fn)
            return s.fuse(HybridSearcher.make_params(w, min(k, pool), pool, pool, rr_k), B, rows, dense, bm,
                          None, rerank, None, gate)
        return self.finish(self.submit(q_dev, term_id_lists, k, weights, pool_floor, bm25_mode, rerank_k, gate_fn, rerank_fn))

    def submit(self, q_dev, term_id_lists, k: int, weights: Optional[FusionWeights] = None, pool_floor: int = 150,
               bm25_mode: str = "forward", rerank_k: int = 0, gate_fn=None, rerank_fn=None) -> "PendingBatch":
        w = weights or FusionWeights()
        B = q_dev.shape[0]
        pool = min(max(k, rerank_k, pool_floor), self.n_total)
        self._check_merge_size(pool)
        pool_local = min(pool, self.s.index.n_rows)
        rr_k = min(rerank_k, pool)
        if self.world > 1:
            assert pool_local == pool, "each shard needs at least `pool` rows"
        tl = term_id_lists if term_id_lists is not None else [[] for _ in range(B)]
        two_pass = gate_fn is not None or (rerank_fn is not None and rr_k > 0)
        if self._ov is not None:
            if not two_pass:
                t = self._submit_overlapped(q_dev, tl, B, k, pool, pool_local, w, bm25_mode)
                if t is not None:
                    return t
            self._flush_overlap()
        lay, buf = self.local_payload(q_dev, tl, pool_local, bm25_mode)
        pending = exchange_start(buf, self.world, self.group)
        return PendingBatch(B, k, pool, pool_local, rr_k, w, lay, buf, pending, gate_fn, rerank_fn)

    def _check_merge_size(self, pool: int) -> None:
        if self.world * pool > MAX_CANDIDATES:
            raise ValueError(f"{self.world} shards x pool {pool} = {self.world * pool} candidates per query exceed "
                             f"the merge limit of {MAX_CANDIDATES}: the pool may be at most "
                             f"{MAX_CANDIDATES // self.world} with {self.world} shards")

    def _flush_overlap(self) -> None:
        ov = self._ov
        if ov is not None and ov.pending is not None:
            t, ov.pending = ov.pending, None
            self._build_payload(t)

    def _submit_overlapped(self, q_dev, tl, B, k, pool, pool_local, w, bm25_mode):
        import torch
        import torch.distributed as dist
        ov, s = self._ov, self.s
        if ov.unfinished > 2:
            raise RuntimeError("the overlapped pipeline is three batches deep: finish() earlier tickets before submitting more")
        slot = ov.seq % ov.SLOTS
        with_floor = self.world > 1 and self.use_floor and dist.is_available() and dist.is_initialized()
        kth = 0
        if with_floor:
            kth = min(max((pool_local + self.world - 1) // self.world, (pool_local + 7) // 8 + 1), pool_local)
        cur = torch.cuda.current_stream(s.device)
        ready = torch.cuda.Event()
        ready.record(cur)
        with torch.cuda.stream(ov.scan_stream):
            ov.scan_stream.wait_event(ready)
            bound_ring = ov.buffers(("bound", B), lambda: torch.empty((B,), dtype=torch.float32, device=s.device))
            bound = s.dense_scan_slot(slot, q_dev, pool_local, kth, bound_out=bound_ring[slot])
            plain_q = None
            if bound is None:
                if not with_floor:
                    return None
                bound = bound_ring[slot]
                bound.fill_(float("-inf"))
                plain_q = q_dev
            work = exchange_floor_start(bound, self.world, self.group) if with_floor else None
        ov.seq += 1
        ov.unfinished += 1
        lay = PayloadLayout(B, pool_local)
        t = PendingBatch(B, k, pool, pool_local, 0, w, lay, None, None, stage=0, slot=slot,
                         bound=bound if with_floor else None, floor_work=work, terms=tl, bm25_mode=bm25_mode, plain_q=plain_q)
        prev, ov.pending = ov.pending, t
        if prev is not None:
            self._build_payload(prev)
        return t

    def _build_payload(self, t: "PendingBatch") -> None:
        import torch
        ov, s = self._ov, self.s
        B, pool_local, lay = t.B, t.pool_local, t.lay
        ring = ov.buffers(("payload", lay.nbytes, self.world), lambda: (
            torch.empty(lay.nbytes, dtype=torch.uint8, device=s.device),
            torch.empty((self.world, lay.nbytes), dtype=torch.uint8, device=s.device)))
        buf, gathered = ring[t.slot]
        v = lay.views(buf)
        with torch.cuda.stream(ov.tail_stream):
            if t.floor_work is not None:
                t.floor_work.wait()
            if t.plain_q is not None:
                s.dense_pool(t.plain_q, pool_local, out=(v["rows"], v["dense"]), slot=t.slot)
            else:
                s.dense_select_slot(t.slot, B, pool_local, floor=t.bound, out=(v["rows"], v["dense"]))
            s.bm25_at(t.terms, v["rows"], t.bm25_mode, out=v["bm25"])
            _lib.check(s.lib.rr_index_gather_meta_dev(
                s.index.handle, C.c_void_p(v["rows"].data_ptr()), B * pool_local,
                C.c_void_p(v["n"].data_ptr()), C.c_void_p(v["avg"].data_ptr()),
                C.c_void_p(v["l1p"].data_ptr()), s._stream()), "rr_index_gather_meta_dev")
            t.pending = exchange_start(buf, self.world, self.group, out=gathered)
        t.buf, t.stage, t.terms, t.plain_q = buf, 1, None, None

    def _finish_overlapped(self, t: "PendingBatch"):
        import torch
        ov, s = self._ov, self.s
        if t.stage == 0:
            if ov.pending is t:
                ov.pending = None
            self._build_payload(t)
        B, k, pool, pool_local, w, lay = t.B, t.k, t.pool, t.pool_local, t.w, t.lay
        k_out = min(k, pool)
        out_rows, cols, order = ov.buffers(("out", B, pool, k_out), lambda: (
            torch.empty((B, pool), dtype=torch.int64, device=s.device),
            torch.empty((B, 8, pool), dtype=torch.float64, device=s.device),
            torch.empty((B, k_out), dtype=torch.int32, device=s.device)))[t.slot]
        cur = torch.cuda.current_stream(s.device)
        with torch.cuda.stream(ov.tail_stream):
            gathered = t.pending.wait()
            base = gathered.data_ptr()
            ptr = lambda off: C.c_void_p(base + off)
            params = HybridSearcher.make_params(w, k_out, pool, self.world * pool_local, 0,
                                                cand_per_rank=pool_local, stride_bytes=lay.nbytes)
            _lib.check(s.lib.rr_fuse_topk_dev(
                s.index.handle, C.byref(params), B, ptr(lay.off_rows), ptr(lay.off_dense), ptr(lay.off_bm25),
                ptr(lay.off_n), ptr(lay.off_avg), ptr(lay.off_l1p), None, None, None,
                C.c_void_p(out_rows.data_ptr()), C.c_void_p(cols.data_ptr()), C.c_void_p(order.data_ptr()), s._stream()),
                "rr_fuse_topk_dev")
            done = torch.cuda.Event()
            done.record(ov.tail_stream)
        cur.wait_event(done)
        t.stage = 2
        ov.unfinished -= 1
        return out_rows, cols, order

    def finish(self, t: "PendingBatch"):
        import torch
        if t.slot >= 0:
            return self._finish_overlapped(t)
        s = self.s
        B, k, pool, pool_local, rr_k, w, lay = t.B, t.k, t.pool, t.pool_local, t.rr_k, t.w, t.lay
        gate_fn, rerank_fn = t.gate_fn, t.rerank_fn
        two_pass = gate_fn is not None or (rerank_fn is not None and rr_k > 0)
        gathered = t.pending.wait()
        base = gathered.data_ptr()
        ptr = lambda off: C.c_void_p(base + off)
        p = lambda x: C.c_void_p(x.data_ptr()) if x is not None else None

        def fuse(k_out, rerank, gate, rr):
            params = HybridSearcher.make_params(w, k_out, pool, self.world * pool_local, rr,
                                                cand_per_rank=pool_local, stride_bytes=lay.nbytes)
            out_rows = torch.empty((B, pool), dtype=torch.int64, device=s.device)
            cols = torch.empty((B, 8, pool), dtype=torch.float64, device=s.device)
            order = torch.empty((B, params.k), dtype=torch.int32, device=s.device)
            _lib.check(s.lib.rr_fuse_topk_dev(
# ... 35 lines not shown
```

Before: 137,400 queries/s.

## Fuse BM25 scoring of pooled candidates into the dense select kernel

```diff
diff --git a/include/rr_hip.h b/include/rr_hip.h
--- a/include/rr_hip.h
+++ b/include/rr_hip.h
@@ -78,6 +78,9 @@
 int rr_bm25_scores_at_dev(rr_bm25* bm, const int32_t* d_term_ids, const int32_t* d_term_off,
                           int32_t n_queries, const int64_t* d_rows, int32_t pool, int32_t mode,
                           float* d_out, void* stream);
+int rr_dense_topk_bm25_dev(rr_index* ix, int32_t slot, const float* d_queries, int32_t n_queries, int32_t pool,
+                           int64_t* d_out_rows, float* d_out_scores, rr_bm25* bm, const int32_t* d_term_ids,
+                           const int32_t* d_term_off, float* d_out_bm25, void* stream);
 
 int rr_bm25_build(int32_t device, int32_t inputs_on_device, const int32_t* tok, int64_t n_tok,
                   const int64_t* doc_off, int64_t n_src, int64_t n_terms, const int64_t* order,
diff --git a/review-recommender_amd/_lib.py b/review-recommender_amd/_lib.py
--- a/review-recommender_amd/_lib.py
+++ b/review-recommender_amd/_lib.py
@@ -69,6 +69,7 @@
     "rr_bm25_get_scores": (C.c_int, [c_vp, c_vp, c_i32, c_vp]),
     "rr_bm25_scores_at": (C.c_int, [c_vp, c_vp, c_vp, c_i32, c_vp, c_i32, c_i32, c_vp]),
     "rr_bm25_scores_at_dev": (C.c_int, [c_vp, c_vp, c_vp, c_i32, c_vp, c_i32, c_i32, c_vp, c_vp]),
+    "rr_dense_topk_bm25_dev": (C.c_int, [c_vp, c_i32, c_vp, c_i32, c_i32, c_vp, c_vp, c_vp, c_vp, c_vp, c_vp, c_vp]),
     "rr_bm25_build": (C.c_int, [c_i32, c_i32, c_vp, c_i64, c_vp, c_i64, c_i64, c_vp, c_i64, c_i64, c_i64,
                                 c_f64, c_f64, c_i64, c_vp, P(c_vp)]),
     "rr_bm25_build_stats": (C.c_int, [c_vp, c_vp, c_vp]),
diff --git a/review-recommender_amd/csrc/rr_bm25.hip b/review-recommender_amd/csrc/rr_bm25.hip
--- a/review-recommender_amd/csrc/rr_bm25.hip
+++ b/review-recommender_amd/csrc/rr_bm25.hip
@@ -1,37 +1,8 @@
 #include "rr_common.h"
+#include "rr_bm25_dev.h"
 
 #define RR_SLICE 4096
 #define RR_AT_CANDS 64
-
-struct rr_bm25_view {
-    const int64_t* post_indptr;
-    const int32_t* post_docs;
-    const int32_t* post_tf;
-    const int64_t* doc_indptr;
-    const int32_t* doc_terms;
-    const int32_t* doc_tf;
-    const int32_t* doc_len;
-    const double* idf;
-    double avgdl, k1, b;
-    int64_t n_docs, n_terms, row_offset;
-};
-
-__device__ __forceinline__ double rr_bm25_term(double idf, int tf, int dl, double avgdl, double k1,
-                                               double b) {
-    const double f = (double)tf;
-    const double one_minus_b = 1.0 - b;
-    const double norm = one_minus_b + (b * (double)dl) / avgdl;
-    return idf * ((f * (k1 + 1.0)) / (f + k1 * norm));
-}
-
-__device__ __forceinline__ int64_t rr_lower_bound(const int32_t* __restrict__ a, int64_t lo,
-                                                  int64_t hi, int32_t key) {
-    while (lo < hi) {
-        const int64_t mid = lo + ((hi - lo) >> 1);
-        if (a[mid] < key) lo = mid + 1; else hi = mid;
-    }
-    return lo;
-}
 
 __device__ __forceinline__ int64_t rr_lower_bound_wave(const int32_t* __restrict__ a, int64_t lo, int64_t hi, int32_t key) {
     const int lane = threadIdx.x & 63;
@@ -112,43 +83,15 @@
                                                   const int32_t* __restrict__ term_off,
                                                   const int64_t* __restrict__ rows, int pool,
                                                   float* __restrict__ out) {
-    __shared__ double contrib[RR_AT_CANDS][RR_MAX_QTERMS + 1];
-    const int tid = threadIdx.x;
+    __shared__ double contrib[RR_AT_CANDS * (RR_MAX_QTERMS + 1)];
     const int q = blockIdx.y;
     const int c0 = blockIdx.x * RR_AT_CANDS;
     const int t0 = term_off[q];
     const int nt = term_off[q + 1] - t0;
     const int nc = pool - c0 < RR_AT_CANDS ? pool - c0 : RR_AT_CANDS;
-    double sum = 0.0;
-
-    for (int jb = 0; jb < nt; jb += RR_MAX_QTERMS) {
-        const int nj = nt - jb < RR_MAX_QTERMS ? nt - jb : RR_MAX_QTERMS;
-        for (int i = tid; i < nc * nj; i += 256) {
-            const int c = i / nj, j = i % nj;
-            const int64_t d = rows[(int64_t)q * pool + c0 + c] - v.row_offset;
-            const int32_t t = term_ids[t0 + jb + j];
-            double val = 0.0;
-            if (d >= 0 && d < v.n_docs && t >= 0 && t < v.n_terms) {
-                int tf = 0;
-                if (MODE == 0) {
-                    const int64_t s = v.doc_indptr[d], e = v.doc_indptr[d + 1];
-                    const int64_t p = rr_lower_bound(v.doc_terms, s, e, t);
-                    if (p < e && v.doc_terms[p] == t) tf = v.doc_tf[p];
-                } else {
-                    const int64_t s = v.post_indptr[t], e = v.post_indptr[t + 1];
-                    const int64_t p = rr_lower_bound(v.post_docs, s, e, (int32_t)d);
-                    if (p < e && v.post_docs[p] == (int32_t)d) tf = v.post_tf[p];
-                }
-                if (tf > 0) val = rr_bm25_term(v.idf[t], tf, v.doc_len[d], v.avgdl, v.k1, v.b);
-            }
-            contrib[c][j] = val;
-        }
-        __syncthreads();
-        if (tid < nc)
-            for (int j = 0; j < nj; ++j) sum += contrib[tid][j];
-        __syncthreads();
-    }
-    if (tid < nc) out[(int64_t)q * pool + c0 + tid] = (float)sum;
+    const int64_t* qrows = rows + (int64_t)q * pool + c0;
+    rr_bm25_at_cands<MODE, 256>(v, term_ids, t0, nt, [&](int c) { return qrows[c]; }, nc, contrib, RR_MAX_QTERMS + 1,
+                                out + (int64_t)q * pool + c0);
 }
 
 template <typename T>
@@ -159,7 +102,7 @@
     return RR_OK;
 }
 
-static rr_bm25_view rr_view(const rr_bm25* bm) {
+rr_bm25_view rr_bm25_view_of(const rr_bm25* bm) {
     rr_bm25_view v;
     v.post_indptr = bm->d_post_indptr; v.post_docs = bm->d_post_docs; v.post_tf = bm->d_post_tf;
     v.doc_indptr = bm->d_doc_indptr; v.doc_terms = bm->d_doc_terms; v.doc_tf = bm->d_doc_tf;
@@ -167,6 +110,14 @@
     v.avgdl = bm->avgdl; v.k1 = bm->k1; v.b = bm->b;
     v.n_docs = bm->n_docs; v.n_terms = bm->n_terms; v.row_offset = bm->row_offset;
     return v;
+}
+
+int rr_bm25_at_launch(const rr_k2_args& k2, int q0, int nq, const int64_t* d_rows, int pool, hipStream_t st) {
+    const dim3 grid((unsigned)((pool + RR_AT_CANDS - 1) / RR_AT_CANDS), (unsigned)nq);
+    hipLaunchKernelGGL((rr_bm25_at<0>), grid, dim3(256), 0, st, k2.v, k2.term_ids, k2.term_off + q0, d_rows, pool,
+                       k2.out + (int64_t)q0 * pool);
+    RR_HIP_TRY(hipGetLastError());
+    return RR_OK;
 }
 
 extern "C" int rr_bm25_create(int32_t device, int64_t n_docs, int64_t n_terms, int64_t nnz,
@@ -285,7 +236,7 @@
     if (n_terms_in_query)
         hipMemcpyAsync(d_terms, h_term_ids, sizeof(int32_t) * n_terms_in_query, hipMemcpyHostToDevice,
                        bm->stream);
-    hipLaunchKernelGGL(rr_bm25_slices, dim3(grid), dim3(256), 0, bm->stream, rr_view(bm), d_terms,
+    hipLaunchKernelGGL(rr_bm25_slices, dim3(grid), dim3(256), 0, bm->stream, rr_bm25_view_of(bm), d_terms,
                        n_terms_in_query, bm->d_scores, bm->d_dirty);
     hipError_t e = hipGetLastError();
     if (e == hipSuccess)
@@ -313,10 +264,10 @@
     hipStream_t st = (hipStream_t)stream;
     dim3 grid((unsigned)((pool + RR_AT_CANDS - 1) / RR_AT_CANDS), (unsigned)n_queries);
     if (mode == 0)
-        hipLaunchKernelGGL((rr_bm25_at<0>), grid, dim3(256), 0, st, rr_view(bm), d_term_ids, d_term_off,
+        hipLaunchKernelGGL((rr_bm25_at<0>), grid, dim3(256), 0, st, rr_bm25_view_of(bm), d_term_ids, d_term_off,
                            d_rows, pool, d_out);
     else
-        hipLaunchKernelGGL((rr_bm25_at<1>), grid, dim3(256), 0, st, rr_view(bm), d_term_ids, d_term_off,
+        hipLaunchKernelGGL((rr_bm25_at<1>), grid, dim3(256), 0, st, rr_bm25_view_of(bm), d_term_ids, d_term_off,
                            d_rows, pool, d_out);
     RR_HIP_TRY(hipGetLastError());
     return RR_OK;
diff --git a/review-recommender_amd/csrc/rr_bm25_dev.h b/review-recommender_amd/csrc/rr_bm25_dev.h
--- /dev/null
+++ b/review-recommender_amd/csrc/rr_bm25_dev.h
@@ -0,0 +1,55 @@
+#pragma once
+#include "rr_common.h"
+
+__device__ __forceinline__ double rr_bm25_term(double idf, int tf, int dl, double avgdl, double k1,
+                                               double b) {
+    const double f = (double)tf;
+    const double one_minus_b = 1.0 - b;
+    const double norm = one_minus_b + (b * (double)dl) / avgdl;
+    return idf * ((f * (k1 + 1.0)) / (f + k1 * norm));
+}
+
+__device__ __forceinline__ int64_t rr_lower_bound(const int32_t* __restrict__ a, int64_t lo,
+                                                  int64_t hi, int32_t key) {
+    while (lo < hi) {
+        const int64_t mid = lo + ((hi - lo) >> 1);
+        if (a[mid] < key) lo = mid + 1; else hi = mid;
+    }
+    return lo;
+}
+
+template <int MODE, int THREADS, typename RowOf>
+__device__ __forceinline__ void rr_bm25_at_cands(const rr_bm25_view& v, const int32_t* __restrict__ term_ids, int t0, int nt,
+                                                 RowOf row_of, int nc, double* contrib, int stride, float* out) {
+    const int tid = threadIdx.x;
+    double sum = 0.0;
+
+    for (int jb = 0; jb < nt; jb += RR_MAX_QTERMS) {
+        const int nj = nt - jb < RR_MAX_QTERMS ? nt - jb : RR_MAX_QTERMS;
+        for (int i = tid; i < nc * nj; i += THREADS) {
+            const int c = i / nj, j = i % nj;
+            const int64_t d = row_of(c) - v.row_offset;
+            const int32_t t = term_ids[t0 + jb + j];
+            double val = 0.0;
+            if (d >= 0 && d < v.n_docs && t >= 0 && t < v.n_terms) {
+                int tf = 0;
+                if (MODE == 0) {
+                    const int64_t s = v.doc_indptr[d], e = v.doc_indptr[d + 1];
+                    const int64_t p = rr_lower_bound(v.doc_terms, s, e, t);
+                    if (p < e && v.doc_terms[p] == t) tf = v.doc_tf[p];
+                } else {
+                    const int64_t s = v.post_indptr[t], e = v.post_indptr[t + 1];
+                    const int64_t p = rr_lower_bound(v.post_docs, s, e, (int32_t)d);
+                    if (p < e && v.post_docs[p] == (int32_t)d) tf = v.post_tf[p];
+                }
+                if (tf > 0) val = rr_bm25_term(v.idf[t], tf, v.doc_len[d], v.avgdl, v.k1, v.b);
+            }
+            contrib[c * stride + j] = val;
+        }
+        __syncthreads();
+        if (tid < nc)
+            for (int j = 0; j < nj; ++j) sum += contrib[tid * stride + j];
+        __syncthreads();
+    }
+    if (tid < nc) out[tid] = (float)sum;
+}
diff --git a/review-recommender_amd/csrc/rr_common.h b/review-recommender_amd/csrc/rr_common.h
--- a/review-recommender_amd/csrc/rr_common.h
+++ b/review-recommender_amd/csrc/rr_common.h
@@ -45,6 +45,25 @@
     void* flt_pending = nullptr;
 };
 
+struct rr_bm25_view {
+    const int64_t* post_indptr;
+    const int32_t* post_docs;
+    const int32_t* post_tf;
+    const int64_t* doc_indptr;
+    const int32_t* doc_terms;
+    const int32_t* doc_tf;
+    const int32_t* doc_len;
+    const double* idf;
+    double avgdl, k1, b;
+    int64_t n_docs, n_terms, row_offset;
+};
+struct rr_k2_args {
+    rr_bm25_view v;
+    const int32_t* term_ids;
+    const int32_t* term_off;
+    float* out;
+};
+
 struct rr_index {
     int device = 0;
     int64_t n_rows = 0;
@@ -77,6 +96,9 @@
     bool scratch_small = false;
     bool flt_prep_fresh = false;
     void* flt_pending = nullptr;
+    rr_k2_args k2 = {};
+    const int64_t* k2_rows = nullptr;
+    bool k2_chunk_done = false, k2_escape = false;
     unsigned short* d_shadow = nullptr;
     bool shadow_valid = false;
     int32_t use_shadow = 1;
@@ -126,6 +148,9 @@
     std::mutex mu;
 };
 
+rr_bm25_view rr_bm25_view_of(const rr_bm25* bm);
+int rr_bm25_at_launch(const rr_k2_args& k2, int q0, int nq, const int64_t* d_rows, int pool, hipStream_t st);
+
 static inline int64_t rr_round_up(int64_t x, int64_t m) { return (x + m - 1) / m * m; }
 
 #ifdef __HIPCC__
diff --git a/review-recommender_amd/csrc/rr_dense.h b/review-recommender_amd/csrc/rr_dense.h
--- a/review-recommender_amd/csrc/rr_dense.h
+++ b/review-recommender_amd/csrc/rr_dense.h
@@ -55,7 +55,8 @@
                              const float* eps = nullptr, const float* sigma = nullptr, int nq_b = 0,
                              int64_t mmax_set_stride = 0, int64_t smax_set_stride = 0, const float* floor = nullptr);
 void rr_launch_select_rescored(rr_index* ix, const rr_scan_geom& G, int nq, int pool, int64_t* d_rows,
-                               float* d_scores, hipStream_t st, bool floor_mode = false);
+                               float* d_scores, hipStream_t st, bool floor_mode = false, bool with_k2 = false);
+bool rr_k2_wanted(const rr_index* ix, int pool);
 void rr_launch_group_kth(rr_index* ix, const rr_scan_geom& G, int nq_a, int nq_b, int kth, const float* eps, float* d_bound,
                          int64_t smax_set_stride, hipStream_t st);
 int rr_resident_waves(const void* kernel, int threads, int device);
diff --git a/review-recommender_amd/csrc/rr_dense.hip b/review-recommender_amd/csrc/rr_dense.hip
--- a/review-recommender_amd/csrc/rr_dense.hip
+++ b/review-recommender_amd/csrc/rr_dense.hip
@@ -1,6 +1,7 @@
 #include <stdlib.h>
 
 #include "rr_common.h"
+#include "rr_bm25_dev.h"
 #include "rr_dense.h"
 #include "rr_x3.h"
 
@@ -10,6 +11,14 @@
 #define RR_SEL_SORTCAP 8192
 #define RR_SEL_RCAP 8192
 #define RR_SEL_LCAP 4096
+#define RR_SEL_K2_POOL 512
+#define RR_SEL_K2_CAP (RR_SEL_RCAP - RR_SEL_K2_POOL)
+
+static bool rr_tail_v1() {
+    static const bool v1 = getenv("RR_TAIL_V1") != nullptr;
+    return v1;
+}
+static rr_k2_args rr_k2_none() { rr_k2_args a = {}; return a; }
 
 template <int NF>
 __device__ __forceinline__ void rr_load_rows(f32x4 (&dst)[NF], const f32x4* __restrict__ mat,
@@ -579,22 +588,43 @@
     return tau;
 }
 
+__device__ __forceinline__ void rr_k2_from_keys(const rr_k2_args& k2, int qg, uint64_t* cand, int pool, int64_t row_offset) {
+    __syncthreads();
+    const int t0 = k2.term_off[qg];
+    const int nt = k2.term_off[qg + 1] - t0;
+    const int stride = (nt < RR_MAX_QTERMS ? nt : RR_MAX_QTERMS) + 1;
+    int per = RR_SEL_K2_CAP / stride;
+    if (per > RR_SEL_THREADS) per = RR_SEL_THREADS;
+    double* contrib = reinterpret_cast<double*>(cand + RR_SEL_K2_POOL);
+    for (int c0 = 0; c0 < pool; c0 += per) {
+        const int nc = pool - c0 < per ? pool - c0 : per;
+        rr_bm25_at_cands<0, RR_SEL_THREADS>(
+            k2.v, k2.term_ids, t0, nt,
+            [&](int c) { return (int64_t)(0xFFFFFFFFu - (uint32_t)(cand[c0 + c] & 0xFFFFFFFFu)) + row_offset; },
+            nc, contrib, stride, k2.out + (int64_t)qg * pool + c0);
+    }
+}
+
 __global__ __launch_bounds__(RR_SEL_THREADS) void rr_select(
     rr_scan_geom G, const float* __restrict__ sims, const float* __restrict__ gmax,
     const uint32_t* __restrict__ smax, int pool, int64_t row_offset,
     int64_t* __restrict__ out_rows, float* __restrict__ out_scores, int32_t* __restrict__ dbg,
     const int32_t* __restrict__ only_if, int n_total, int64_t sims_slice, int64_t gmax_slice, int64_t smax_slice,
-    const int32_t* __restrict__ qlist, int32_t* __restrict__ clear_flags) {
+    const int32_t* __restrict__ qlist, int32_t* __restrict__ clear_flags,
+    rr_k2_args k2, int k2_q0) {
+    int qg = k2_q0 + (int)blockIdx.x;
     if (qlist) {
         if ((int)blockIdx.x >= qlist[0]) return;
         const int qo = qlist[1 + blockIdx.x] - (int)blockIdx.x;
         out_rows += (int64_t)qo * pool; out_scores += (int64_t)qo * pool; dbg += qo * 16;
         if (threadIdx.x == 0) clear_flags[qo + (int)blockIdx.x] = 0;
+        qg += qo;
     }
     if (gridDim.y > 1) {
         const int y = blockIdx.y;
         if (64 * y + (int)blockIdx.x >= n_total) return;
         only_if += 64 * y;
+        qg += 64 * y;
         out_rows += (int64_t)64 * y * pool; out_scores += (int64_t)64 * y * pool; dbg += 64 * y * 16;
         sims += y * sims_slice; gmax += y * gmax_slice; smax += y * smax_slice;
     }
@@ -700,6 +730,7 @@
         out_rows[(int64_t)q * pool + i] = (int64_t)row + row_offset;
         out_scores[(int64_t)q * pool + i] = rr_key2f((uint32_t)(key >> 32));
     }
+    if (k2.out) rr_k2_from_keys(k2, qg, cand, pool, row_offset);
 }
 
 __global__ __launch_bounds__(RR_SEL_THREADS) void rr_select_mtiles(
@@ -860,12 +891,13 @@
     }
 }
 
-template <int RCAP>
+template <int RCAP, bool K2 = false>
 __global__ __launch_bounds__(RR_SEL_THREADS) void rr_select_rescored(
     rr_scan_geom G, const uint32_t* __restrict__ mtiles, const int32_t* __restrict__ count,
     const uint32_t* __restrict__ tau_of, const float* __restrict__ sc, int pool, int64_t row_offset,
     int64_t* __restrict__ out_rows, float* __restrict__ out_scores, int32_t* __restrict__ fb,
-    int32_t* __restrict__ dbg, int floor_mode) {
+    int32_t* __restrict__ dbg, int floor_mode, rr_k2_args k2, int k2_q0) {
+    static_assert(!K2 || RCAP >= RR_SEL_K2_POOL + RR_SEL_K2_CAP, "K2's contributions share the key area");
     __shared__ uint32_t counters[2];
     __shared__ uint64_t cand[RCAP];
     const int tid = threadIdx.x;
@@ -933,7 +965,10 @@
         out_rows[(int64_t)q * pool + i] = (int64_t)row + row_offset;
         out_scores[(int64_t)q * pool + i] = rr_key2f((uint32_t)(key >> 32));
     }
-}
+    if (K2) rr_k2_from_keys(k2, k2_q0 + q, cand, pool, row_offset);
+}
+
+static int rr_k2_q0(const rr_index* ix, const int64_t* d_rows, int pool) { return (int)((d_rows - ix->k2_rows) / pool); }
 
 rr_x3_scratch rr_x3_scratch_of(const rr_index* ix) {
     rr_x3_scratch s;
@@ -960,15 +995,22 @@
                        smax_set_stride, floor);
 }
 void rr_launch_select_rescored(rr_index* ix, const rr_scan_geom& G, int nq, int pool, int64_t* d_rows,
-                               float* d_scores, hipStream_t st, bool floor_mode) {
+                               float* d_scores, hipStream_t st, bool floor_mode, bool with_k2) {
     const rr_x3_scratch s = rr_x3_scratch_of(ix);
-    if (pool <= 512)
+    if (with_k2)
+        hipLaunchKernelGGL((rr_select_rescored<RR_SEL_RCAP, true>), dim3(nq), dim3(RR_SEL_THREADS), 0, st, G, s.mtiles, s.count,
+                           s.tau, s.sc, pool, ix->row_offset, d_rows, d_scores, s.fb, ix->d_sel_trace, floor_mode ? 1 : 0,
+                           ix->k2, rr_k2_q0(ix, d_rows, pool));
+    else if (pool <= 512)
         hipLaunchKernelGGL((rr_select_rescored<RR_SEL_RCAP>), dim3(nq), dim3(RR_SEL_THREADS), 0, st, G, s.mtiles, s.count, s.tau,
-                           s.sc, pool, ix->row_offset, d_rows, d_scores, s.fb, ix->d_sel_trace, floor_mode ? 1 : 0);
+                           s.sc, pool, ix->row_offset, d_rows, d_scores, s.fb, ix->d_sel_trace, floor_mode ? 1 : 0,
+                           rr_k2_none(), 0);
     else
         hipLaunchKernelGGL((rr_select_rescored<RR_SEL_CCAP>), dim3(nq), dim3(RR_SEL_THREADS), 0, st, G, s.mtiles, s.count, s.tau,
-                           s.sc, pool, ix->row_offset, d_rows, d_scores, s.fb, ix->d_sel_trace, floor_mode ? 1 : 0);
-}
+                           s.sc, pool, ix->row_offset, d_rows, d_scores, s.fb, ix->d_sel_trace, floor_mode ? 1 : 0,
+                           rr_k2_none(), 0);
+}
+bool rr_k2_wanted(const rr_index* ix, int pool) { return ix->k2.out && pool <= RR_SEL_K2_POOL && !rr_tail_v1(); }
 
 __global__ __launch_bounds__(RR_SEL_THREADS) void rr_group_kth(rr_scan_geom G, const uint32_t* __restrict__ smax, int kth,
                                                                const float* __restrict__ eps, float* __restrict__ bound,
@@ -1144,7 +1186,8 @@
     const dim3 grid(slices > 1 ? RR_MFMA_MAXQ : nq, slices > 1 ? slices : 1);
     hipLaunchKernelGGL(rr_select, grid, dim3(RR_SEL_THREADS), 0, st, G, ix->d_sims, ix->d_gmax,
                        ix->d_smax, pool, ix->row_offset, d_rows, d_scores, ix->d_sel_trace, only_if, nq, sims_slice,
-                       gmax_slice, smax_slice, (const int32_t*)nullptr, (int32_t*)nullptr);
+                       gmax_slice, smax_slice, (const int32_t*)nullptr, (int32_t*)nullptr,
+                       ix->k2_escape ? ix->k2 : rr_k2_none(), ix->k2_escape ? rr_k2_q0(ix, d_rows, pool) : 0);
 }
 int rr_resident_waves(const void* kernel, int threads, int device) {
     int per_cu = 0, cus = 0;
@@ -1190,7 +1233,8 @@
                        (const int32_t*)flags, nq, ix->d_flag_list);
     hipLaunchKernelGGL(rr_select, dim3(8), dim3(RR_SEL_THREADS), 0, st, G, ix->d_sims, ix->d_gmax, ix->d_smax, pool,
                        ix->row_offset, d_rows, d_scores, ix->d_sel_trace, (const int32_t*)nullptr, 8, (int64_t)0, (int64_t)0,
-                       (int64_t)0, (const int32_t*)ix->d_flag_list, flags);
+                       (int64_t)0, (const int32_t*)ix->d_flag_list, flags,
+                       ix->k2_escape ? ix->k2 : rr_k2_none(), ix->k2_escape ? rr_k2_q0(ix, d_rows, pool) : 0);
     RR_HIP_TRY(hipGetLastError());
     return RR_OK;
 }
@@ -1217,7 +1261,7 @@
     }
     hipLaunchKernelGGL(rr_select, dim3(nq), dim3(RR_SEL_THREADS), 0, st, G, ix->d_sims, ix->d_gmax,
                        ix->d_smax, pool, ix->row_offset, d_rows, d_scores, ix->d_sel_trace, (const int32_t*)nullptr, nq, (int64_t)0, (int64_t)0, (int64_t)0,
-                       (const int32_t*)nullptr, (int32_t*)nullptr);
+                       (const int32_t*)nullptr, (int32_t*)nullptr, rr_k2_none(), 0);
     RR_HIP_TRY(hipGetLastError());
     return RR_OK;
 }
@@ -1249,7 +1293,7 @@
     if (ix->ring_head - ix->ring_tail > rr_index::kRing) ix->ring_tail = ix->ring_head - rr_index::kRing;
     hipLaunchKernelGGL(rr_select, dim3(nq), dim3(RR_SEL_THREADS), 0, st, G, ix->d_sims, ix->d_gmax,
                        ix->d_smax, pool, ix->row_offset, d_rows, d_scores, ix->d_sel_trace, (const int32_t*)nullptr, nq, (int64_t)0, (int64_t)0, (int64_t)0,
-                       (const int32_t*)nullptr, (int32_t*)nullptr);
+                       (const int32_t*)nullptr, (int32_t*)nullptr, rr_k2_none(), 0);
     RR_HIP_TRY(hipGetLastError());
     return RR_OK;
 }
@@ -1293,6 +1337,7 @@
         int64_t* rows = d_rows + (int64_t)q0 * pool;
         float* scores = d_scores + (int64_t)q0 * pool;
         int n;
+        ix->k2_chunk_done = false;
         bool small = false;
         if (mfma_ok && left > valu_max && !f32_chain && !exact_scan && ix->scan_mode == RR_SCAN_MODE_DEFAULT &&
             (ix->n_rows + 63) / 64 < 8 * (int64_t)pool)
@@ -1323,6 +1368,10 @@
                       : rr_dense_chunk(ix, q, n, pool, rows, scores, st, q0 == 0);
         }
         if (rc) return rc;
+        if (ix->k2.out && !ix->k2_chunk_done) {
+            rc = rr_bm25_at_launch(ix->k2, q0, n, rows, pool, st);
+            if (rc) return rc;
+        }
         q0 += n;
     }
     return RR_OK;
@@ -1411,9 +1460,14 @@
     return rr_dense_select_slot_dev(ix, 0, n_queries, pool, d_floor, d_out_rows, d_out_scores, stream);
 }
 
-extern "C" int rr_dense_topk_slot_dev(rr_index* ix, int32_t slot, const float* d_queries, int32_t n_queries,
-                                      int32_t pool, int64_t* d_out_rows, float* d_out_scores,
-                                      void* stream) {
+struct rr_k2_guard {
+    rr_index* ix;
+    ~rr_k2_guard() { ix->k2 = rr_k2_none(); ix->k2_rows = nullptr; ix->k2_chunk_done = ix->k2_escape = false; }
+};
+
+static int rr_dense_topk_slot_k2(rr_index* ix, int32_t slot, const float* d_queries, int32_t n_queries,
+                                 int32_t pool, int64_t* d_out_rows, float* d_out_scores,
+                                 void* stream, const rr_k2_args* k2) {
     RR_REQUIRE(ix && d_queries && d_out_rows && d_out_scores, "rr_dense_topk_dev: NULL argument");
     RR_REQUIRE(n_queries >= 1 && n_queries <= RR_MAX_BATCH, "rr_dense_topk_dev: n_queries %d out of [1,%d]",
                n_queries, RR_MAX_BATCH);
@@ -1426,6 +1480,11 @@
     std::lock_guard<std::mutex> lk(ix->mu);
     RR_HIP_TRY(hipSetDevice(ix->device));
     hipStream_t st = (hipStream_t)stream;
+    rr_k2_guard k2_guard{ix};
+    if (k2) {
+        ix->k2 = *k2;
+        ix->k2_rows = d_out_rows;
+    }
     int rc0 = rr_slot_activate(ix, slot);
     if (rc0) return rc0;
     rr_flt_drop_pending(ix);
@@ -1447,6 +1506,26 @@
     ix->flt_prep_fresh = false;
     if (rc) return rc;
     return rr_scratch_leave(ix, st);
+}
+
+extern "C" int rr_dense_topk_slot_dev(rr_index* ix, int32_t slot, const float* d_queries, int32_t n_queries,
+                                      int32_t pool, int64_t* d_out_rows, float* d_out_scores,
+                                      void* stream) {
+    return rr_dense_topk_slot_k2(ix, slot, d_queries, n_queries, pool, d_out_rows, d_out_scores, stream, nullptr);
+}
+
+extern "C" int rr_dense_topk_bm25_dev(rr_index* ix, int32_t slot, const float* d_queries, int32_t n_queries, int32_t pool,
+                                      int64_t* d_out_rows, float* d_out_scores, rr_bm25* bm, const int32_t* d_term_ids,
+                                      const int32_t* d_term_off, float* d_out_bm25, void* stream) {
+    RR_REQUIRE(ix && bm && d_term_ids && d_term_off && d_out_bm25, "rr_dense_topk_bm25_dev: NULL argument");
+    RR_REQUIRE(bm->device == ix->device, "rr_dense_topk_bm25_dev: the index is on device %d, the BM25 handle on %d", ix->device, bm->device);
+    if (!bm->d_idf) { rr_set_error("rr_dense_topk_bm25_dev: no idf yet (rr_bm25_set_idf)"); return RR_E_STATE; }
+    rr_k2_args k2;
+    k2.v = rr_bm25_view_of(bm);
+    k2.term_ids = d_term_ids;
+    k2.term_off = d_term_off;
+    k2.out = d_out_bm25;
+    return rr_dense_topk_slot_k2(ix, slot, d_queries, n_queries, pool, d_out_rows, d_out_scores, stream, &k2);
 }
 
 extern "C" int rr_dense_topk_dev(rr_index* ix, const float* d_queries, int32_t n_queries,
diff --git a/review-recommender_amd/csrc/rr_dense_flt.hip b/review-recommender_amd/csrc/rr_dense_flt.hip
--- a/review-recommender_amd/csrc/rr_dense_flt.hip
+++ b/review-recommender_amd/csrc/rr_dense_flt.hip
@@ -1214,8 +1214,15 @@
                            X.mtiles, X.count, X.fb, X.sc, plane_rows, X.tau, X.eps);
     RR_HIP_TRY(hipGetLastError());
     if (!(parts & 4)) return RR_OK;
-    rr_launch_select_rescored(ix, G, nq, pool, d_rows, d_scores, st, floor != nullptr);
+    const bool with_k2 = !floor && rr_k2_wanted(ix, pool);
+    rr_launch_select_rescored(ix, G, nq, pool, d_rows, d_scores, st, floor != nullptr, with_k2);
     RR_HIP_TRY(hipGetLastError());
+    if (with_k2) ix->k2_chunk_done = true;
+    struct escape_k2 {
+        rr_index* ix;
+        ~escape_k2() { ix->k2_escape = false; }
+    } escape_guard{ix};
+    ix->k2_escape = with_k2;
     if (!ROWS_BF16) {
         const int rc = rr_dense_listed_fallback(ix, d_q, nq, pool, d_rows, d_scores, X.fb, st);
         if (rc != RR_OK) return rc;
diff --git a/review-recommender_amd/engine.py b/review-recommender_amd/engine.py
--- a/review-recommender_amd/engine.py
+++ b/review-recommender_amd/engine.py
@@ -202,6 +202,26 @@
             C.c_void_p(rows_dev.data_ptr()), pool, {"forward": 0, "postings": 1}[mode],
             C.c_void_p(out.data_ptr()), self._stream()), "rr_bm25_scores_at_dev")
         return out
+
+    def dense_pool_bm25(self, q_dev, pool: int, term_id_lists, mode: str = "forward"):
+        torch = _torch()
+        staged = isinstance(term_id_lists, StagedTerms)
+        flat_form = isinstance(term_id_lists, tuple) and len(term_id_lists) == 2 and isinstance(term_id_lists[1], np.ndarray)
+        empty = (term_id_lists.n_ids == 0) if staged else \
+            (len(term_id_lists[0]) == 0) if flat_form else not any(len(t) for t in term_id_lists)
+        if self.bm25 is None or empty or mode != "forward":
+            rows, dense = self.dense_pool(q_dev, pool)
+            return rows, dense, self.bm25_at(term_id_lists, rows, mode)
+        B = q_dev.shape[0]
+        rows = torch.empty((B, pool), dtype=torch.int64, device=self.device)
+        dense = torch.empty((B, pool), dtype=torch.float32, device=self.device)
+        out = torch.empty((B, pool), dtype=torch.float32, device=self.device)
+        ids_dev, off_dev = (term_id_lists.ids, term_id_lists.off) if staged else self._stage_terms(term_id_lists)[:2]
+        _lib.check(self.lib.rr_dense_topk_bm25_dev(
+            self.index.handle, 0, C.c_void_p(q_dev.data_ptr()), B, pool, C.c_void_p(rows.data_ptr()),
+            C.c_void_p(dense.data_ptr()), self.bm25.handle, C.c_void_p(ids_dev.data_ptr()), C.c_void_p(off_dev.data_ptr()),
+            C.c_void_p(out.data_ptr()), self._stream()), "rr_dense_topk_bm25_dev")
+        return rows, dense, out
 
     def _stage_terms(self, term_id_lists):
         torch = _torch()
diff --git a/review-recommender_amd/sharded.py b/review-recommender_amd/sharded.py
--- a/review-recommender_amd/sharded.py
+++ b/review-recommender_amd/sharded.py
@@ -303,8 +303,11 @@
         two_pass = gate_fn is not None or (rerank_fn is not None and rr_k > 0)
         if self.world == 1 and not self.force_payload:
             self._flush_overlap()
-            rows, dense = s.dense_pool(q_dev, pool)
-            bm = s.bm25_at(tl, rows, bm25_mode)
+            if two_pass:
+                rows, dense = s.dense_pool(q_dev, pool)
+                bm = s.bm25_at(tl, rows, bm25_mode)
+            else:
+                rows, dense, bm = s.dense_pool_bm25(q_dev, pool, tl, bm25_mode)
             gate = rerank = None
             if two_pass:
                 gate, rerank = self._pool_columns(rows, B, pool, rr_k, gate_fn, rerank_fn)
```

After: 135,300 queries/s. -1.5%, worse.
